# Cwuwhu/FCD-GAN-pytorch

Measured on AMD Instinct MI355X. Metric: tile-pairs/sec (train step) on 256x256x13 OSCD, higher is better.
Workload: dtype f32

## Files before the change

fcd_gan_pytorch_amd/Loss.py:

```python
import os
import warnings

import torch
import torch.nn as nn
import torch.nn.functional as F

from . import _lib
from . import _ops as ops
from .ssim import MS_SSIM

_VGG_CFG = (64, 64, 'M', 128, 128, 'M', 256, 256, 256, 'M', 512, 512, 512, 'M', 512, 512, 512, 'M')
_TAPS = (29, 22, 15, 8, 3)


def _vgg16_features():
    layers, cin = [], 3
    for v in _VGG_CFG:
        if v == 'M':
            layers.append(nn.MaxPool2d(kernel_size=2, stride=2))
        else:
            layers += [nn.Conv2d(cin, v, kernel_size=3, padding=1), nn.ReLU(inplace=True)]
            cin = v
    return nn.Sequential(*layers)


_HUB_FILE = 'vgg16-397923af.pth'


def _vgg_checkpoint_path():
    path = os.environ.get('FCDGAN_VGG16_WEIGHTS', '')
    if path:
        if not os.path.exists(path):
            raise FileNotFoundError('FCDGAN_VGG16_WEIGHTS=%s does not exist' % path)
        return path
    roots = [os.path.join(os.environ['TORCH_HOME'], 'hub')] if os.environ.get('TORCH_HOME') else []
    roots.append(os.path.join(os.path.expanduser('~'), '.cache', 'torch', 'hub'))
    for r in roots:
        cand = os.path.join(r, 'checkpoints', _HUB_FILE)
        if os.path.exists(cand):
            return cand
    return None


def _load_vgg_weights(net, allow_seeded):
    path = _vgg_checkpoint_path()
    if path:
        sd = torch.load(path, map_location='cpu')
        sd = {k.replace('features.', ''): v for k, v in sd.items() if 'classifier' not in k}
        net.load_state_dict(sd)
        return True
    if not allow_seeded:
        raise RuntimeError(
            'PerceptionLoss: the ImageNet VGG16 weights the reference uses (Loss.py:25, vgg16(pretrained=True)) are '
            'not available offline.  Set FCDGAN_VGG16_WEIGHTS to a torch-saved state_dict of torchvision\'s vgg16 '
            '(or place %s in the torch hub cache), or pass allow_seeded=True to run on fixed-seed random filters '
            '(parity tests / benchmarks only: the loss value then differs from the reference\'s).' % _HUB_FILE)
    warnings.warn('PerceptionLoss: allow_seeded=True -- VGG16 runs on a fixed-seed He initialisation, NOT on the '
                  'ImageNet weights of the reference.')
    g = torch.Generator().manual_seed(16)
    with torch.no_grad():
        for m in net:
            if isinstance(m, nn.Conv2d):
                fan_in = m.weight.shape[1] * 9
                m.weight.copy_(torch.randn(m.weight.shape, generator=g) * (2.0 / fan_in) ** 0.5)
                m.bias.zero_()
    return False


class PerceptionLoss(nn.Module):

    def __init__(self, feature_layer=1, perception_perBand=False, allow_seeded=False):
        super(PerceptionLoss, self).__init__()
        vgg = _vgg16_features().eval()
        self.pretrained = _load_vgg_weights(vgg, allow_seeded)
        for param in vgg.parameters():
            param.requires_grad = False
        self.net = vgg
        feature_layer = feature_layer if feature_layer > 0 else 1
        feature_layer = feature_layer if feature_layer < 6 else 5
        self.feature_layer_list = list(_TAPS[:feature_layer])
        self.perception_perBand = perception_perBand
        self.loss = nn.MSELoss()

    def _first_filter_1ch(self):
        w = self.net[0].weight
        hit = self.__dict__.get('_fcd_w1')
        if hit is None or hit[0] != w._version or hit[1].device != w.device:
            hit = (w._version, w.detach().sum(dim=1, keepdim=True).contiguous())
            self.__dict__['_fcd_w1'] = hit
        return hit[1]

    def _features(self, z, single_band=False):
        taps = {}
        layers = list(self.net)
        i = 0
        while i < len(layers):
            layer = layers[i]
            run = self._frozen_run(layers, i) if isinstance(layer, nn.Conv2d) and i > 0 else None
            if run is not None and ops.frozen_chain_ok(z, [c.weight for c in run[0]]):
                convs, pool, nxt = run
                z = ops.frozen_conv_chain(z, [c.weight for c in convs], [c.bias for c in convs], pool=pool)
                last = nxt - 1
                if last in self.feature_layer_list:
                    taps[last] = z
                i = nxt
                continue
            if isinstance(layer, nn.Conv2d):
                fuse = i + 1 < len(layers) and isinstance(layers[i + 1], nn.ReLU)
                wgt = self._first_filter_1ch() if (i == 0 and single_band) else layer.weight
                pool_next = fuse and i + 2 < len(layers) and isinstance(layers[i + 2], nn.MaxPool2d)
                if pool_next and (i + 1) not in self.feature_layer_list:
                    z = ops.conv2d_relu_maxpool2(z, wgt, layer.bias)
                    i += 3
                    continue
                z = ops.conv2d(z, wgt, layer.bias, 1, 1, relu=fuse)
                if fuse:
                    i += 1
            elif isinstance(layer, nn.ReLU):
                z = ops.bn_act(z, None, ops.ACT_RELU)
            else:
                z = ops.maxpool2(z)
            if i in self.feature_layer_list:
                taps[i] = z
            i += 1
        return taps

    def _frozen_run(self, layers, i):
        convs, k = [], i
        while (k + 1 < len(layers) and isinstance(layers[k], nn.Conv2d) and isinstance(layers[k + 1], nn.ReLU)
               and not layers[k].weight.requires_grad and layers[k].bias is not None and not layers[k].bias.requires_grad):
            convs.append(layers[k])
            k += 2
            if (k - 1) in self.feature_layer_list:
                break
        if len(convs) < 2:
            return None
        pool = (k < len(layers) and isinstance(layers[k], nn.MaxPool2d) and (k - 1) not in self.feature_layer_list
                and k not in self.feature_layer_list)
        return convs, pool, (k + 1 if pool else k)

    def forward(self, target_image, generate_image, cmask, stacked=None):
        n = target_image.shape[0]
        nl = len(self.feature_layer_list)
        if not self.perception_perBand:
            assert target_image.shape[1] >= 3
            if target_image.shape[1] == 3:
                z = stacked if stacked is not None else masked_pair(target_image, generate_image, cmask)
            else:
                keep = 1 - cmask
                z = torch.cat([target_image[:, 0:3] * keep, generate_image[:, 0:3] * keep], dim=0)
            nb = n
        else:
            C, H, W = target_image.shape[1:]
            z = stacked if stacked is not None else masked_pair(target_image, generate_image, cmask)
            z = z.reshape(2 * n * C, 1, H, W)
            nb = n * C
        feats = self._features(z, single_band=self.perception_perBand)
        total = 0
        for i in sorted(self.feature_layer_list):
            f = feats[i]
            total = total + mse_halves(f, nb) / nl
        return total


def masked_pair(target_image, generate_image, cmask):
    if not _lib.switch('FUSED_GLUE') or not target_image.is_cuda:
        keep = 1 - cmask
        return torch.cat([target_image * keep, generate_image * keep], dim=0)
    return ops.masked_stack([target_image, generate_image], cmask)


class _MseHalves(torch.autograd.Function):

    @staticmethod
    def forward(ctx, f, nb):
        d = f[:nb] - f[nb:]
        ctx.save_for_backward(d)
        ctx.n_total = f.shape[0]
        flat = d.reshape(-1)
        return torch.dot(flat, flat) / flat.numel()

    @staticmethod
    def backward(ctx, gout):
        d, = ctx.saved_tensors
        nb = d.shape[0]
        c = gout * (2.0 / d.numel())
        g = torch.empty((ctx.n_total,) + tuple(d.shape[1:]), dtype=d.dtype, device=d.device)
        torch.mul(d, c, out=g[:nb])
        torch.mul(d, -c, out=g[nb:])
        return g, None


def mse_halves(f, nb):
    if f.shape[0] != 2 * nb:
        raise ValueError('mse_halves: %d rows for two halves of %d' % (f.shape[0], nb))
    if not _lib.switch('FUSED_GLUE') or not f.is_cuda:
        return F.mse_loss(f[:nb], f[nb:])
    return _MseHalves.apply(f, nb)


def _masked_ratio(a, b, m, kind, complement, scale, skip_zero):
    if not _lib.switch('FUSED_GLUE'):
        num, wsum = ops.masked_sums(a, b, m, kind, complement)
        return _per_sample_ratio(num, wsum, scale, skip_zero)
    return ops.masked_ratio_mean(a, b, m, kind, complement, scale, skip_zero)


def _per_sample_ratio(num, wsum, scale, skip_zero):
    if skip_zero:
        ok = wsum != 0
        terms = torch.where(ok, num * scale / torch.where(ok, wsum, torch.ones_like(wsum)), torch.zeros_like(num))
    else:
        terms = num * scale / wsum
    return terms.sum() / num.shape[0]


class CNetLoss(nn.Module):

    def __init__(self, channel=4, perception_layer=1, perception_perBand=True, allow_seeded=False):
        super(CNetLoss, self).__init__()
        self.mse = nn.MSELoss()
        self.loss_generator = nn.L1Loss()
        self.loss_perception = PerceptionLoss(feature_layer=perception_layer, perception_perBand=perception_perBand,
                                              allow_seeded=allow_seeded)
        self.ssim = MS_SSIM(data_range=1.0, channel=channel)

    def forward(self, target_image, generate_image, cmap, generator_mask_switch=False):
        C = target_image.shape[1]
        cmask = (torch.sign(cmap - 0.5) + 1) / 2
        generator_loss = _masked_ratio(target_image, generate_image, cmap, 0, True, 1.0 / C, skip_zero=False)
        l1_loss = torch.mean(abs(cmap))
        n = target_image.shape[0]
        z = masked_pair(target_image, generate_image, cmap)
        perception_loss = self.loss_perception(target_image, generate_image, cmask if generator_mask_switch else cmap,
                                               stacked=None if generator_mask_switch else z)
        ssim_loss = 1 - self.ssim(*z.split(n, dim=0))
        return generator_loss, l1_loss, perception_loss, ssim_loss


class CGeneratorLoss(nn.Module):

    def __init__(self, channel=3, perception_layer=1, perception_perBand=False, allow_seeded=False):
        super(CGeneratorLoss, self).__init__()
        self.loss_generator = nn.MSELoss()
        self.ssim = MS_SSIM(data_range=1.0, channel=channel)
        self.loss_perception = PerceptionLoss(feature_layer=perception_layer, perception_perBand=perception_perBand,
                                              allow_seeded=allow_seeded)

    def forward(self, target_image, generate_image, cmap):
        C = target_image.shape[1]
        generator_loss = _masked_ratio(target_image, generate_image, cmap, 1, True, 1.0 / C, skip_zero=True)
        n = target_image.shape[0]
        z = masked_pair(target_image, generate_image, cmap)
        ssim_loss = 1 - self.ssim(*z.split(n, dim=0))
        perception_loss = self.loss_perception(target_image, generate_image, cmap, stacked=z)
        return generator_loss, ssim_loss, perception_loss


def region_loss(cmap, region, criterion):
    if isinstance(criterion, str):
        kind = {'l1': 0, 'mse': 1}[criterion]
    elif isinstance(criterion, nn.L1Loss):
        kind = 0
    elif isinstance(criterion, nn.MSELoss):
        kind = 1
    else:
        raise TypeError('region_loss: criterion must be nn.L1Loss / nn.MSELoss')
    return _masked_ratio(cmap, None, region, kind, False, 1.0 / cmap.shape[1], skip_zero=True)
```

fcd_gan_pytorch_amd/_lib.py:

```python
import ctypes
import os
import subprocess

import torch

from ctypes import POINTER, Structure, c_char_p, c_double, c_float, c_int, c_int32, c_int64, c_size_t, c_void_p

_HERE = os.path.dirname(os.path.abspath(__file__))
LIB_PATH = os.environ.get('FCD_LIB') or os.path.join(_HERE, 'libfcdgan_hip.so')
CSRC = os.path.join(_HERE, 'csrc')


class FcdError(RuntimeError):
    pass


def build(force=False, verbose=False):
    if force and os.path.exists(LIB_PATH):
        os.remove(LIB_PATH)
    cmd = ['make', '-C', CSRC, '-j', str(max(2, os.cpu_count() or 2))]
    r = subprocess.run(cmd, stdout=subprocess.PIPE, stderr=subprocess.STDOUT, text=True)
    if verbose or r.returncode != 0:
        print(r.stdout)
    if r.returncode != 0 or not os.path.exists(LIB_PATH):
        raise FcdError('building libfcdgan_hip.so failed (make -C %s)' % CSRC)
    return LIB_PATH


def kernel_source_hash():
    import runpy
    return runpy.run_path(os.path.join(CSRC, 'source_hash.py'))['source_hash']()


class WinoFwdExtras(Structure):
    _fields_ = [('v_keep', c_void_p), ('bn_part', c_void_p), ('bn_groups', c_int32), ('in_groups', c_int32),
                ('in_scale', c_void_p), ('in_shift', c_void_p)]


class ConvDesc(Structure):
    _fields_ = [(n, c_int32) for n in ('N', 'C', 'H', 'W', 'K', 'R', 'S', 'stride', 'pad', 'P', 'Q')]


P = c_void_p

_SIGS = {
    'fcd_version': (c_int, []),
    'fcd_build_hash': (c_char_p, []),
    'fcd_last_error_string': (c_char_p, []),
    'fcd_switch_count': (c_int, []),
    'fcd_switch_name': (c_char_p, [c_int]),
    'fcd_switch_help': (c_char_p, [c_int]),
    'fcd_switch_default': (c_int, [c_int]),
    'fcd_switch_get': (c_int, [c_char_p]),
    'fcd_switch_set': (c_int, [c_char_p, c_int]),
    'fcd_conv_packed_elems': (c_int64, [c_int, c_int, c_int, c_int, c_int]),
    'fcd_conv_pack_weights': (c_int, [P, P, c_int, c_int, c_int, c_int, c_int, P]),
    'fcd_conv2d_fwd': (c_int, [POINTER(ConvDesc), P, P, P, P, c_int, P]),
    'fcd_conv2d_fwd_ex': (c_int, [POINTER(ConvDesc), P, P, P, P, c_int, P, c_float, P, P]),
    'fcd_conv2d_relu_bits_bytes': (c_size_t, [POINTER(ConvDesc)]),
    'fcd_conv2d_fwd_relu_bits': (c_int, [POINTER(ConvDesc), P, P, P, P, P, P]),
    'fcd_conv2d_bwd_data_bits': (c_int, [POINTER(ConvDesc), P, P, P, P, P]),
    'fcd_conv1x1_head_plan': (c_int, [c_int, c_int, c_int, c_int]),
    'fcd_conv1x1_head_fwd': (c_int, [P, P, P, P, c_int, c_int, c_int, c_int, P]),
    'fcd_conv1x1_head_bwd_ws_bytes': (c_size_t, [c_int, c_int]),
    'fcd_conv1x1_head_bwd': (c_int, [P, P, P, P, P, P, P, c_int, c_int, c_int, P, c_size_t, P]),
    'fcd_conv1x1_head_bn_fwd': (c_int, [P, P, P, c_int, P, P, P, c_int, c_int, c_int, c_int, P]),
    'fcd_conv1x1_head_bn_bwd_ws_bytes': (c_size_t, [c_int, c_int, c_int]),
    'fcd_conv1x1_head_bn_bwd': (c_int, [P, P, P, P, P, P, P, P, c_int, P, P, P, P, P, c_int, c_int, c_int, P, c_size_t, P]),
    'fcd_conv_wino_plan': (c_int, [POINTER(ConvDesc), c_int]),
    'fcd_conv_wino_set': (c_int, [c_int]),
    'fcd_conv_wino_split_set': (c_int, [c_int]),
    'fcd_conv_wgrad_split_set': (c_int, [c_int]),
    'fcd_conv_wino_cat_ok': (c_int, [P]),
    'fcd_conv2d_fwd_wino_cat': (c_int, [P, P, P, c_int, P, P, P, c_int, P, c_size_t, P]),
    'fcd_conv2d_bwd_data_wino_cat': (c_int, [P, P, P, P, P, P, c_int, P, c_size_t, P]),
    'fcd_conv2d_bwd_weight_bias_cat': (c_int, [P, P, P, c_int, P, P, P, P, P, c_size_t, P]),
    'fcd_conv_wino_ws_bytes': (c_size_t, [POINTER(ConvDesc), c_int]),
    'fcd_conv_wino_keepv_bytes': (c_size_t, [POINTER(ConvDesc)]),
    'fcd_conv_wino_in_affine_ok': (c_int, [POINTER(ConvDesc)]),
    'fcd_conv_wino_bn_split': (c_int, [POINTER(ConvDesc), c_int]),
    'fcd_conv_wino_bn_part_bytes': (c_size_t, [POINTER(ConvDesc), c_int]),
    'fcd_conv2d_fwd_wino_x': (c_int, [POINTER(ConvDesc), P, P, P, P, c_int, P, P, P, c_size_t, P, P]),
    'fcd_conv2d_fwd_wino_cat_x': (c_int, [P, P, P, c_int, P, P, P, c_int, P, c_size_t, P, P]),
    'fcd_conv_wino_relu_bits_bytes': (c_size_t, [POINTER(ConvDesc)]),
    'fcd_conv2d_fwd_wino_relu_bits': (c_int, [POINTER(ConvDesc), P, P, P, P, P, P, c_size_t, P]),
    'fcd_conv2d_bwd_data_wino_bits': (c_int, [POINTER(ConvDesc), P, P, P, P, P, c_size_t, P]),
    'fcd_conv_wino_chain_ok': (c_int, [P, c_int, c_int]),
    'fcd_conv_wino_chain_ws_bytes': (c_size_t, [P, c_int, c_int]),
    'fcd_conv_wino_chain_bits_bytes': (c_size_t, [POINTER(ConvDesc)]),
    'fcd_conv2d_fwd_wino_chain': (c_int, [P, c_int, P, P, P, P, P, P, P, P, c_size_t, P]),
    'fcd_conv2d_bwd_data_wino_chain': (c_int, [P, c_int, P, P, P, P, P, P, P, c_size_t, P]),
    'fcd_conv2d_fwd_wino_keepv': (c_int, [POINTER(ConvDesc), P, P, P, P, c_int, P, P, P, c_size_t, P, P]),
    'fcd_conv2d_fwd_wino_cat_keepv': (c_int, [P, P, P, c_int, P, P, P, c_int, P, c_size_t, P, P]),
    'fcd_conv2d_bwd_weight_bias_v': (c_int, [POINTER(ConvDesc), P, P, P, P, P, P, c_size_t, P]),
    'fcd_conv_wino_filter_elems': (c_int64, [c_int, c_int, c_int, c_int]),
    'fcd_conv_wino_pack': (c_int, [P, P, c_int, c_int, c_int, c_int, P]),
    'fcd_conv_wino_pack_blocks': (c_int, [c_int, c_int, c_int]),
    'fcd_conv_wino_pack_multi': (c_int, [P, c_int, c_int, c_double, P]),
    'fcd_conv2d_fwd_wino': (c_int, [POINTER(ConvDesc), P, P, P, P, c_int, P, P, P, c_size_t, P]),
    'fcd_conv2d_bwd_data_wino': (c_int, [POINTER(ConvDesc), P, P, P, P, P, P, c_size_t, P]),
    'fcd_conv_s2_dgrad_plan': (c_int, [POINTER(ConvDesc)]),
    'fcd_conv_s2_dgrad_packed_elems': (c_int64, [c_int, c_int]),
    'fcd_conv_s2_dgrad_pack': (c_int, [P, P, c_int, c_int, P]),
    'fcd_conv2d_bwd_data_s2': (c_int, [POINTER(ConvDesc), P, P, P, P, P]),
    'fcd_conv_wino2_plan': (c_int, [POINTER(ConvDesc), c_int]),
    'fcd_conv_wino2_filter_elems': (c_int64, [c_int, c_int, c_int]),
    'fcd_conv_wino2_pack': (c_int, [P, P, c_int, c_int, c_int, P]),
    'fcd_conv2d_fwd_wino2': (c_int, [POINTER(ConvDesc), P, P, P, P, c_int, P, c_float, P, P, P, P]),
    'fcd_conv2d_bwd_data_wino2': (c_int, [POINTER(ConvDesc), P, P, P, P, P, P]),
    'fcd_conv2d_bwd_data': (c_int, [POINTER(ConvDesc), P, P, P, P, P]),
    'fcd_conv2d_fwd_relu_pool': (c_int, [POINTER(ConvDesc), P, P, P, P, P, P]),
    'fcd_conv2d_bwd_data_pooled': (c_int, [POINTER(ConvDesc), P, P, P, P, P]),
    'fcd_conv2d_bwd_weight_ws_bytes': (c_size_t, [POINTER(ConvDesc)]),
    'fcd_conv2d_bwd_weight': (c_int, [POINTER(ConvDesc), P, P, P, P, P, c_size_t, P]),
    'fcd_conv2d_bwd_weight_bias': (c_int, [POINTER(ConvDesc), P, P, P, P, P, P, c_size_t, P]),
    'fcd_channel_sum_ws_bytes': (c_size_t, [c_int]),
    'fcd_channel_sum': (c_int, [P, P, P, c_int, c_int, c_int, P, c_size_t, P]),
    'fcd_bn_act_ws_bytes': (c_size_t, [c_int, c_int]),
    'fcd_bn_act_fwd': (c_int, [P, P, c_int, c_int, c_int, c_int, c_int, P, P, P, P, c_float, c_float, c_int,
                               P, P, c_int, P, c_float, P, c_size_t, P]),
    'fcd_bn_act_fwd_replay': (c_int, [P, P, c_int, c_int, c_int, c_int, P, c_int, P, P, P, P, c_float, c_float, P, P, c_int, P,
                                      c_float, P, c_size_t, P]),
    'fcd_bn_act_bwd': (c_int, [P, P, P, c_int, c_int, c_int, c_int, c_int, P, P, P, P, c_float, c_int, P, P,
                               c_int, P, c_float, P, P, P, P, c_size_t, P]),
    'fcd_bn_relu_pool_plan': (c_int, [c_int, c_int, c_int, c_int, c_int]),
    'fcd_bn_relu_pool_fwd': (c_int, [P, P, P, c_int, c_int, c_int, c_int, c_int, P, P, P]),
    'fcd_bn_relu_pool_bwd': (c_int, [P, P, P, P, c_int, c_int, c_int, c_int, c_int, P, P, P, P, P, P, P, c_size_t, P]),
    'fcd_bn_train_stats': (c_int, [P, c_int, c_int, c_int, c_int, P, c_int, P, P, P, P, c_float, c_float, P, P, P, P, P, c_size_t, P]),
    'fcd_bn_act_fwd_parts': (c_int, [P, P, c_int, c_int, c_int, c_int, P, c_int, P, P, P, P, c_float, c_float, P, P, c_int, P, c_float,
                                     P, c_size_t, P]),
    'fcd_bn_partial_stats': (c_int, [P, P, c_int, c_int, c_int, c_int, P, c_size_t, P]),
    'fcd_bn_act_fwd_from_stats': (c_int, [P, P, c_int, c_int, c_int, c_int, P, c_double, P, P, P, P, c_float, c_float,
                                          P, P, c_int, P, c_float, P, c_size_t, P]),
    'fcd_bn_bwd_partial': (c_int, [P, P, P, c_int, c_int, c_int, c_int, P, P, P, P, c_int, P, c_float, P, c_size_t, P]),
    'fcd_bn_bwd_from_sums': (c_int, [P, P, P, c_int, c_int, c_int, c_int, P, c_double, P, P, P, P, c_int, P, c_float,
                                     P, c_size_t, P]),
    'fcd_maxpool2_fwd': (c_int, [P, P, c_int, c_int, c_int, P]),
    'fcd_maxpool2_bwd': (c_int, [P, P, P, c_int, c_int, c_int, P]),
    'fcd_maxpool2_bwd_add': (c_int, [P, P, P, P, c_int, c_int, c_int, P]),
    'fcd_upsample2x_fwd': (c_int, [P, P, c_int, c_int, c_int, P]),
    'fcd_upsample2x_bwd': (c_int, [P, P, c_int, c_int, c_int, P]),
    'fcd_avgpool2_pad_fwd': (c_int, [P, P, c_int, c_int, c_int, P]),
    'fcd_avgpool2_pad_bwd': (c_int, [P, P, c_int, c_int, c_int, P]),
    'fcd_pair_gap_diff_fwd': (c_int, [P, P, c_int, c_int, c_int, c_int, P]),
    'fcd_pair_gap_diff_bwd': (c_int, [P, P, c_int, c_int, c_int, c_int, P]),
    'fcd_masked_stack_fwd': (c_int, [P, P, P, P, c_int, P, P, c_int, c_int, c_int, P]),
    'fcd_masked_stack_bwd': (c_int, [P, P, P, P, P, c_int, P, P, P, P, P, P, c_int, c_int, c_int, P]),
    'fcd_normalize_tiles': (c_int, [P, P, P, P, P, c_int, c_int, c_int, P]),
    'fcd_masked_recon_ws_bytes': (c_size_t, [c_int]),
    'fcd_masked_recon_fwd': (c_int, [P, P, P, P, c_int, c_int, c_int, c_int, c_int, P, c_size_t, P]),
    'fcd_masked_recon_bwd': (c_int, [P, P, P, P, P, P, P, P, c_int, c_int, c_int, c_int, c_int, P]),
    'fcd_ratio_mean_fwd': (c_int, [P, c_int, c_float, c_int, P, P]),
    'fcd_ratio_mean_bwd': (c_int, [P, P, c_int, c_float, c_int, P, P, P]),
    'fcd_ssim_ws_bytes': (c_size_t, [c_int, c_int, c_int]),
    'fcd_ssim_level_fwd': (c_int, [P, P, P, c_int, P, c_int, c_int, c_int, c_float, c_float, P, c_size_t, P]),
    'fcd_ssim_level_bwd': (c_int, [P, P, P, c_int, P, P, P, P, c_int, c_int, c_int, c_float, c_float, P, c_size_t, P]),
    'fcd_adam_step': (c_int, [P, P, P, P, c_int64, c_float, c_float, c_float, c_float, c_float, c_int, c_float, P]),
    'fcd_rmsprop_step': (c_int, [P, P, P, c_int64, c_float, c_float, c_float, c_float, c_float, P]),
    'fcd_adam_step_h': (c_int, [P, P, P, P, c_int64, P, c_float, c_float, c_float, c_float, c_float, P]),
    'fcd_rmsprop_step_h': (c_int, [P, P, P, c_int64, P, c_float, c_float, c_float, c_float, P]),
    'fcd_prof_enable': (None, [c_int]),
    'fcd_prof_families': (c_int, []),
    'fcd_prof_detail_read': (c_int64, [c_char_p, c_int64, c_int]),
    'fcd_prof_read': (c_int, [POINTER(c_double), c_int]),
    'fcd_prof_family_name': (c_char_p, [c_int]),
}

EXPORTS = sorted(_SIGS)


def _load():
    if not os.path.exists(LIB_PATH):
        raise FcdError('libfcdgan_hip.so not found at %s -- run `python -c "import __graft_entry__ as g; '
                       'g.build()"` (needs hipcc); there is no CPU fallback.' % LIB_PATH)
    lib = ctypes.CDLL(LIB_PATH)
    for name, (res, args) in _SIGS.items():
        try:
            fn = getattr(lib, name)
        except AttributeError:
            raise FcdError('libfcdgan_hip.so does not export %s (stale build?)' % name)
        fn.restype = res
        fn.argtypes = args
    return lib


lib = _load()


def switch(name):
    v = lib.fcd_switch_get(name.encode())
    if v < 0:
        raise FcdError('unknown switch %r' % name)
    return v


def set_switch(name, value):
    old = lib.fcd_switch_set(name.encode(), -1 if value is None else int(value))
    if old < 0:
        raise FcdError('unknown switch %r' % name)
    return old


class switched:

    def __init__(self, **kv):
        self.kv, self.old = kv, {}

    def __enter__(self):
        for k, v in self.kv.items():
            self.old[k] = set_switch(k, v)
        return self

    def __exit__(self, *exc):
        for k, v in self.old.items():
            set_switch(k, v)
        return False


def switch_table():
    return [(lib.fcd_switch_name(i).decode(), lib.fcd_switch_get(lib.fcd_switch_name(i)), lib.fcd_switch_default(i),
             lib.fcd_switch_help(i).decode()) for i in range(lib.fcd_switch_count())]


def build_hash():
    return lib.fcd_build_hash().decode()


def check(rc, what=''):
    if rc != 0:
        msg = lib.fcd_last_error_string()
        raise FcdError('%s failed (%d): %s' % (what or 'fcd call', rc, msg.decode() if msg else ''))


def prof_read(reset=True):
    nf = lib.fcd_prof_families()
    buf = (c_double * (nf * 4))()
    check(lib.fcd_prof_read(buf, 1 if reset else 0), 'fcd_prof_read')
    out = {}
    for f in range(nf):
        out[lib.fcd_prof_family_name(f).decode()] = dict(ms=buf[f * 4], launches=int(buf[f * 4 + 1]),
                                                         flops=buf[f * 4 + 2], bytes=buf[f * 4 + 3])
    return out


def prof_detail(reset=True):
    need = lib.fcd_prof_detail_read(None, 0, 0)
    buf = ctypes.create_string_buffer(int(need))
    lib.fcd_prof_detail_read(buf, need, 1 if reset else 0)
    out = []
    for line in buf.value.decode().splitlines():
        fam, tag, ms, fl, by = line.split('\t')
        out.append(dict(family=fam, tag=tag, ms=float(ms), flops=float(fl), bytes=float(by)))
    return out
```

fcd_gan_pytorch_amd/_ops.py:

```python
import collections
import ctypes
import threading
import time

import torch

from . import _lib
from ._lib import ConvDesc, check, lib, switch

ACT_NONE, ACT_RELU, ACT_LEAKY, ACT_PRELU = 0, 1, 2, 3


class _LaunchWindow:
    EVERY = 128

    def __init__(self):
        self.count, self.events = 0, collections.deque()

    def note(self, stream):
        self.count += 1
        if self.count % self.EVERY:
            return
        limit = switch('LAUNCH_WINDOW')
        if limit <= 0 or torch.cuda.is_current_stream_capturing():
# ... 278 lines not shown
                nw = lib.fcd_conv_wino_relu_bits_bytes(ctypes.byref(d))
                if nw and switch('WINO_RELU_BITS'):
                    wbits = torch.empty(nw // 2, dtype=torch.int16, device=x.device)
                    ws = _ws(lib.fcd_conv_wino_ws_bytes(ctypes.byref(d), 0), x.device)
                    check(lib.fcd_conv2d_fwd_wino_relu_bits(ctypes.byref(d), _p(x), _p(wino_weight(weight, 0, 4)), _p(b), _p(y),
                                                            _p(wbits), _p(ws), ws.numel(), _stream()),
                          'fcd_conv2d_fwd_wino_relu_bits')
        vk = None
        if bits is None and wbits is None:
            vk = _keepv(d, ctx.needs_input_grad[1], x.device)
            _fwd_conv(d, x, weight, b, y, relu, v_keep=vk, bn_part=bn_part, bn_groups=bn_groups)
        ctx.save_for_backward(x if (weight.requires_grad and vk is None) else None, weight,
                              (y if relu and bits is None and wbits is None else None), bits, vk, wbits)
        ctx.geom = (stride, pad, bias is not None, tuple(x.shape))
        ctx.bias_param = bias
        return y

    @staticmethod
    def backward(ctx, dy):
        x, weight, yrelu, bits, vk, wbits = ctx.saved_tensors
        stride, pad, has_bias, xshape = ctx.geom
        dy = _dev(dy, 'conv grad')
        d = _desc(xshape, weight.shape, stride, pad)
        dx = dw = db = None
        if ctx.needs_input_grad[0]:
            dx = torch.empty(xshape, dtype=torch.float32, device=dy.device)
            if bits is not None:
                check(lib.fcd_conv2d_bwd_data_bits(ctypes.byref(d), _p(dy), _p(bits), _p(packed_weight(weight, 1)), _p(dx),
                                                   _stream()), 'fcd_conv2d_bwd_data_bits')
            elif wbits is not None:
                ws = _ws(lib.fcd_conv_wino_ws_bytes(ctypes.byref(d), 1), dy.device)
                check(lib.fcd_conv2d_bwd_data_wino_bits(ctypes.byref(d), _p(dy), _p(wbits), _p(wino_weight(weight, 1, 4)), _p(dx),
                                                        _p(ws), ws.numel(), _stream()), 'fcd_conv2d_bwd_data_wino_bits')
            else:
                _bwd_data_conv(d, dy, weight, dx, yrelu=yrelu)
        want_db = has_bias and ctx.needs_input_grad[2]
        if ctx.needs_input_grad[1]:
            dw = _grad_out(weight, weight.shape, dy.device)
            if want_db:
                db = _grad_out(ctx.bias_param, (d.K,), dy.device)
            ws = _ws(lib.fcd_conv2d_bwd_weight_ws_bytes(ctypes.byref(d)), dy.device)
            if vk is not None:
                check(lib.fcd_conv2d_bwd_weight_bias_v(ctypes.byref(d), _p(vk), _p(dy), _p(yrelu), _p(dw), _p(db), _p(ws),
                                                       ws.numel(), _stream()), 'fcd_conv2d_bwd_weight_bias_v')
            else:
                check(lib.fcd_conv2d_bwd_weight_bias(ctypes.byref(d), _p(x), _p(dy), _p(yrelu), _p(dw), _p(db), _p(ws),
                                                     ws.numel(), _stream()), 'fcd_conv2d_bwd_weight_bias')
        elif want_db:
            db = _channel_sum(dy, yrelu, d.N, d.K, d.P * d.Q)
        return dx, dw, db, None, None, None, None, None


def _ptr_list(ptrs):
    return (ctypes.c_void_p * len(ptrs))(*ptrs)


class _ConvPairCat(torch.autograd.Function):

    @staticmethod
    def forward(ctx, f2n, up, weight, bias, relu, bn_part=None, bn_groups=0):
        f2n, up = _dev(f2n, 'skip pair'), _dev(up, 'upsampled input')
        n, cu, H, W = up.shape
        c = f2n.shape[1]
        d = _desc((n, 2 * c + cu, H, W), weight.shape, 1, 1)
        y = torch.empty((d.N, d.K, d.P, d.Q), dtype=torch.float32, device=up.device)
        half = n * c * H * W * 4
        srcs = _ptr_list([f2n.data_ptr(), f2n.data_ptr() + half, up.data_ptr()])
        chans = (ctypes.c_int * 3)(c, c, cu)
        ws = _ws(lib.fcd_conv_wino_ws_bytes(ctypes.byref(d), 0), up.device)
        b = _dev(bias, 'conv bias') if bias is not None else None
        vk = _keepv(d, ctx.needs_input_grad[2], up.device)
        check(lib.fcd_conv2d_fwd_wino_cat_x(ctypes.byref(d), srcs, chans, 3, _p(wino_weight(weight, 0, 4)), _p(b), _p(y),
                                            1 if relu else 0, _p(ws), ws.numel(), _extras(vk, bn_part, bn_groups), _stream()),
              'fcd_conv2d_fwd_wino_cat')
        keep_x = weight.requires_grad and vk is None
        ctx.save_for_backward(f2n if keep_x else None, up if keep_x else None, weight, y if relu else None, vk)
        ctx.geom = (tuple(f2n.shape), tuple(up.shape), bias is not None)
        ctx.bias_param = bias
        return y

    @staticmethod
    def backward(ctx, dy):
        f2n, up, weight, yrelu, vk = ctx.saved_tensors
        fshape, ushape, has_bias = ctx.geom
        dy = _dev(dy, 'conv grad')
        n, cu, H, W = ushape
        c = fshape[1]
        d = _desc((n, 2 * c + cu, H, W), weight.shape, 1, 1)
        chans = (ctypes.c_int * 3)(c, c, cu)
        half = n * c * H * W * 4
        df = du = dw = db = None
        if ctx.needs_input_grad[0] or ctx.needs_input_grad[1]:
            df = torch.empty(fshape, dtype=torch.float32, device=dy.device)
            du = torch.empty(ushape, dtype=torch.float32, device=dy.device)
            ws = _ws(lib.fcd_conv_wino_ws_bytes(ctypes.byref(d), 1), dy.device)
            check(lib.fcd_conv2d_bwd_data_wino_cat(ctypes.byref(d), _p(dy), _p(yrelu), _p(wino_weight(weight, 1, 4)),
                                                   _ptr_list([df.data_ptr(), df.data_ptr() + half, du.data_ptr()]), chans, 3,
                                                   _p(ws), ws.numel(), _stream()), 'fcd_conv2d_bwd_data_wino_cat')
        want_db = has_bias and ctx.needs_input_grad[3]
        if ctx.needs_input_grad[2]:
            dw = _grad_out(weight, weight.shape, dy.device)
            if want_db:
                db = _grad_out(ctx.bias_param, (d.K,), dy.device)
            ws = _ws(lib.fcd_conv2d_bwd_weight_ws_bytes(ctypes.byref(d)), dy.device)
            if vk is not None:
                check(lib.fcd_conv2d_bwd_weight_bias_v(ctypes.byref(d), _p(vk), _p(dy), _p(yrelu), _p(dw), _p(db), _p(ws),
                                                       ws.numel(), _stream()), 'fcd_conv2d_bwd_weight_bias_v')
            else:
                check(lib.fcd_conv2d_bwd_weight_bias_cat(ctypes.byref(d), _ptr_list([f2n.data_ptr(), f2n.data_ptr() + half,
                                                                                      up.data_ptr()]), chans, 3, _p(dy), _p(yrelu),
                                                         _p(dw), _p(db), _p(ws), ws.numel(), _stream()),
                      'fcd_conv2d_bwd_weight_bias_cat')
        elif want_db:
            db = _channel_sum(dy, yrelu, d.N, d.K, d.P * d.Q)
        return df, du, dw, db, None, None, None


def conv3x3_pair_cat_ok(f2n, up, weight):
    if f2n.dim() != 4 or up.dim() != 4 or tuple(weight.shape[2:]) != (3, 3) or not switch('PAIR_CAT'):
        return False
    n, cu, H, W = up.shape
    c = f2n.shape[1]
    if f2n.shape[0] != 2 * n or tuple(f2n.shape[2:]) != (H, W) or (c % 32) or (cu % 32) or weight.shape[1] != 2 * c + cu:
        return False
    if not (f2n.is_cuda and up.is_cuda and f2n.is_contiguous() and up.is_contiguous()):
        return False
    d = _desc((n, 2 * c + cu, H, W), weight.shape, 1, 1)
    return bool(lib.fcd_conv_wino_cat_ok(ctypes.byref(d)))


def conv3x3_pair_cat(f2n, up, weight, bias=None, relu=False, bn_groups=0):
    n, cu, H, W = up.shape
    d = _desc((n, 2 * f2n.shape[1] + cu, H, W), weight.shape, 1, 1)
    part = _bn_part(d, bn_groups, relu, up.device)
    return _tag_bn(_ConvPairCat.apply(f2n, up, weight, bias, bool(relu), part, int(bn_groups)), d, part, bn_groups)


def conv2d(x, weight, bias=None, stride=1, padding=0, relu=False, bn_groups=0):
    part = None
    if bn_groups and not relu and x.is_cuda:
        d = _desc(x.shape, weight.shape, int(stride), int(padding))
        part = _bn_part(d, bn_groups, relu, x.device)
        if part is not None:
            return _tag_bn(_Conv2d.apply(x, weight, bias, int(stride), int(padding), False, part, int(bn_groups)), d, part, bn_groups)
    return _Conv2d.apply(x, weight, bias, int(stride), int(padding), bool(relu))


@torch.no_grad()
def conv2d_infer(x, weight, bias, stride=1, padding=0, act=ACT_NONE, slope=None, slope_imm=0.0, residual=None):
    x = _dev(x, 'conv input')
    d = _desc(x.shape, weight.shape, int(stride), int(padding))
    y = torch.empty((d.N, d.K, d.P, d.Q), dtype=torch.float32, device=x.device)
    res = _dev(residual, 'residual') if residual is not None else None
    if res is not None and res.shape != y.shape:
        raise _lib.FcdError('conv2d_infer: residual shape %s != output shape %s' % (tuple(res.shape), tuple(y.shape)))
    if lib.fcd_conv_wino2_plan(ctypes.byref(d), 0):
        check(lib.fcd_conv2d_fwd_wino2(ctypes.byref(d), _p(x), _p(wino2_weight(weight, 0)), _p(bias), _p(y), act, _p(slope),
                                       float(slope_imm), _p(res), None, None, _stream()), 'fcd_conv2d_fwd_wino2')
        return y
    wp = packed_weight(weight, 0)
    check(lib.fcd_conv2d_fwd_ex(ctypes.byref(d), _p(x), _p(wp), _p(bias), _p(y), act, _p(slope), float(slope_imm),
                                _p(res), _stream()), 'fcd_conv2d_fwd_ex')
    return y


class _ConvReluPool(torch.autograd.Function):

    @staticmethod
    def forward(ctx, x, weight, bias):
        x = _dev(x, 'conv input')
        d = _desc(x.shape, weight.shape, 1, 1)
        yp = torch.empty((d.N, d.K, d.P // 2, d.Q // 2), dtype=torch.float32, device=x.device)
        code = torch.empty(yp.shape, dtype=torch.uint8, device=x.device)
        _fwd_conv(d, x, weight, bias, None, True, pool_y=yp, code=code)
        ctx.save_for_backward(weight, code)
        ctx.xshape = tuple(x.shape)
        return yp

    @staticmethod
    def backward(ctx, dyp):
        weight, code = ctx.saved_tensors
        dyp = _dev(dyp, 'pooled grad')
        d = _desc(ctx.xshape, weight.shape, 1, 1)
        dx = None
        if ctx.needs_input_grad[0]:
            dx = torch.empty(ctx.xshape, dtype=torch.float32, device=dyp.device)
            _bwd_data_conv(d, dyp, weight, dx, code=code)
        return dx, None, None


def conv_relu_pool_supported(x, weight):
    K, C, R, S = weight.shape
    if switch('NO_POOLFUSE'):
        return False
    return (R == 3 and S == 3 and K > 32 and C > 32 and not weight.requires_grad
            and x.shape[2] >= 2 and x.shape[3] >= 2)


def conv2d_relu_maxpool2(x, weight, bias):
    if conv_relu_pool_supported(x, weight) and (bias is None or not bias.requires_grad):
        return _ConvReluPool.apply(x, weight, bias)
    return maxpool2(conv2d(x, weight, bias, 1, 1, relu=True))


def _desc_array(descs):
    arr = (ConvDesc * len(descs))()
    for i, d in enumerate(descs):
        for f, _ in ConvDesc._fields_:
            setattr(arr[i], f, getattr(d, f))
    return arr


def _chain_descs(xshape, weights):
    N, C, H, W = xshape
    out = []
    for w in weights:
        out.append(_desc((N, C, H, W), w.shape, 1, 1))
        C = w.shape[0]
    return out


def _chain_bwd_start(descs):
    n = len(descs)
    for j in range(n):
        if lib.fcd_conv_wino_chain_ok(_desc_array(descs[j:]), n - j, 1):
            return j
    return n


def frozen_chain_ok(x, weights):
    if not switch('WINO_CHAIN') or len(weights) < 2 or len(weights) > 8 or not x.is_cuda or x.dim() != 4:
        return False
    if any(w.requires_grad or tuple(w.shape[2:]) != (3, 3) for w in weights):
        return False
    descs = _chain_descs(x.shape, weights)
    if not lib.fcd_conv_wino_chain_ok(_desc_array(descs), len(descs), 0):
        return False
    return _chain_bwd_start(descs) <= 1


class _FrozenChain(torch.autograd.Function):

    @staticmethod
    def forward(ctx, x, pool, *wb):
        x = _dev(x, 'conv input')
        n = len(wb) // 2
        weights, biases = list(wb[:n]), [_dev(b, 'conv bias') for b in wb[n:]]
        descs = _chain_descs(x.shape, weights)
        darr = _desc_array(descs)
        N, H, W = descs[0].N, descs[0].H, descs[0].W
        K = descs[-1].K
        dev = x.device
        want = ctx.needs_input_grad[0]
        bits = []
        if want:
            for i in range(n - (1 if pool else 0)):
                bits.append(torch.empty(lib.fcd_conv_wino_chain_bits_bytes(ctypes.byref(descs[i])) // 2, dtype=torch.int16, device=dev))
        y = yp = code = None
        if pool:
            yp = torch.empty((N, K, H // 2, W // 2), dtype=torch.float32, device=dev)
            code = torch.empty(yp.shape, dtype=torch.uint8, device=dev)
        else:
            y = torch.empty((N, K, H, W), dtype=torch.float32, device=dev)
        Us = [wino_weight(w, 0, 4) for w in weights]
        ws = _ws(lib.fcd_conv_wino_chain_ws_bytes(darr, n, 0), dev)
        bptr = _ptr_list([b.data_ptr() for b in bits] + [None] * (n - len(bits))) if want else None
        check(lib.fcd_conv2d_fwd_wino_chain(darr, n, _p(x), _ptr_list([u.data_ptr() for u in Us]),
                                            _ptr_list([b.data_ptr() for b in biases]), _p(y), _p(yp), _p(code), bptr, _p(ws),
                                            ws.numel(), _stream()), 'fcd_conv2d_fwd_wino_chain')
        ctx.save_for_backward(code, *weights, *bits)
        ctx.geom = (tuple(x.shape), n, bool(pool))
        return yp if pool else y

    @staticmethod
    def backward(ctx, dy):
        xshape, n, pool = ctx.geom
        saved = ctx.saved_tensors
        code, weights, bits = saved[0], list(saved[1:1 + n]), list(saved[1 + n:])
        dy = _dev(dy, 'conv grad')
        if not ctx.needs_input_grad[0]:
            return (None,) * (2 + 2 * n)
        descs = _chain_descs(xshape, weights)
        j = _chain_bwd_start(descs)
        if j > 1:
            raise _lib.FcdError('frozen_conv_chain: no backward run for these layers (frozen_chain_ok was not consulted)')
        dev = dy.device
        dx = torch.empty((xshape[0], descs[j].C) + tuple(xshape[2:]), dtype=torch.float32, device=dev)
        darr = _desc_array(descs[j:])
        m = n - j
        ws = _ws(lib.fcd_conv_wino_chain_ws_bytes(darr, m, 1), dev)
        blist = [(bits[i].data_ptr() if i < len(bits) else None) for i in range(j, n)]
        U1 = [wino_weight(w, 1, 4) for w in weights[j:]]
        check(lib.fcd_conv2d_bwd_data_wino_chain(darr, m, _p(dy), _p(code) if pool else None, _ptr_list(blist),
                                                 _p(bits[0]) if j == 1 else None, _ptr_list([u.data_ptr() for u in U1]),
                                                 _p(dx), _p(ws), ws.numel(), _stream()), 'fcd_conv2d_bwd_data_wino_chain')
        if j == 1:
            dx0 = torch.empty(xshape, dtype=torch.float32, device=dev)
            _bwd_data_conv(descs[0], dx, weights[0], dx0)
            dx = dx0
        return (dx, None) + (None,) * (2 * n)


def frozen_conv_chain(x, weights, biases, pool=False):
    return _FrozenChain.apply(x, bool(pool), *weights, *biases)


class _ConvT2x2(torch.autograd.Function):

    @staticmethod
    def forward(ctx, x, weight, bias):
        x = _dev(x, 'convT input')
        Cin, Cout = weight.shape[0], weight.shape[1]
        N, _, h, w = x.shape
        d = ConvDesc(N, Cout, 2 * h, 2 * w, Cin, 2, 2, 2, 0, h, w)
        y = torch.empty((N, Cout, 2 * h, 2 * w), dtype=torch.float32, device=x.device)
        wpb = packed_weight(weight, 1)
        check(lib.fcd_conv2d_bwd_data(ctypes.byref(d), _p(x), None, _p(wpb), _p(y), _stream()), 'convT fwd')
        if bias is not None:
            y += bias.view(1, -1, 1, 1)
        ctx.save_for_backward(x, weight)
        ctx.has_bias = bias is not None
        return y

    @staticmethod
    def backward(ctx, dy):
        x, weight = ctx.saved_tensors
        dy = _dev(dy, 'convT grad')
        Cin, Cout = weight.shape[0], weight.shape[1]
        N, _, h, w = x.shape
        d = ConvDesc(N, Cout, 2 * h, 2 * w, Cin, 2, 2, 2, 0, h, w)
        dx = dw = db = None
        if ctx.needs_input_grad[0]:
            dx = torch.empty_like(x)
            wp = packed_weight(weight, 0)
            check(lib.fcd_conv2d_fwd(ctypes.byref(d), _p(dy), _p(wp), None, _p(dx), 0, _stream()), 'convT bwd data')
        if ctx.needs_input_grad[1]:
            dw = _grad_out(weight, weight.shape, x.device)
            ws = _ws(lib.fcd_conv2d_bwd_weight_ws_bytes(ctypes.byref(d)), x.device)
            check(lib.fcd_conv2d_bwd_weight(ctypes.byref(d), _p(dy), _p(x), None, _p(dw), _p(ws), ws.numel(), _stream()),
                  'convT bwd weight')
        if ctx.has_bias and ctx.needs_input_grad[2]:
            db = _channel_sum(dy, None, N, Cout, 4 * h * w)
        return dx, dw, db


def conv_transpose2x2(x, weight, bias=None):
    return _ConvT2x2.apply(x, weight, bias)


SYNC_BN = {'enabled': False, 'group': None}


def _sync_world():
    if SYNC_BN['enabled']:
        from . import dp
        return dp.exchanging(SYNC_BN['group'])
    return 0


def sync_bn_active():
    return bool(_sync_world())


class _BnAct(torch.autograd.Function):
    @staticmethod
    def forward(ctx, x, gamma, beta, slope, running_mean, running_var, training, momentum, eps, groups, act,
                slope_imm, order=None):
        x = _dev(x, 'bn input')
        N, C, H, W = x.shape
        has_bn = gamma is not None
        y = torch.empty_like(x)
        save_mean = save_invstd = None
        if has_bn and training:
            save_mean = torch.empty(groups * C, dtype=torch.float32, device=x.device)
            save_invstd = torch.empty(groups * C, dtype=torch.float32, device=x.device)
        ws = _ws(lib.fcd_bn_act_ws_bytes(C, groups), x.device)
        world = _sync_world() if (has_bn and training) else 0
        parts = getattr(x, '_fcd_bn', None) if (has_bn and training and not world) else None
        if parts is not None and (parts[3] != x.data_ptr() or parts[4] != x._version):
            parts = None
        if order is not None:
            if not (has_bn and training) or world:
                raise ValueError('bn_act(order=...): train-mode BatchNorm without SyncBN only')
            arr = (ctypes.c_int * len(order))(*[int(g) for g in order])
            check(lib.fcd_bn_act_fwd_replay(_p(x), _p(y), N, C, H * W, groups, arr, len(order), _p(gamma), _p(beta),
                                            _p(running_mean), _p(running_var), float(momentum), float(eps), _p(save_mean),
                                            _p(save_invstd), act, _p(slope), float(slope_imm), _p(ws), ws.numel(), _stream()),
                  'fcd_bn_act_fwd_replay')
        elif parts is not None and parts[2] == groups and parts[1] > 0:
            check(lib.fcd_bn_act_fwd_parts(_p(x), _p(y), N, C, H * W, groups, _p(parts[0]), parts[1], _p(gamma), _p(beta),
                                           _p(running_mean), _p(running_var), float(momentum), float(eps), _p(save_mean),
                                           _p(save_invstd), act, _p(slope), float(slope_imm), _p(ws), ws.numel(), _stream()),
                  'fcd_bn_act_fwd_parts')
        elif world:
            import torch.distributed as dist
            sums = torch.empty(groups * C * 2, dtype=torch.float64, device=x.device)
            check(lib.fcd_bn_partial_stats(_p(x), _p(sums), N, C, H * W, groups, _p(ws), ws.numel(), _stream()),
                  'fcd_bn_partial_stats')
            dist.all_reduce(sums, group=SYNC_BN['group'])
            SYNC_BN['calls'] = SYNC_BN.get('calls', 0) + 1
            count = float(N // groups) * H * W * world
            check(lib.fcd_bn_act_fwd_from_stats(_p(x), _p(y), N, C, H * W, groups, _p(sums), count, _p(gamma), _p(beta),
                                                _p(running_mean), _p(running_var), float(momentum), float(eps),
                                                _p(save_mean), _p(save_invstd), act, _p(slope), float(slope_imm),
                                                _p(ws), ws.numel(), _stream()), 'fcd_bn_act_fwd_from_stats')
        else:
            check(lib.fcd_bn_act_fwd(_p(x), _p(y), N, C, H * W, groups, int(has_bn), _p(gamma), _p(beta),
                                     _p(running_mean), _p(running_var), float(momentum), float(eps), int(training),
                                     _p(save_mean), _p(save_invstd), act, _p(slope), float(slope_imm), _p(ws),
                                     ws.numel(), _stream()), 'fcd_bn_act_fwd')
        if has_bn and training and running_mean is not None:
            torch._C._increment_version([running_mean, running_var])
        keep_running = has_bn and not training
        ctx.save_for_backward(x, gamma, beta, slope, save_mean, save_invstd,
                              running_mean if keep_running else None, running_var if keep_running else None)
        ctx.cfg = (bool(training), float(eps), groups, act, float(slope_imm), has_bn, world)
        return y

    @staticmethod
    def backward(ctx, dz):
        x, gamma, beta, slope, save_mean, save_invstd, running_mean, running_var = ctx.saved_tensors
        training, eps, groups, act, slope_imm, has_bn, world = ctx.cfg
        dz = _dev(dz, 'bn grad')
        N, C, H, W = x.shape
        dx = torch.empty_like(x)
        dgamma = dbeta = dslope = None
        ws = _ws(lib.fcd_bn_act_ws_bytes(C, groups), x.device)
        if world:
            import torch.distributed as dist
            part = torch.empty(groups * C * 3, dtype=torch.float64, device=x.device)
            check(lib.fcd_bn_bwd_partial(_p(dz), _p(x), _p(part), N, C, H * W, groups, _p(gamma), _p(beta),
                                         _p(save_mean), _p(save_invstd), act, _p(slope), slope_imm, _p(ws), ws.numel(),
                                         _stream()), 'fcd_bn_bwd_partial')
            local = part.view(groups, C, 3)
            dbeta = local[:, :, 0].sum(0).float()
            dgamma = local[:, :, 1].sum(0).float()
            if slope is not None and ctx.needs_input_grad[3]:
                dslope = local[:, :, 2].sum().float().view(slope.shape)
            tot = part.clone()
            dist.all_reduce(tot, group=SYNC_BN['group'])
            SYNC_BN['calls'] = SYNC_BN.get('calls', 0) + 1
            count = float(N // groups) * H * W * world
            check(lib.fcd_bn_bwd_from_sums(_p(dz), _p(x), _p(dx), N, C, H * W, groups, _p(tot), count, _p(gamma),
                                           _p(beta), _p(save_mean), _p(save_invstd), act, _p(slope), slope_imm, _p(ws),
                                           ws.numel(), _stream()), 'fcd_bn_bwd_from_sums')
            return dx, dgamma, dbeta, dslope, None, None, None, None, None, None, None, None, None
        if has_bn and (ctx.needs_input_grad[1] or ctx.needs_input_grad[2]):
            dgamma = _grad_out(gamma, (C,), x.device)
            dbeta = _grad_out(beta, (C,), x.device)
        if slope is not None and ctx.needs_input_grad[3]:
            dslope = _grad_out(slope, tuple(slope.shape), x.device)
        check(lib.fcd_bn_act_bwd(_p(dz), _p(x), _p(dx), N, C, H * W, groups, int(has_bn), _p(gamma), _p(beta),
                                 _p(running_mean), _p(running_var), eps, int(training), _p(save_mean),
                                 _p(save_invstd), act, _p(slope), slope_imm, _p(dgamma), _p(dbeta), _p(dslope),
                                 _p(ws), ws.numel(), _stream()), 'fcd_bn_act_bwd')
        return dx, dgamma, dbeta, dslope, None, None, None, None, None, None, None, None, None


class _BnReluConv2d(torch.autograd.Function):

    @staticmethod
    def forward(ctx, z, gamma, beta, running_mean, running_var, momentum, eps, groups, weight, bias, parts, bn_part, bn_groups):
        z = _dev(z, 'bn input')
        _dev(weight, 'conv weight')
        N, C, H, W = z.shape
        d = _desc(z.shape, weight.shape, 1, 1)
        dev = z.device
        save_mean = torch.empty(groups * C, dtype=torch.float32, device=dev)
        save_invstd = torch.empty(groups * C, dtype=torch.float32, device=dev)
        sc = torch.empty(2, groups * C, dtype=torch.float32, device=dev)
        ws = _ws(lib.fcd_bn_act_ws_bytes(C, groups), dev)
        check(lib.fcd_bn_train_stats(_p(z), N, C, H * W, groups, _p(parts[0]) if parts is not None else None,
                                     parts[1] if parts is not None else 0, _p(gamma), _p(beta), _p(running_mean), _p(running_var),
                                     float(momentum), float(eps), _p(save_mean), _p(save_invstd), _p(sc[0]), _p(sc[1]), _p(ws),
                                     ws.numel(), _stream()), 'fcd_bn_train_stats')
        if running_mean is not None:
            torch._C._increment_version([running_mean, running_var])
        y = torch.empty((d.N, d.K, d.P, d.Q), dtype=torch.float32, device=dev)
        b = _dev(bias, 'conv bias') if bias is not None else None
        vk = _keepv(d, ctx.needs_input_grad[8], dev)
        ex = _lib.WinoFwdExtras(vk.data_ptr() if vk is not None else None, bn_part.data_ptr() if bn_part is not None else None,
                                int(bn_groups), int(groups), sc[0].data_ptr(), sc[1].data_ptr())
        wsc = _ws(lib.fcd_conv_wino_ws_bytes(ctypes.byref(d), 0), dev)
        check(lib.fcd_conv2d_fwd_wino_x(ctypes.byref(d), _p(z), _p(wino_weight(weight, 0, 4)), _p(b), _p(y), 0, None, None, _p(wsc),
                                        wsc.numel(), ctypes.byref(ex), _stream()), 'fcd_conv2d_fwd_wino_x')
        if ctx.needs_input_grad[8] and vk is None:
            raise _lib.FcdError('bn_relu_conv3x3: the layer keeps no transformed input for its weight gradient (check bn_relu_conv3x3_ok)')
        ctx.save_for_backward(z, gamma, beta, save_mean, save_invstd, weight, vk)
        ctx.cfg = (float(eps), int(groups), bias is not None)
        ctx.bias_param = bias
        return y

    @staticmethod
    def backward(ctx, dy):
        z, gamma, beta, save_mean, save_invstd, weight, vk = ctx.saved_tensors
        eps, groups, has_bias = ctx.cfg
        dy = _dev(dy, 'conv grad')
        N, C, H, W = z.shape
        d = _desc(z.shape, weight.shape, 1, 1)
        dev = dy.device
        dz = dgamma = dbeta = dw = db = None
        want_bn = ctx.needs_input_grad[0] or ctx.needs_input_grad[1] or ctx.needs_input_grad[2]
        if want_bn:
            da = torch.empty(z.shape, dtype=torch.float32, device=dev)
            _bwd_data_conv(d, dy, weight, da)
            dz = torch.empty_like(z)
            if ctx.needs_input_grad[1] or ctx.needs_input_grad[2]:
                dgamma = _grad_out(gamma, (C,), dev)
                dbeta = _grad_out(beta, (C,), dev)
            ws = _ws(lib.fcd_bn_act_ws_bytes(C, groups), dev)
            check(lib.fcd_bn_act_bwd(_p(da), _p(z), _p(dz), N, C, H * W, groups, 1, _p(gamma), _p(beta), None, None, eps, 1,
                                     _p(save_mean), _p(save_invstd), ACT_RELU, None, 0.0, _p(dgamma), _p(dbeta), None, _p(ws),
                                     ws.numel(), _stream()), 'fcd_bn_act_bwd')
            del da
        want_db = has_bias and ctx.needs_input_grad[9]
        if ctx.needs_input_grad[8]:
            dw = _grad_out(weight, weight.shape, dev)
            if want_db:
                db = _grad_out(ctx.bias_param, (d.K,), dev)
            ws = _ws(lib.fcd_conv2d_bwd_weight_ws_bytes(ctypes.byref(d)), dev)
            check(lib.fcd_conv2d_bwd_weight_bias_v(ctypes.byref(d), _p(vk), _p(dy), None, _p(dw), _p(db), _p(ws), ws.numel(),
                                                   _stream()), 'fcd_conv2d_bwd_weight_bias_v')
        elif want_db:
            db = _channel_sum(dy, None, d.N, d.K, d.P * d.Q)
        return dz, dgamma, dbeta, None, None, None, None, None, dw, db, None, None, None


def bn_relu_conv3x3_ok(z, bn, weight, groups=1):
    if not (torch.is_tensor(z) and z.is_cuda and z.dim() == 4 and z.dtype == torch.float32):
        return False
    if not (bn.training or bn.running_mean is None) or bn.weight is None or bn.bias is None or _sync_world():
        return False
    if tuple(weight.shape[2:]) != (3, 3) or weight.shape[1] != z.shape[1] or z.shape[0] % groups:
        return False
    d = _desc(z.shape, weight.shape, 1, 1)
    if lib.fcd_conv_wino2_plan(ctypes.byref(d), 0) or not lib.fcd_conv_wino_in_affine_ok(ctypes.byref(d)):
        return False
    return not (weight.requires_grad and torch.is_grad_enabled()) or lib.fcd_conv_wino_keepv_bytes(ctypes.byref(d)) > 0


def bn_relu_conv3x3(z, bn, weight, bias=None, groups=1, bn_groups=0):
    parts = getattr(z, '_fcd_bn', None)
    if parts is not None and (parts[3] != z.data_ptr() or parts[4] != z._version or parts[2] != groups or parts[1] <= 0):
        parts = None
    d = _desc(z.shape, weight.shape, 1, 1)
    part = _bn_part(d, bn_groups, False, z.device)
    y = _BnReluConv2d.apply(z, bn.weight, bn.bias, bn.running_mean, bn.running_var,
                            bn.momentum if bn.momentum is not None else 0.1, bn.eps, int(groups), weight, bias,
                            (parts[0], parts[1]) if parts is not None else None, part, int(bn_groups) if part is not None else 0)
    _count_batches(bn, groups)
    return _tag_bn(y, d, part, bn_groups)


_TLS = threading.local()


def _count_batches(bn, calls):
    if bn.track_running_stats and bn.num_batches_tracked is not None:
        pending = getattr(_TLS, 'counters', None)
        if pending is not None:
            pending.append((bn.num_batches_tracked, calls))
        else:
            bn.num_batches_tracked += calls


class batched_bn_counters:

    def __enter__(self):
        self.outer = getattr(_TLS, 'counters', None) is not None
        if not self.outer:
            _TLS.counters = []
        return self

    def __exit__(self, *exc):
        if self.outer:
            return False
        todo, _TLS.counters = _TLS.counters, None
        by_step = {}
        for t, g in todo:
            by_step.setdefault(int(g), []).append(t)
        for g, ts in by_step.items():
            uniq, seen = [], {}
            for t in ts:
                k = id(t)
                if k in seen:
                    seen[k][1] += g
                else:
                    seen[k] = [t, g]
            same = [v[0] for v in seen.values() if v[1] == g]
            if same:
                torch._foreach_add_(same, g)
            for t, tot in seen.values():
                if tot != g:
                    t += tot
        return False


def bn_act(x, bn=None, act=ACT_NONE, slope=None, slope_imm=0.0, groups=1, order=None):
    if bn is None:
        return _BnAct.apply(x, None, None, slope, None, None, False, 0.0, 0.0, groups, act, slope_imm)
    training = bn.training or bn.running_mean is None
    if order is not None and not (training and bn.running_mean is not None):
        order = None
    calls = len(order) if order is not None else groups
    y = _BnAct.apply(x, bn.weight, bn.bias, slope, bn.running_mean, bn.running_var, training,
                     bn.momentum if bn.momentum is not None else 0.1, bn.eps, groups, act, slope_imm,
                     tuple(order) if order is not None else None)
# ... 511 lines not shown
```

fcd_gan_pytorch_amd/csrc/conv_wino.h:

```cpp
#pragma once
#include <stdlib.h>

#include "common.h"

typedef float f32x16 __attribute__((ext_vector_type(16)));
typedef float f32x4 __attribute__((ext_vector_type(4)));
typedef float f32x2 __attribute__((ext_vector_type(2)));
typedef __attribute__((address_space(3))) void lds_void_t;
typedef __attribute__((address_space(1))) const void gbl_void_t;

template <int M> struct WinoMat;
template <> struct WinoMat<2> {
  static constexpr int A = 4;
  __host__ __device__ static constexpr float BT(int i, int j) {
    constexpr float t[4][4] = {{1, 0, -1, 0}, {0, 1, 1, 0}, {0, -1, 1, 0}, {0, 1, 0, -1}};
    return t[i][j];
  }
  __host__ __device__ static constexpr float G(int i, int j) {
    constexpr float t[4][3] = {{1, 0, 0}, {.5f, .5f, .5f}, {.5f, -.5f, .5f}, {0, 0, 1}};
    return t[i][j];
  }
  __host__ __device__ static constexpr float AT(int i, int j) {
    constexpr float t[2][4] = {{1, 1, 1, 0}, {0, 1, -1, -1}};
    return t[i][j];
  }
};
template <> struct WinoMat<4> {
  static constexpr int A = 6;
  __host__ __device__ static constexpr float BT(int i, int j) {
    constexpr float t[6][6] = {{225.f / 512, 0, -169.f / 128, 0, 1.f / 2, 0},   {0, -45.f / 64, -9.f / 8, 5.f / 16, 1.f / 2, 0},
                               {0, 45.f / 64, -9.f / 8, -5.f / 16, 1.f / 2, 0}, {0, -75.f / 128, -25.f / 64, 3.f / 2, 1, 0},
                               {0, 75.f / 128, -25.f / 64, -3.f / 2, 1, 0},     {0, 225.f / 512, 0, -169.f / 128, 0, 1.f / 2}};
    return t[i][j];
  }
  __host__ __device__ static constexpr float G(int i, int j) {
    constexpr float t[6][3] = {{512.f / 225, 0, 0},
                               {-4096.f / 2975, -512.f / 595, -64.f / 119},
                               {-4096.f / 2975, 512.f / 595, -64.f / 119},
                               {128.f / 1071, 64.f / 357, 32.f / 119},
                               {128.f / 1071, -64.f / 357, 32.f / 119},
                               {0, 0, 2}};
    return t[i][j];
  }
  __host__ __device__ static constexpr float AT(int i, int j) {
    constexpr float t[4][6] = {{1, 1, 1, 1, 1, 0},
                               {0, 5.f / 8, -5.f / 8, 3.f / 2, -3.f / 2, 0},
                               {0, 25.f / 64, 25.f / 64, 9.f / 4, 9.f / 4, 0},
                               {0, 125.f / 512, -125.f / 512, 27.f / 8, -27.f / 8, 1}};
    return t[i][j];
  }
};

struct WinoCat {
  const float* p[3];
  int c[3];
  int n;
};
__device__ __forceinline__ const float* wino_cat_pick(const WinoCat& k, int& ch, int& chans) {
  int s = 0;
  if (k.n > 1 && ch >= k.c[0]) { ch -= k.c[0]; s = 1; if (k.n > 2 && ch >= k.c[1]) { ch -= k.c[1]; s = 2; } }
  chans = k.c[s];
  return k.p[s];
}

struct WinoInArgs {
  const float* x;
  const float* mask;
  const unsigned short* mbits;
  const unsigned char* code;
  float* V;
  int N, C, H, W, Hp, Wp, TH, TW, Q;
  long long T;
  int exp;
  int xcd;
  WinoCat cat;
  const float* aff_scale;
  const float* aff_shift;
  int aff_ng;
};

__device__ __forceinline__ unsigned xcd_contiguous_id(unsigned lin, unsigned total) {
  const unsigned j = lin & 7u, i = lin >> 3, q8 = total >> 3, r8 = total & 7u;
  return j * q8 + (j < r8 ? j : r8) + i;
}

struct WinoGemmArgs {
  const float* A;
  const float* B;
  float* C;
  int M, N, Kc, m_tiles, n_tiles, xcd_remap;
  long long a_ld, a_batch, b_ld, b_adv, b_batch;
  long long a_adv;
  int stages_per_split;
  const unsigned short* As;
  long long as_plane;
  int batches, xb;
  int c_blk;
  int c_mblk, c_tblk;
  long long c_batch;
  int bt;
  long long bt_T;
  unsigned long long* tbuf;
};

__device__ __forceinline__ void wino_gemm_block(int mode, unsigned& v, unsigned& by, unsigned& bz) {
  const unsigned gx = gridDim.x, gy = gridDim.y;
  if (mode == 2) {
    const unsigned L = blockIdx.x + gx * (blockIdx.y + gy * blockIdx.z);
    const unsigned P = gy * gridDim.z, P8 = P & ~7u;
    unsigned p, t;
    if (L < P8 * gx) {
      const unsigned r = L >> 3;
      t = r % gx;
      p = (r / gx) * 8 + (L & 7u);
    } else {
      const unsigned Lt = L - P8 * gx, rem = P - P8;
      p = P8 + Lt % rem;
      t = Lt / rem;
    }
    v = t; by = p % gy; bz = p / gy;
    return;
  }
  by = blockIdx.y; bz = blockIdx.z;
  const unsigned b = blockIdx.x;
  if (mode == 1) {
    const unsigned q8 = gx >> 3, r8 = gx & 7u, xcd = b & 7u;
    v = (xcd < r8 ? xcd * (q8 + 1) : r8 * (q8 + 1) + (xcd - r8) * q8) + (b >> 3);
  } else {
    v = b;
  }
}

struct WinoOutArgs {
  const float* Mb;
  const float* bias;
  float* y;
  float* pool_y;
  unsigned char* code;
  int K, P, Q, TH, TW, relu;
  long long T;
  WinoCat cat;
  int tblk;
  long long xs_blk;
  unsigned short* bits;
  const unsigned short* gate;
  double* bn_part;
  int bn_bpg;
};

struct WinoOiArgs {
  const float* Mb;
  long long xs_blk;
  int tblk;
  const float* bias;
  int relu;
  unsigned short* bits_out;
  const unsigned short* gate;
  float* V;
  int N, K, H, W, TH, TW, Q;
  long long T;
};
int wino_oi_ok(int K, int H, int W);
void wino_oi_launch(const WinoOiArgs& a, hipStream_t st);

struct WinoPlan {
  int m, A2, rows, red, Kc, Q, TH, TW;
  long long T;
  size_t v_bytes, m_bytes;
};


#define WINO_TERM(S, FIRST, C, X)                                        \
  {                                                                      \
    const float c_ = (C);                                                \
    if (c_ != 0.f) {                                                     \
      if (FIRST) { S = (c_ == 1.f) ? (X) : ((c_ == -1.f) ? -(X) : c_ * (X)); FIRST = false; } \
      else if (c_ == 1.f) S = S + (X);                                   \
      else if (c_ == -1.f) S = S - (X);                                  \
      else S = __builtin_fmaf(c_, (X), S);                               \
    }                                                                    \
  }
template <int MM>
__device__ __forceinline__ void wino_out_tile(const float (&mv)[WinoMat<MM>::A][WinoMat<MM>::A], float b, int relu,
                                              float (&o)[MM][MM]) {
#pragma clang fp contract(off)
  constexpr int A = WinoMat<MM>::A;
  float t1[MM][A];
#pragma unroll
  for (int i = 0; i < MM; ++i)
#pragma unroll
    for (int j = 0; j < A; ++j) {
      float s = 0.f;
      bool first = true;
#pragma unroll
      for (int q = 0; q < A; ++q) WINO_TERM(s, first, WinoMat<MM>::AT(i, q), mv[q][j])
      t1[i][j] = s;
    }
#pragma unroll
  for (int i = 0; i < MM; ++i)
#pragma unroll
    for (int j = 0; j < MM; ++j) {
      float s = 0.f;
      bool first = true;
#pragma unroll
      for (int q = 0; q < A; ++q) WINO_TERM(s, first, WinoMat<MM>::AT(j, q), t1[i][q])
      s = s + b;
      if (relu) s = s > 0.f ? s : 0.f;
      o[i][j] = s;
    }
}
template <int MM>
__device__ __forceinline__ void wino_in_rows(const float (&d)[WinoMat<MM>::A][WinoMat<MM>::A],
                                             float (&t1)[WinoMat<MM>::A][WinoMat<MM>::A]) {
#pragma clang fp contract(off)
  constexpr int A = WinoMat<MM>::A;
#pragma unroll
  for (int i = 0; i < A; ++i)
#pragma unroll
    for (int j = 0; j < A; ++j) {
      float s = 0.f;
      bool first = true;
#pragma unroll
      for (int k = 0; k < A; ++k) WINO_TERM(s, first, WinoMat<MM>::BT(i, k), d[k][j])
      t1[i][j] = s;
    }
}
template <int MM>
__device__ __forceinline__ float wino_in_col(const float (&t1)[WinoMat<MM>::A][WinoMat<MM>::A], int i, int j) {
#pragma clang fp contract(off)
  constexpr int A = WinoMat<MM>::A;
  float s = 0.f;
  bool first = true;
#pragma unroll
  for (int k = 0; k < A; ++k) WINO_TERM(s, first, WinoMat<MM>::BT(j, k), t1[i][k])
  return s;
}
```

fcd_gan_pytorch_amd/csrc/conv_wino.hip:

```cpp
#include "conv_wino.h"


__device__ __forceinline__ unsigned short bf16_rn_bits(float x) {
  const __bf16 b = (__bf16)x;
  return __builtin_bit_cast(unsigned short, b);
}

template <int MM>
__device__ __forceinline__ void wino_filter_items(const float* __restrict__ w, float* __restrict__ U, int K, int C, int rows, int Kc,
                                                  int mode, unsigned short* __restrict__ planes, long long i0, long long istep) {
  constexpr int A = WinoMat<MM>::A;
  const long long total = (long long)rows * Kc;
  const long long pairs = total >> 1;
  for (long long i = i0; i < pairs; i += istep) {
    const int kc0 = (int)((2 * i) % Kc), row = (int)((2 * i) / Kc);
    float g[2][3][3];
#pragma unroll
    for (int e = 0; e < 2; ++e) {
      const int kc = kc0 + e;
#pragma unroll
      for (int r = 0; r < 3; ++r)
#pragma unroll
        for (int s = 0; s < 3; ++s) {
          float v = 0.f;
// ... 971 lines not shown
#pragma unroll
    for (int j = 0; j < 2; ++j)
#pragma unroll
      for (int r = 0; r < 16; ++r) acc[i][j][r] = 0.f;

#if YG_TIME
  unsigned long long ytacc[8] = {0, 0, 0, 0, 0, 0, 0, 0};
#endif
  YG_T(y_begin)
  int fq = 0, fb = 0;
#define Y_DMA(SA, SB)                                                                            \
  {                                                                                              \
    const unsigned short* as_ = Ab + (size_t)fb * a.a_batch + (size_t)fq * KC;                   \
    const float* bs_ = Bb + (size_t)fb * a.b_batch + (size_t)fq * a.b_adv;                       \
    _Pragma("unroll") for (int j = 0; j < PPW_A; ++j)                                            \
      __builtin_amdgcn_global_load_lds((gbl_void_t*)(as_ + (size_t)(j >> 1) * a.as_plane + a_goff[j & 1]), \
                                       (lds_void_t*)((SA) + (wave + NW * j) * 512), 16, 0, 0);   \
    _Pragma("unroll") for (int j = 0; j < PPW_B; ++j)                                            \
      __builtin_amdgcn_global_load_lds((gbl_void_t*)(bs_ + b_goff[j]),                           \
                                       (lds_void_t*)((SB) + (wave + NW * j) * 256), 16, 0, 0);   \
    if (++fq == Q) { fq = 0; ++fb; }                                                             \
  }
#define Y_LOADA(SA, S, IH, AH, AM, AL)                                                           \
  _Pragma("unroll") for (int i = 0; i < 2; ++i) {                                                \
    const unsigned short* ap = (SA) + aoff[2 * (IH) + i] + (((S) ^ swa) * 8);                    \
    AH[i] = *(const u32x4*)(ap);                        \
    AM[i] = *(const u32x4*)(ap + 2 * BM * 2 * 8);         \
    AL[i] = *(const u32x4*)(ap + 2 * (2 * BM * 2 * 8)); \
  }
#define Y_MFMA(IH, AV, BV)                                                                       \
  _Pragma("unroll") for (int i = 0; i < 2; ++i)                                                  \
    _Pragma("unroll") for (int j = 0; j < 2; ++j)                                                \
      acc[2 * (IH) + i][j] = __builtin_amdgcn_mfma_f32_32x32x16_bf16(                            \
          __builtin_bit_cast(bf16x8, AV[i]), __builtin_bit_cast(bf16x8, BV[j]), acc[2 * (IH) + i][j], 0, 0, 0);
#define Y_SIX(IH, AH, AM, AL, BH, BM_, BL)                                                       \
  Y_MFMA(IH, AL, BH) Y_MFMA(IH, AH, BL) Y_MFMA(IH, AM, BM_) Y_MFMA(IH, AM, BH) Y_MFMA(IH, AH, BM_) Y_MFMA(IH, AH, BH)
#define Y_STEP(SA, SB, SAN, SBN)                                                                 \
  {                                                                                              \
    YG_T(ys0)                                                                                    \
    f32x4 xa[2][2];                                                                              \
    u32x4 pah[2], pam[2], pal[2], qah[2], qam[2], qal[2];                                        \
    u32x4 bh0[2], bm0[2], bl0[2], bh1[2], bm1[2], bl1[2];                                        \
    _Pragma("unroll") for (int j = 0; j < 2; ++j) {                                              \
      xa[j][0] = *(const f32x4*)((SB) + boff[j] + ((0 ^ swb) * 4)); \
      xa[j][1] = *(const f32x4*)((SB) + boff[j] + ((1 ^ swb) * 4)); \
    }                                                                                            \
    Y_LOADA(SA, 0, 0, pah, pam, pal)                                                             \
    _Pragma("unroll") for (int j = 0; j < 2; ++j) WS_SPLIT(xa[j][0], xa[j][1], bh0[j], bm0[j], bl0[j]) \
    _Pragma("unroll") for (int j = 0; j < 2; ++j) {                                              \
      xa[j][0] = *(const f32x4*)((SB) + boff[j] + ((2 ^ swb) * 4)); \
      xa[j][1] = *(const f32x4*)((SB) + boff[j] + ((3 ^ swb) * 4)); \
    }                                                                                            \
    YG_T(ys1)                                                                                    \
    Y_SIX(0, pah, pam, pal, bh0, bm0, bl0)                                                       \
    _Pragma("unroll") for (int j = 0; j < 2; ++j) WS_SPLIT(xa[j][0], xa[j][1], bh1[j], bm1[j], bl1[j]) \
    Y_LOADA(SA, 0, 1, qah, qam, qal)                                                             \
    Y_SIX(1, qah, qam, qal, bh0, bm0, bl0)                                                       \
    if (fb < nb) Y_DMA(SAN, SBN)       \
    Y_LOADA(SA, 1, 0, pah, pam, pal)                                                             \
    Y_SIX(0, pah, pam, pal, bh1, bm1, bl1)                                                       \
    Y_LOADA(SA, 1, 1, qah, qam, qal)                                                             \
    Y_SIX(1, qah, qam, qal, bh1, bm1, bl1)                                                       \
    __builtin_amdgcn_sched_group_barrier(0x100, 10, 0);              \
    __builtin_amdgcn_sched_group_barrier(0x002, 88, 0);                        \
    __builtin_amdgcn_sched_group_barrier(0x008, 1, 0);                                           \
    __builtin_amdgcn_sched_group_barrier(0x100, 4, 0);                         \
    __builtin_amdgcn_sched_group_barrier(0x008, 3, 0);                                           \
    _Pragma("unroll") for (int k = 0; k < 14; ++k) {         \
      __builtin_amdgcn_sched_group_barrier(0x008, 1, 0);                                         \
      __builtin_amdgcn_sched_group_barrier(0x002, 6, 0);                                         \
    }                                                                                            \
    __builtin_amdgcn_sched_group_barrier(0x002, 4, 0);                                           \
    _Pragma("unroll") for (int k = 0; k < 6; ++k) {           \
      __builtin_amdgcn_sched_group_barrier(0x008, 1, 0);                                         \
      __builtin_amdgcn_sched_group_barrier(0x100, 1, 0);                                         \
    }                                                                                            \
    _Pragma("unroll") for (int k = 0; k < 6; ++k) {          \
      __builtin_amdgcn_sched_group_barrier(0x008, 2, 0);                                         \
      __builtin_amdgcn_sched_group_barrier(0x100, 1, 0);                                         \
    }                                                                                            \
    __builtin_amdgcn_sched_group_barrier(0x008, 12, 0);                                          \
    _Pragma("unroll") for (int k = 0; k < 6; ++k) {          \
      __builtin_amdgcn_sched_group_barrier(0x008, 2, 0);                                         \
      __builtin_amdgcn_sched_group_barrier(0x100, 1, 0);                                         \
    }                                                                                            \
    __builtin_amdgcn_sched_group_barrier(0x008, 36, 0);                                          \
    __builtin_amdgcn_sched_barrier(0);                                                           \
    YG_T(ys2)                                                                                    \
    if (YG_TIME) __builtin_amdgcn_s_waitcnt(0x0F70);         \
    YG_T(ys2b)                                                                                   \
    __syncthreads();                                                                             \
    YG_T(ys3)                                                                                    \
    YG_TACC(0, ys1, ys0) YG_TACC(1, ys2, ys1) YG_TACC(2, ys3, ys2b) YG_TACC(4, ys2b, ys2)         \
  }

  Y_DMA(sa0, sb0)
  __syncthreads();
#pragma unroll 1
  for (int cb = 0; cb < nb; ++cb) {
    for (int qc = 0; qc < Q; qc += 2) {
      Y_STEP(sa0, sb0, sa1, sb1)
      if (qc + 1 < Q) Y_STEP(sa1, sb1, sa0, sb0)
    }
    YG_T(yc0)
    if (a.c_blk) {
      float* Cb = a.C + (size_t)(b_first + cb) * a.c_batch;
#pragma unroll
      for (int i = 0; i < 4; ++i)
#pragma unroll
        for (int j = 0; j < 2; ++j) {
          const int mb = (m0 + wm * 128 + i * 32) >> 5, tb = (n0 + wn * 64 + j * 32) >> 5;
          if (mb < a.c_mblk && tb < a.c_tblk) {
            float* blk = Cb + ((size_t)mb * a.c_tblk + tb) * 1024 + (half * 4 * 32 + l31) * 4;
#pragma unroll
            for (int g = 0; g < 4; ++g)
              { const f32x4 cv_ = f32x4{acc[i][j][4 * g], acc[i][j][4 * g + 1], acc[i][j][4 * g + 2], acc[i][j][4 * g + 3]};
                __builtin_nontemporal_store(cv_, (f32x4*)(blk + g * 128)); }
          }
#pragma unroll
          for (int r = 0; r < 16; ++r) acc[i][j][r] = 0.f;
        }
      YG_T(yc1)
      YG_TACC(3, yc1, yc0)
      continue;
    }
    int ldc = a.N;
    asm volatile("" : "+s"(ldc));
    float* Cb = a.C + (size_t)(b_first + cb) * a.M * ldc;
#pragma unroll
    for (int i = 0; i < 4; ++i)
#pragma unroll
      for (int r = 0; r < 16; ++r) {
        const int m = m0 + wm * 128 + i * 32 + (r & 3) + 8 * (r >> 2) + 4 * half;
#pragma unroll
        for (int j = 0; j < 2; ++j) {
          const int n = n0 + wn * 64 + j * 32 + l31;
          if (m < a.M && n < ldc) Cb[(size_t)m * ldc + n] = acc[i][j][r];
          acc[i][j][r] = 0.f;
        }
      }
  }
#if YG_TIME
  {
    const unsigned long long y_end = __builtin_readcyclecounter();
    ytacc[6] = y_end - y_begin;
    if (a.tbuf && lane == 0) {
      const size_t wg = (size_t)blockIdx.y * gridDim.x + blockIdx.x;
#pragma unroll
      for (int i = 0; i < 8; ++i) a.tbuf[(wg * NW + wave) * 8 + i] = ytacc[i];
    }
  }
#endif
#undef Y_STEP
#undef Y_SIX
#undef Y_MFMA
#undef Y_LOADA
#undef Y_DMA
}

static int wino_gemm_cfg() { return fcd_sw(FCD_SW_WINO_TILE); }

static int wino_gemm_xb(long long tiles, int batches, int splits, int q_stages) {
  const int forced = fcd_sw(FCD_SW_WINO_XB);
  if (forced > 0) return std::min(forced, batches);
  if (q_stages & 1) return 1;
  static const int cand[] = {36, 18, 12, 9, 6, 4, 3, 2};
  for (int xb : cand) {
    if (batches % xb) continue;
    if (tiles * (batches / xb) * splits >= 2048) return xb;
  }
  return 1;
}

static int wino_split() { return fcd_sw(FCD_SW_WINO_SPLIT); }
static int wino_split_state() { return wino_split(); }
extern "C" int fcd_conv_wino_split_set(int on) {
  const int old = wino_split();
  if (on >= 0) g_fcd_switch[FCD_SW_WINO_SPLIT] = on > 2 ? 1 : on;
  return old;
}

static int wino_xcd();
static int wino_xcd_mode(int tiles, int groups) {
  const int max_tiles = fcd_sw(FCD_SW_WINO_XCD2);
  if (!wino_xcd()) return 0;
  return (tiles <= max_tiles && groups >= 8) ? 2 : 1;
}

static void wino_gemm_launch(WinoGemmArgs ga, int batches, int splits, hipStream_t st) {
  int cfg = wino_gemm_cfg();
  if (ga.As && ga.M > 64 && wino_split()) {
    ga.batches = batches;
    if (splits > 1 || ga.bt || ga.a_adv) {
      ga.m_tiles = cdiv(ga.M, 128); ga.n_tiles = cdiv(ga.N, 128);
      ga.xb = 1;
      ga.xcd_remap = wino_xcd_mode(ga.m_tiles * ga.n_tiles, batches * splits) == 2 ? 2 : 0;
      const dim3 grid((unsigned)(ga.m_tiles * ga.n_tiles), (unsigned)batches, (unsigned)splits);
      if (ga.bt) hipLaunchKernelGGL((wino_gemm_split_kernel<2, 2, true>), grid, dim3(256), 0, st, ga);
      else hipLaunchKernelGGL((wino_gemm_split_kernel<2, 2>), grid, dim3(256), 0, st, ga);
      return;
    }
    if (fcd_sw(FCD_SW_WINO_RES) && ga.c_blk && ga.M <= 128 && ga.Kc <= 128 && (long long)cdiv(ga.N, 256) * batches >= 512) {
      ga.m_tiles = 1; ga.n_tiles = cdiv(ga.N, 256);
      ga.xb = 1;
      const int wgs = fcd_sw(FCD_SW_WINO_RES_WGS);
      const int chunks = std::max(1, std::min(ga.n_tiles, wgs / batches));
      hipLaunchKernelGGL(wino_gemm_split_res_kernel, dim3((unsigned)chunks, (unsigned)batches), dim3(512), 0, st, ga);
      return;
    }
    const int big = fcd_sw(FCD_SW_WINO_SPLIT_BIG);
    const bool force = big == 2 || wino_split() == 2;
    if (big && ga.M >= 256 && (force || (long long)cdiv(ga.M, 256) * cdiv(ga.N, 256) * batches >= 1024)) {
      ga.m_tiles = cdiv(ga.M, 256); ga.n_tiles = cdiv(ga.N, 256);
      ga.xb = wino_gemm_xb((long long)ga.m_tiles * ga.n_tiles * 2, batches, 1, ga.Kc / 32);
      ga.xcd_remap = wino_xcd_mode(ga.m_tiles * ga.n_tiles, cdiv(batches, ga.xb));
      const dim3 grid((unsigned)(ga.m_tiles * ga.n_tiles), (unsigned)cdiv(batches, ga.xb));
#if YG_TIME
      ga.tbuf = g_yg_tbuf;
#endif
      hipLaunchKernelGGL((wino_gemm_split256_kernel<0>), grid, dim3(512), 0, st, ga);
      return;
    }
    ga.m_tiles = cdiv(ga.M, 128); ga.n_tiles = cdiv(ga.N, 128);
    ga.xb = wino_gemm_xb((long long)ga.m_tiles * ga.n_tiles, batches, 1, ga.Kc / 32);
    ga.xcd_remap = wino_xcd_mode(ga.m_tiles * ga.n_tiles, cdiv(batches, ga.xb));
    hipLaunchKernelGGL((wino_gemm_split_kernel<2, 2>), dim3((unsigned)(ga.m_tiles * ga.n_tiles), (unsigned)cdiv(batches, ga.xb)),
                       dim3(256), 0, st, ga);
    return;
  }
  if (cfg == 2 && (ga.M < 256 || ga.N < 256)) cfg = 1;
  if (cfg == 1 && ga.M < 256) cfg = 0;
  ga.batches = batches;
#define WG_LAUNCH(WM_, WN_, BM_, BN_, THREADS_)                                                              \
  {                                                                                                          \
    ga.m_tiles = cdiv(ga.M, BM_); ga.n_tiles = cdiv(ga.N, BN_);                                              \
    ga.xb = splits > 1 ? 1 : wino_gemm_xb((long long)ga.m_tiles * ga.n_tiles, batches, splits, ga.Kc / 32);                               \
    hipLaunchKernelGGL((wino_gemm_kernel<WM_, WN_>),                                                         \
                       dim3((unsigned)(ga.m_tiles * ga.n_tiles), (unsigned)cdiv(batches, ga.xb), (unsigned)splits), \
                       dim3(THREADS_), 0, st, ga);                                                           \
  }
  if (ga.M <= 64) {
    WG_LAUNCH(1, 4, 64, 256, 256)
  } else if (cfg == 2) {
    WG_LAUNCH(4, 4, 256, 256, 1024)
  } else if (cfg == 1) {
    WG_LAUNCH(4, 2, 256, 128, 512)
  } else {
    WG_LAUNCH(2, 2, 128, 128, 256)
  }
#undef WG_LAUNCH
}

template <int MM>
__device__ __forceinline__ void wino_out_one(const WinoOutArgs& a, const float (&mv)[WinoMat<MM>::A][WinoMat<MM>::A], int k,
                                             long long t, double* s1 = nullptr, double* s2 = nullptr) {
  constexpr int A = WinoMat<MM>::A;
  const float b = a.bias ? a.bias[k] : 0.f;
  float o[MM][MM];
  wino_out_tile<MM>(mv, b, a.relu, o);
  const int tx = (int)(t % a.TW);
  const long long r2 = t / a.TW;
  const int ty = (int)(r2 % a.TH), n = (int)(r2 / a.TH);
  if (MM == 4 && a.gate != nullptr) {
    const unsigned gw = a.gate[(((size_t)n * a.K + k) * a.TH + ty) * a.TW + tx];
#pragma unroll
    for (int i = 0; i < MM; ++i)
#pragma unroll
      for (int j = 0; j < MM; ++j) o[i][j] = ((gw >> (4 * i + j)) & 1u) ? o[i][j] : 0.f;
  }
  if (s1 != nullptr) {
    double a1 = 0.0, a2 = 0.0;
#pragma unroll
    for (int i = 0; i < MM; ++i)
#pragma unroll
      for (int j = 0; j < MM; ++j)
        if (ty * MM + i < a.P && tx * MM + j < a.Q) { a1 += (double)o[i][j]; a2 += (double)o[i][j] * (double)o[i][j]; }
    *s1 = a1; *s2 = a2;
  }
  if (MM == 4 && a.bits != nullptr) {
    unsigned w = 0;
#pragma unroll
    for (int i = 0; i < MM; ++i)
#pragma unroll
      for (int j = 0; j < MM; ++j) w |= (o[i][j] > 0.f ? 1u : 0u) << (4 * i + j);
    a.bits[(((size_t)n * a.K + k) * a.TH + ty) * a.TW + tx] = (unsigned short)w;
  }
  const int p0 = ty * MM, q0 = tx * MM;
  if (a.pool_y != nullptr) {
    const int Pp = a.P >> 1, Qp = a.Q >> 1;
    float mabs = 0.f;
#pragma unroll
    for (int i = 0; i < A; ++i)
#pragma unroll
      for (int j = 0; j < A; ++j) mabs = fmaxf(mabs, fabsf(mv[i][j]));
    const float tie_floor = (MM == 4 ? 4e-6f : 5e-7f) * mabs;
#pragma unroll
    for (int wi = 0; wi < MM / 2; ++wi)
#pragma unroll
      for (int wj = 0; wj < MM / 2; ++wj) {
        const int pp = (p0 >> 1) + wi, qq = (q0 >> 1) + wj;
        if (pp >= Pp || qq >= Qp) continue;
        const float c0 = o[2 * wi][2 * wj], c1 = o[2 * wi][2 * wj + 1], c2 = o[2 * wi + 1][2 * wj],
                    c3 = o[2 * wi + 1][2 * wj + 1];
        const float m = fmaxf(fmaxf(c0, c1), fmaxf(c2, c3));
        const float tie = (MM == 4 ? 3e-5f : 2e-6f) * fmaxf(fmaxf(fabsf(c0), fabsf(c1)), fmaxf(fabsf(c2), fabsf(c3))) + tie_floor;
        const float mx = m - tie;
        int arg = 3;
        if (c2 >= mx) arg = 2;
        if (c1 >= mx) arg = 1;
        if (c0 >= mx) arg = 0;
        const size_t oo = (((size_t)n * a.K + k) * Pp + pp) * Qp + qq;
        a.pool_y[oo] = m;
        a.code[oo] = (unsigned char)(arg | (m > 0.f ? 4 : 0));
      }
    return;
  }
  float* yo = a.y + (((size_t)n * a.K + k) * a.P + p0) * a.Q + q0;
  if (a.cat.n > 0) {
    int ch = k, chans;
    float* base = const_cast<float*>(wino_cat_pick(a.cat, ch, chans));
    yo = base + (((size_t)n * chans + ch) * a.P + p0) * a.Q + q0;
  }
  const bool vec = (MM == 4) ? ((a.Q & 3) == 0) : ((a.Q & 1) == 0);
#pragma unroll
  for (int i = 0; i < MM; ++i) {
    if (p0 + i >= a.P) continue;
    if (vec && q0 + MM <= a.Q) {
      if (MM == 4) {
        f32x4 v4 = {o[i][0], o[i][1], o[i][2], o[i][3]};
        *(f32x4*)(yo + (size_t)i * a.Q) = v4;
      } else {
        f32x2 v2 = {o[i][0], o[i][1]};
        *(f32x2*)(yo + (size_t)i * a.Q) = v2;
      }
    } else {
#pragma unroll
      for (int j = 0; j < MM; ++j)
        if (q0 + j < a.Q) yo[(size_t)i * a.Q + j] = o[i][j];
    }
  }
}

template <int MM>
__global__ __launch_bounds__(256) void wino_output_kernel(WinoOutArgs a) {
  constexpr int A = WinoMat<MM>::A;
  const long long t = (long long)blockIdx.x * 256 + threadIdx.x;
  const int k = blockIdx.y;
  if (t >= a.T) return;
  const size_t xs = (size_t)a.K * a.T;
  const float* mp = a.Mb + (size_t)k * a.T + t;
  float mv[A][A];
#pragma unroll
  for (int i = 0; i < A; ++i)
#pragma unroll
    for (int j = 0; j < A; ++j) mv[i][j] = mp[(size_t)(i * A + j) * xs];
  wino_out_one<MM>(a, mv, k, t);
}

__global__ __launch_bounds__(256) void wino_output_blk_kernel(WinoOutArgs a) {
  constexpr int A = 6;
  const long long t = (long long)blockIdx.x * 256 + threadIdx.x;
  const int k0 = blockIdx.y * 4;
  if (t >= a.T) return;
  const float* mp = a.Mb + ((size_t)(k0 >> 5) * a.tblk + (size_t)(t >> 5)) * 1024 +
                    ((((k0 >> 2) & 1) * 4 + ((k0 >> 3) & 3)) * 32 + (int)(t & 31)) * 4;
  f32x4 m4[A * A];
#pragma unroll
  for (int q = 0; q < A * A; ++q) m4[q] = __builtin_nontemporal_load((const f32x4*)(mp + (size_t)q * a.xs_blk));
#pragma unroll
  for (int c = 0; c < 4; ++c) {
    if (k0 + c >= a.K) break;
    float mv[A][A];
#pragma unroll
    for (int q = 0; q < A * A; ++q) mv[q / A][q % A] = m4[q][c];
    wino_out_one<4>(a, mv, k0 + c, t);
  }
}

__global__ __launch_bounds__(256) void wino_output_blk_bn_kernel(WinoOutArgs a) {
  constexpr int A = 6;
  __shared__ double red[4][8];
  const long long t = (long long)blockIdx.x * 256 + threadIdx.x;
  const int k0 = blockIdx.y * 4;
  const bool live = t < a.T;
  double bs[4][2];
#pragma unroll
  for (int c = 0; c < 4; ++c) bs[c][0] = bs[c][1] = 0.0;
  if (live) {
    const float* mp = a.Mb + ((size_t)(k0 >> 5) * a.tblk + (size_t)(t >> 5)) * 1024 +
                      ((((k0 >> 2) & 1) * 4 + ((k0 >> 3) & 3)) * 32 + (int)(t & 31)) * 4;
    f32x4 m4[A * A];
#pragma unroll
    for (int q = 0; q < A * A; ++q) m4[q] = __builtin_nontemporal_load((const f32x4*)(mp + (size_t)q * a.xs_blk));
#pragma unroll
    for (int c = 0; c < 4; ++c) {
      if (k0 + c >= a.K) break;
      float mv[A][A];
#pragma unroll
      for (int q = 0; q < A * A; ++q) mv[q / A][q % A] = m4[q][c];
      wino_out_one<4>(a, mv, k0 + c, t, &bs[c][0], &bs[c][1]);
    }
  }
  const int lane = threadIdx.x & 63, wave = threadIdx.x >> 6;
#pragma unroll
  for (int c = 0; c < 4; ++c)
#pragma unroll
    for (int e = 0; e < 2; ++e) {
      const double v = wave_sum_d(bs[c][e]);
      if (lane == 0) red[wave][c * 2 + e] = v;
    }
  __syncthreads();
  if (threadIdx.x < 8) {
    const int c = threadIdx.x >> 1, e = threadIdx.x & 1;
    if (k0 + c < a.K) {
      const double v = (red[0][threadIdx.x] + red[1][threadIdx.x]) + (red[2][threadIdx.x] + red[3][threadIdx.x]);
      const int g = (int)(blockIdx.x / a.bn_bpg), bi = (int)(blockIdx.x % a.bn_bpg);
      a.bn_part[(((size_t)g * a.K + (k0 + c)) * a.bn_bpg + bi) * 3 + e] = v;
    }
  }
}

static int wino_env() { return fcd_sw(FCD_SW_WINO); }

int fcd_wino_mode_now() { return wino_env(); }

extern "C" int fcd_conv_wino_set(int m) {
  const int prev = wino_env();
  if (m == 0 || m == 2 || m == 4) g_fcd_switch[FCD_SW_WINO] = m;
  return prev;
}

extern "C" int fcd_conv_wino_plan(const fcd_conv_desc* d, int mode) {
  if (!d || wino_env() == 0) return 0;
  if (!(d->R == 3 && d->S == 3 && d->stride == 1 && d->pad == 1)) return 0;
  const int red = mode == 0 ? d->C : d->K;
  const int rows = mode == 0 ? d->K : d->C;
  const int min_red = fcd_sw(FCD_SW_WINO_MINC), min_rows = fcd_sw(FCD_SW_WINO_MINROWS);
  if (red % 32 != 0 || red < min_red || rows < min_rows) return 0;
  if (d->P < 4 || d->Q < 4) return 0;
  return wino_env();
}

static bool wino_plan(const fcd_conv_desc* d, int mode, WinoPlan* pl) {
  pl->m = fcd_conv_wino_plan(d, mode);
  if (!pl->m) return false;
  const int a = pl->m + 2;
  pl->A2 = a * a;
  pl->rows = mode == 0 ? d->K : d->C;
  pl->red = mode == 0 ? d->C : d->K;
  pl->Kc = round_up(pl->red, 32);
  pl->Q = pl->Kc / 32;
  pl->TH = cdiv(d->H, pl->m);
  pl->TW = cdiv(d->W, pl->m);
  pl->T = (long long)d->N * pl->TH * pl->TW;
  pl->v_bytes = (size_t)pl->A2 * pl->Q * pl->T * 32 * sizeof(float);
  pl->m_bytes = (size_t)pl->A2 * round_up(pl->rows, 32) * ((pl->T + 31) / 32 * 32) * sizeof(float);
  return true;
}

extern "C" size_t fcd_conv_wino_ws_bytes(const fcd_conv_desc* d, int mode) {
  WinoPlan pl;
  if (!d || !wino_plan(d, mode, &pl)) return 0;
  return pl.v_bytes + pl.m_bytes + 256;
}

extern "C" int64_t fcd_conv_wino_filter_elems(int K, int C, int mode, int m) {
  if (m != 2 && m != 4) return 0;
  const int rows = mode == 0 ? K : C, red = mode == 0 ? C : K;
  const int64_t elems = (int64_t)(m + 2) * (m + 2) * rows * round_up(red, 32);
  return elems + elems / 2 * 3;
}

static int wino_split_state();
extern "C" int fcd_conv_wino_pack(const float* w, float* U, int K, int C, int mode, int m, void* stream) {
  FCD_CHECK_ARG(w && U && K > 0 && C > 0 && (mode == 0 || mode == 1) && (m == 2 || m == 4),
                "fcd_conv_wino_pack: bad arguments");
  const int rows = mode == 0 ? K : C, Kc = round_up(mode == 0 ? C : K, 32);
  const long long total = (long long)rows * Kc;
  const int grid = (int)std::min<long long>(cdiv64(total / 2, 256), 4096);
  FcdProfScope prof(FCD_K_PACK, (hipStream_t)stream, 0.0, 4.0 * total * (9 + 1.5 * (m + 2) * (m + 2)));
  unsigned short* planes = (unsigned short*)(U + (long long)(m + 2) * (m + 2) * total);
  const bool split = wino_split_state() != 0 && rows > 64;
  float* Uw = split ? nullptr : U;
  if (!split) planes = nullptr;
  if (m == 2)
    hipLaunchKernelGGL(wino_filter_kernel<2>, dim3(grid), dim3(256), 0, (hipStream_t)stream, w, Uw, K, C, rows, Kc, mode, planes);
  else
    hipLaunchKernelGGL(wino_filter_kernel<4>, dim3(grid), dim3(256), 0, (hipStream_t)stream, w, Uw, K, C, rows, Kc, mode, planes);
  FCD_LAUNCH_CHECK("wino_pack");
  return FCD_OK;
}

extern "C" int fcd_conv_wino_pack_blocks(int K, int C, int mode) {
  const int rows = mode == 0 ? K : C, Kc = round_up(mode == 0 ? C : K, 32);
  return (int)std::min<long long>(cdiv64((long long)rows * Kc / 2, 256), 4096);
}
extern "C" int fcd_conv_wino_pack_multi(const long long* items_dev, int n, int total_blocks, double total_elems, void* stream) {
  FCD_CHECK_ARG(items_dev && n > 0 && total_blocks > 0, "fcd_conv_wino_pack_multi: bad arguments");
  FcdProfScope prof(FCD_K_PACK, (hipStream_t)stream, 0.0, 4.0 * total_elems * (9 + 1.5 * 36));
  hipLaunchKernelGGL(wino_filter_multi_kernel, dim3((unsigned)total_blocks), dim3(256), 0, (hipStream_t)stream, items_dev, n);
  FCD_LAUNCH_CHECK("wino_pack_multi");
  return FCD_OK;
}

static int wino_xcd() { return fcd_sw(FCD_SW_CONV_XCD); }

template <int MM, int TRB, int TWB>
static void wino_launch_input_cfg(const WinoInArgs& ia, int src, hipStream_t st) {
  dim3 grid((unsigned)cdiv(ia.TW, TWB), (unsigned)cdiv(ia.TH, TRB), (unsigned)(ia.N * ia.Q));
  const bool vec = (ia.W & 3) == 0 && (src != 2 || (ia.Wp & 1) == 0);
#define WINO_IN(SRC_, VEC_) \
  hipLaunchKernelGGL((wino_input_kernel<MM, SRC_, TRB, TWB, VEC_>), grid, dim3(256), 0, st, ia)
  if (src == 0) { if (vec) WINO_IN(0, true); else WINO_IN(0, false); }
  else if (src == 1) { if (vec) WINO_IN(1, true); else WINO_IN(1, false); }
  else { if (vec) WINO_IN(2, true); else WINO_IN(2, false); }
#undef WINO_IN
}

template <int MM>
static void wino_launch_input(const WinoInArgs& ia, int src, hipStream_t st) {
  constexpr int NT = 64 / MM;
  const int roll = fcd_sw(FCD_SW_WINO_IN_ROLL);
  if ((ia.W & 3) == 0 && (src != 2 || (ia.Wp & 1) == 0) && roll > 1 && ia.TW > NT / 4) {
    const int trb = ia.TW > NT / 2 ? 1 : 2, strips = cdiv(ia.TH, trb);
    if (strips >= 2) {
      const int r = std::min(roll, strips);
      dim3 grid((unsigned)cdiv(ia.TW, NT / trb), (unsigned)cdiv(strips, r), (unsigned)(ia.N * ia.Q));
#define WINO_ROLL(SRC_, TRB_) hipLaunchKernelGGL((wino_input_roll_kernel<MM, SRC_, TRB_, NT / TRB_>), grid, dim3(256), 0, st, ia, r)
      if (src == 0) { if (trb == 1) WINO_ROLL(0, 1); else WINO_ROLL(0, 2); }
      else if (src == 1) { if (trb == 1) WINO_ROLL(1, 1); else WINO_ROLL(1, 2); }
      else if (src == 3) {
        if constexpr (MM == 4) { if (trb == 1) WINO_ROLL(3, 1); else WINO_ROLL(3, 2); }
      }
      else { if (trb == 1) WINO_ROLL(2, 1); else WINO_ROLL(2, 2); }
#undef WINO_ROLL
      return;
    }
  }
  if (src == 3) return;
  if (ia.TW > NT / 2 && (ia.exp & 1)) wino_launch_input_cfg<MM, 1, NT / 2>(ia, src, st);
  else if (ia.TW > NT / 2) wino_launch_input_cfg<MM, 1, NT>(ia, src, st);
  else if (ia.TW > NT / 4) wino_launch_input_cfg<MM, 2, NT / 2>(ia, src, st);
  else wino_launch_input_cfg<MM, 4, NT / 4>(ia, src, st);
}

static bool wino_cat_input_ok(const WinoPlan& pl, int W) {
  if (pl.m != 4 || (W & 3) != 0 || pl.TW <= 4) return false;
  const int trb = pl.TW > 8 ? 1 : 2;
  return cdiv(pl.TH, trb) >= 2;
}

static bool wino_blk_path(const WinoPlan& pl) {
  return fcd_sw(FCD_SW_WINO_CBLK) && pl.m == 4 && pl.rows > 64 && wino_split() && (pl.rows & 3) == 0;
}

struct WinoInSrc {
  const float* src; const float* mask; const unsigned short* mask_bits; const unsigned char* code; int Hp, Wp;
  const WinoCat* cat;
  const float* aff_scale; const float* aff_shift; int aff_ng;
};
static void wino_stage_input(const WinoPlan& pl, int N, int in_ch, int H, int W, const WinoInSrc& in, float* V, hipStream_t st) {
  WinoInArgs ia;
  memset(&ia, 0, sizeof(ia));
  if (in.cat) ia.cat = *in.cat;
  ia.x = in.src; ia.mask = in.mask; ia.mbits = in.mask_bits; ia.code = in.code; ia.V = V;
  ia.N = N; ia.C = in_ch; ia.H = H; ia.W = W; ia.Hp = in.Hp; ia.Wp = in.Wp;
  ia.TH = pl.TH; ia.TW = pl.TW; ia.Q = pl.Q; ia.T = pl.T;
  const int srcmode = in.aff_scale ? 3 : (in.code ? 2 : ((in.mask || in.mask_bits) ? 1 : 0));
  ia.aff_scale = in.aff_scale; ia.aff_shift = in.aff_shift; ia.aff_ng = in.aff_ng > 0 ? in.aff_ng : 1;
  {
    const int exp = fcd_sw(FCD_SW_WINO_IN_EXP);
    ia.exp = exp;
    ia.xcd = (wino_xcd() && !(exp & 8)) ? 1 : 0;
  }
  const double in_elems = (double)N * in_ch * H * W;
  FcdProfScope p1(FCD_K_WINO_XFORM, st, 0.0, 4.0 * in_elems * (srcmode == 1 ? (in.mask_bits ? 1.03125 : 2.0) : 1.0) + (double)pl.v_bytes,
                  fcd_prof_tagf("in src=%d C=%d img=%dx%dx%d", srcmode, in_ch, N, H, W));
  if (pl.m == 2) wino_launch_input<2>(ia, srcmode, st); else wino_launch_input<4>(ia, srcmode, st);
}

static WinoGemmArgs wino_stage_gemm(const WinoPlan& pl, const float* U, const float* V, float* Mb, int N, int H, int W, hipStream_t st) {
  WinoGemmArgs ga;
  memset(&ga, 0, sizeof(ga));
  ga.A = U; ga.B = V; ga.C = Mb;
  ga.M = pl.rows; ga.N = (int)pl.T; ga.Kc = pl.Kc;
  ga.m_tiles = cdiv(pl.rows, 128); ga.n_tiles = cdiv((int)pl.T, 128);
  ga.xcd_remap = wino_xcd();
  ga.a_ld = pl.Kc; ga.a_batch = (long long)pl.rows * pl.Kc;
  ga.as_plane = (long long)pl.A2 * pl.rows * pl.Kc;
  ga.As = (const unsigned short*)(U + ga.as_plane);
  ga.b_ld = 32; ga.b_adv = (long long)pl.T * 32; ga.b_batch = (long long)pl.Q * pl.T * 32;
  ga.stages_per_split = pl.Q;
  if (wino_blk_path(pl)) {
    ga.c_blk = 1; ga.c_mblk = cdiv(pl.rows, 32); ga.c_tblk = (int)((pl.T + 31) / 32);
    ga.c_batch = (long long)ga.c_mblk * ga.c_tblk * 1024;
  }
  const bool split = pl.rows > 64 && wino_split();
  FcdProfScope p2(split ? FCD_K_WINO_GEMM_SPLIT : FCD_K_WINO_GEMM, st, 2.0 * pl.A2 * pl.rows * (double)pl.Kc * (double)pl.T,
                  (double)pl.v_bytes + (double)pl.m_bytes + (split ? 6.0 : 4.0) * pl.A2 * pl.rows * pl.Kc,
                  fcd_prof_tagf("conv M=%d N=%lld Kc=%d batch=%d img=%dx%dx%d", pl.rows, pl.T, pl.Kc, pl.A2, N, H, W));
  wino_gemm_launch(ga, pl.A2, 1, st);
  return ga;
}

struct WinoOutDst {
  const float* bias; int relu; float* y; float* pool_y; unsigned char* code;
  const WinoCat* cat; unsigned short* bits; const unsigned short* gate; double* bn_part; int bn_bpg;
};
static void wino_stage_output(const WinoPlan& pl, const WinoGemmArgs& ga, const float* Mb, int N, int H, int W, const WinoOutDst& o,
                              hipStream_t st) {
  WinoOutArgs oa;
  memset(&oa, 0, sizeof(oa));
  if (o.cat) oa.cat = *o.cat;
  oa.Mb = Mb; oa.bias = o.bias; oa.y = o.y; oa.pool_y = o.pool_y; oa.code = o.code; oa.bits = o.bits; oa.gate = o.gate;
  oa.K = pl.rows; oa.P = H; oa.Q = W; oa.TH = pl.TH; oa.TW = pl.TW; oa.relu = o.relu; oa.T = pl.T;
  dim3 og((unsigned)cdiv64(pl.T, 256), (unsigned)pl.rows);
  const double mm = pl.m * pl.m;
  FcdProfScope p3(FCD_K_WINO_XFORM, st, 0.0,
                  (double)pl.m_bytes + (double)pl.m_bytes / pl.A2 * mm * (o.pool_y ? 0.3125 : 1.0),
                  fcd_prof_tagf("out pool=%d K=%d img=%dx%dx%d", o.pool_y ? 1 : 0, pl.rows, N, H, W));
  if (ga.c_blk) {
    oa.tblk = ga.c_tblk; oa.xs_blk = ga.c_batch;
    const dim3 ogb((unsigned)cdiv64(pl.T, 256), (unsigned)cdiv(pl.rows, 4));
    if (o.bn_part) {
      oa.bn_part = o.bn_part; oa.bn_bpg = o.bn_bpg;
      hipLaunchKernelGGL(wino_output_blk_bn_kernel, ogb, dim3(256), 0, st, oa);
    } else {
      hipLaunchKernelGGL(wino_output_blk_kernel, ogb, dim3(256), 0, st, oa);
    }
  } else if (pl.m == 2) hipLaunchKernelGGL(wino_output_kernel<2>, og, dim3(256), 0, st, oa);
  else hipLaunchKernelGGL(wino_output_kernel<4>, og, dim3(256), 0, st, oa);
}

static int wino_run(const WinoPlan& pl, int N, int in_ch, int H, int W, const float* src, const float* mask,
                    const unsigned char* code_in, int Hp, int Wp, const float* U, const float* bias, int relu, float* y,
                    float* pool_y, unsigned char* code_out, void* ws, hipStream_t st,
                    const WinoCat* in_cat = nullptr, const WinoCat* out_cat = nullptr, float* v_keep = nullptr,
                    const unsigned short* mask_bits = nullptr, unsigned short* relu_bits_out = nullptr,
                    double* bn_part = nullptr, int bn_bpg = 0, const float* aff_scale = nullptr, const float* aff_shift = nullptr,
                    int aff_ng = 0) {
  float* V = v_keep ? v_keep : (float*)ws;
  float* Mb = (float*)((char*)ws + ((pl.v_bytes + 255) & ~(size_t)255));
  const WinoInSrc in = {src, mask, mask_bits, code_in, Hp, Wp, in_cat, aff_scale, aff_shift, aff_ng};
  wino_stage_input(pl, N, in_ch, H, W, in, V, st);
  const WinoGemmArgs ga = wino_stage_gemm(pl, U, V, Mb, N, H, W, st);
  const WinoOutDst out = {bias, relu, y, pool_y, code_out, out_cat, relu_bits_out, nullptr, bn_part, bn_bpg};
  wino_stage_output(pl, ga, Mb, N, H, W, out, st);
  return 0;
}

static double conv_flops(const fcd_conv_desc* d) { return 2.0 * d->N * d->K * (double)d->P * d->Q * d->C * 9; }
static double wino_bytes(const WinoPlan& pl) {
  const double v = (double)pl.v_bytes, m = (double)pl.m_bytes;
  const int a2 = pl.A2, mm = pl.m * pl.m;
  return v / a2 * mm + 2.0 * v + 2.0 * m + m / a2 * mm + 4.0 * a2 * pl.rows * pl.Kc;
}

extern "C" size_t fcd_conv_wino_keepv_bytes(const fcd_conv_desc* d);

extern "C" int fcd_conv2d_fwd_wino_x(const fcd_conv_desc* d, const float* x, const float* U, const float* bias, float* y,
                                     int fuse_relu, float* pool_y, unsigned char* code, void* ws, size_t ws_bytes,
                                     const fcd_wino_fwd_extras* ex, void* stream);
extern "C" int fcd_conv2d_fwd_wino_keepv(const fcd_conv_desc* d, const float* x, const float* U, const float* bias, float* y,
                                         int fuse_relu, float* pool_y, unsigned char* code, void* ws, size_t ws_bytes,
                                         float* v_keep, void* stream);
extern "C" int fcd_conv2d_fwd_wino(const fcd_conv_desc* d, const float* x, const float* U, const float* bias, float* y,
                                   int fuse_relu, float* pool_y, unsigned char* code, void* ws, size_t ws_bytes,
                                   void* stream) {
  return fcd_conv2d_fwd_wino_keepv(d, x, U, bias, y, fuse_relu, pool_y, code, ws, ws_bytes, nullptr, stream);
}
extern "C" int fcd_conv2d_fwd_wino_keepv(const fcd_conv_desc* d, const float* x, const float* U, const float* bias, float* y,
                                         int fuse_relu, float* pool_y, unsigned char* code, void* ws, size_t ws_bytes,
                                         float* v_keep, void* stream) {
  fcd_wino_fwd_extras ex;
  memset(&ex, 0, sizeof(ex));
  ex.v_keep = v_keep;
  return fcd_conv2d_fwd_wino_x(d, x, U, bias, y, fuse_relu, pool_y, code, ws, ws_bytes, &ex, stream);
}

extern "C" int fcd_conv_wino_bn_split(const fcd_conv_desc* d, int groups) {
  WinoPlan pl;
  if (!d || !fcd_sw(FCD_SW_WINO_BNSTATS) || groups < 1 || !wino_plan(d, 0, &pl) || !wino_blk_path(pl) || d->N % groups) return 0;
  const long long per_group = pl.T / groups;
  if (per_group < 256 || per_group % 256) return 0;
  return (int)(per_group / 256);
}
extern "C" size_t fcd_conv_wino_bn_part_bytes(const fcd_conv_desc* d, int groups) {
  return (size_t)fcd_conv_wino_bn_split(d, groups) * groups * d->K * 3 * sizeof(double);
}

extern "C" int fcd_conv_wino_in_affine_ok(const fcd_conv_desc* d) {
  WinoPlan pl;
  if (!d || !fcd_sw(FCD_SW_BN_FUSE) || !wino_plan(d, 0, &pl)) return 0;
  if (fcd_sw(FCD_SW_WINO_IN_ROLL) <= 1) return 0;
  return wino_cat_input_ok(pl, d->W) ? 1 : 0;
}

extern "C" int fcd_conv2d_fwd_wino_x(const fcd_conv_desc* d, const float* x, const float* U, const float* bias, float* y,
                                     int fuse_relu, float* pool_y, unsigned char* code, void* ws, size_t ws_bytes,
                                     const fcd_wino_fwd_extras* ex, void* stream) {
  float* v_keep = ex ? ex->v_keep : nullptr;
  double* bn_part = ex ? ex->bn_part : nullptr;
  const int bn_bpg = bn_part ? fcd_conv_wino_bn_split(d, ex->bn_groups) : 0;
  const float* in_scale = ex ? ex->in_scale : nullptr;
  const float* in_shift = ex ? ex->in_shift : nullptr;
  FCD_CHECK_ARG(d && x && U && (y || (pool_y && code)), "fcd_conv2d_fwd_wino: null pointer");
  FCD_CHECK_ARG(!in_scale || (in_shift && ex->in_groups > 0 && d->N % ex->in_groups == 0 && fcd_conv_wino_in_affine_ok(d)),
                "fcd_conv2d_fwd_wino_x: in_scale needs in_shift, in_groups | N and fcd_conv_wino_in_affine_ok(d)");
  FCD_CHECK_ARG(!bn_part || (bn_bpg > 0 && !pool_y && !fuse_relu), "fcd_conv2d_fwd_wino_x: BatchNorm partial sums not available for this call "
                "(fcd_conv_wino_bn_split(d, groups) == 0, or a fused ReLU / pool in front of the BatchNorm)");
  FCD_CHECK_ARG(!v_keep || fcd_conv_wino_keepv_bytes(d) > 0, "fcd_conv2d_fwd_wino_keepv: fcd_conv_wino_keepv_bytes(d) == 0 for this layer");
  WinoPlan pl;
  FCD_CHECK_ARG(wino_plan(d, 0, &pl), "fcd_conv2d_fwd_wino: layer is not planned for the Winograd path");
  if (!ws || ws_bytes < fcd_conv_wino_ws_bytes(d, 0)) {
    fcd_set_error("fcd_conv2d_fwd_wino: workspace %zu < %zu bytes", ws_bytes, fcd_conv_wino_ws_bytes(d, 0));
    return FCD_ERR_WORKSPACE;
  }
  FcdProfScope prof(FCD_K_WINO_FWD, (hipStream_t)stream, conv_flops(d), wino_bytes(pl), fcd_prof_tag_desc("wino_fwd", d));
  wino_run(pl, d->N, d->C, d->H, d->W, x, nullptr, nullptr, 0, 0, U, bias, (fuse_relu || pool_y) ? 1 : 0,
           pool_y ? nullptr : y, pool_y, code, ws, (hipStream_t)stream, nullptr, nullptr, v_keep, nullptr, nullptr, bn_part, bn_bpg,
           in_scale, in_shift, in_scale ? d->N / ex->in_groups : 0);
  FCD_LAUNCH_CHECK("conv2d_fwd_wino");
  return FCD_OK;
}

extern "C" size_t fcd_conv_wino_relu_bits_bytes(const fcd_conv_desc* d) {
  WinoPlan pf, pd;
  if (!d || !wino_plan(d, 0, &pf) || !wino_plan(d, 1, &pd) || pf.m != 4 || pd.m != 4) return 0;
  return (size_t)d->N * d->K * pf.TH * pf.TW * sizeof(unsigned short);
}

extern "C" int fcd_conv2d_fwd_wino_relu_bits(const fcd_conv_desc* d, const float* x, const float* U, const float* bias, float* y,
                                             unsigned short* relu_bits, void* ws, size_t ws_bytes, void* stream) {
  FCD_CHECK_ARG(d && x && U && y && relu_bits, "fcd_conv2d_fwd_wino_relu_bits: null pointer");
  FCD_CHECK_ARG(fcd_conv_wino_relu_bits_bytes(d) > 0, "fcd_conv2d_fwd_wino_relu_bits: fcd_conv_wino_relu_bits_bytes(d) == 0");
  WinoPlan pl;
  wino_plan(d, 0, &pl);
  if (!ws || ws_bytes < fcd_conv_wino_ws_bytes(d, 0)) {
    fcd_set_error("fcd_conv2d_fwd_wino_relu_bits: workspace %zu < %zu bytes", ws_bytes, fcd_conv_wino_ws_bytes(d, 0));
    return FCD_ERR_WORKSPACE;
  }
  FcdProfScope prof(FCD_K_WINO_FWD, (hipStream_t)stream, conv_flops(d), wino_bytes(pl), fcd_prof_tag_desc("wino_fwd", d));
  wino_run(pl, d->N, d->C, d->H, d->W, x, nullptr, nullptr, 0, 0, U, bias, 1, y, nullptr, nullptr, ws, (hipStream_t)stream,
           nullptr, nullptr, nullptr, nullptr, relu_bits);
  FCD_LAUNCH_CHECK("conv2d_fwd_wino_relu_bits");
  return FCD_OK;
}

extern "C" int fcd_conv2d_bwd_data_wino_bits(const fcd_conv_desc* d, const float* dy, const unsigned short* relu_bits,
                                             const float* U, float* dx, void* ws, size_t ws_bytes, void* stream) {
  FCD_CHECK_ARG(d && dy && relu_bits && U && dx, "fcd_conv2d_bwd_data_wino_bits: null pointer");
  FCD_CHECK_ARG(fcd_conv_wino_relu_bits_bytes(d) > 0, "fcd_conv2d_bwd_data_wino_bits: fcd_conv_wino_relu_bits_bytes(d) == 0");
  WinoPlan pl;
  wino_plan(d, 1, &pl);
  if (!ws || ws_bytes < fcd_conv_wino_ws_bytes(d, 1)) {
    fcd_set_error("fcd_conv2d_bwd_data_wino_bits: workspace %zu < %zu bytes", ws_bytes, fcd_conv_wino_ws_bytes(d, 1));
    return FCD_ERR_WORKSPACE;
  }
  FcdProfScope prof(FCD_K_WINO_DGRAD, (hipStream_t)stream, conv_flops(d), wino_bytes(pl), fcd_prof_tag_desc("wino_dgrad", d));
  wino_run(pl, d->N, d->K, d->P, d->Q, dy, nullptr, nullptr, 0, 0, U, nullptr, 0, dx, nullptr, nullptr, ws, (hipStream_t)stream,
           nullptr, nullptr, nullptr, relu_bits, nullptr);
  FCD_LAUNCH_CHECK("conv2d_bwd_data_wino_bits");
  return FCD_OK;
}

extern "C" int fcd_conv2d_bwd_data_wino(const fcd_conv_desc* d, const float* dy, const float* relu_out,
                                        const unsigned char* pool_code, const float* U, float* dx, void* ws,
                                        size_t ws_bytes, void* stream) {
  FCD_CHECK_ARG(d && dy && U && dx, "fcd_conv2d_bwd_data_wino: null pointer");
  WinoPlan pl;
  FCD_CHECK_ARG(wino_plan(d, 1, &pl), "fcd_conv2d_bwd_data_wino: layer is not planned for the Winograd path");
  if (!ws || ws_bytes < fcd_conv_wino_ws_bytes(d, 1)) {
    fcd_set_error("fcd_conv2d_bwd_data_wino: workspace %zu < %zu bytes", ws_bytes, fcd_conv_wino_ws_bytes(d, 1));
    return FCD_ERR_WORKSPACE;
  }
  FcdProfScope prof(FCD_K_WINO_DGRAD, (hipStream_t)stream, conv_flops(d), wino_bytes(pl), fcd_prof_tag_desc("wino_dgrad", d));
  wino_run(pl, d->N, d->K, d->P, d->Q, dy, pool_code ? nullptr : relu_out, pool_code, d->P / 2, d->Q / 2, U, nullptr, 0,
           dx, nullptr, nullptr, ws, (hipStream_t)stream);
  FCD_LAUNCH_CHECK("conv2d_bwd_data_wino");
  return FCD_OK;
}

static bool wino_chain_plans(const fcd_conv_desc* d, int n, int mode, WinoPlan* pls) {
  if (!d || n < 1 || n > 8) return false;
  for (int i = 0; i < n; ++i) {
    if (!wino_plan(&d[i], mode, &pls[i]) || pls[i].m != 4 || !wino_blk_path(pls[i])) return false;
    if (d[i].N != d[0].N || d[i].H != d[0].H || d[i].W != d[0].W || d[i].P != d[0].H || d[i].Q != d[0].W) return false;
    if (i > 0 && (d[i].C != d[i - 1].K || !wino_oi_ok(d[i].C, d[i].H, d[i].W))) return false;
  }
  return true;
}
extern "C" int fcd_conv_wino_chain_ok(const fcd_conv_desc* d, int n, int mode) {
  WinoPlan pls[8];
  return (mode == 0 || mode == 1) && wino_chain_plans(d, n, mode, pls) ? 1 : 0;
}
extern "C" size_t fcd_conv_wino_chain_bits_bytes(const fcd_conv_desc* d) {
  WinoPlan pf;
  if (!d || !wino_plan(d, 0, &pf) || pf.m != 4) return 0;
  return (size_t)d->N * d->K * pf.TH * pf.TW * sizeof(unsigned short);
}
extern "C" size_t fcd_conv_wino_chain_ws_bytes(const fcd_conv_desc* d, int n, int mode) {
  WinoPlan pls[8];
  if (!(mode == 0 || mode == 1) || !wino_chain_plans(d, n, mode, pls)) return 0;
  size_t v = 0, m = 0;
  for (int i = 0; i < n; ++i) { v = std::max(v, pls[i].v_bytes); m = std::max(m, pls[i].m_bytes); }
  return ((v + 255) & ~(size_t)255) + m + 256;
}

static void wino_stage_oi(const WinoPlan& prod, const WinoGemmArgs& ga, const float* Mb, const WinoPlan& cons, int N, int H, int W,
                          const float* bias, int relu, unsigned short* bits_out, const unsigned short* gate, float* V, hipStream_t st) {
  WinoOiArgs oa;
  memset(&oa, 0, sizeof(oa));
  oa.Mb = Mb; oa.xs_blk = ga.c_batch; oa.tblk = ga.c_tblk;
  oa.bias = bias; oa.relu = relu; oa.bits_out = bits_out; oa.gate = gate; oa.V = V;
  oa.N = N; oa.K = prod.rows; oa.H = H; oa.W = W; oa.TH = cons.TH; oa.TW = cons.TW; oa.Q = cons.Q; oa.T = cons.T;
  FcdProfScope p(FCD_K_WINO_XFORM, st, 0.0, (double)prod.m_bytes + (double)cons.v_bytes + 2.0 * prod.rows * (double)cons.T,
                 fcd_prof_tagf("oi gate=%d K=%d img=%dx%dx%d", gate ? 1 : 0, prod.rows, N, H, W));
  wino_oi_launch(oa, st);
}

extern "C" int fcd_conv2d_fwd_wino_chain(const fcd_conv_desc* d, int n, const float* x, const float* const* U,
                                         const float* const* bias, float* y, float* pool_y, unsigned char* code,
                                         unsigned short* const* relu_bits, void* ws, size_t ws_bytes, void* stream) {
  WinoPlan pls[8];
  FCD_CHECK_ARG(d && x && U && bias && (y || (pool_y && code)), "fcd_conv2d_fwd_wino_chain: null pointer");
  FCD_CHECK_ARG(wino_chain_plans(d, n, 0, pls), "fcd_conv2d_fwd_wino_chain: fcd_conv_wino_chain_ok(d, n, 0) == 0 for this run");
  const size_t need = fcd_conv_wino_chain_ws_bytes(d, n, 0);
  if (!ws || ws_bytes < need) {
    fcd_set_error("fcd_conv2d_fwd_wino_chain: workspace %zu < %zu bytes", ws_bytes, need);
    return FCD_ERR_WORKSPACE;
  }
  size_t vmax = 0;
  for (int i = 0; i < n; ++i) vmax = std::max(vmax, pls[i].v_bytes);
  float* V = (float*)ws;
  float* Mb = (float*)((char*)ws + ((vmax + 255) & ~(size_t)255));
  hipStream_t st = (hipStream_t)stream;
  const int N = d[0].N, H = d[0].H, W = d[0].W;
  WinoGemmArgs ga;
  for (int i = 0; i < n; ++i) {
    FCD_CHECK_ARG(U[i], "fcd_conv2d_fwd_wino_chain: null filter pack");
    const WinoPlan& pl = pls[i];
    const double v = (double)pl.v_bytes, m = (double)pl.m_bytes;
    const double in_b = i == 0 ? 4.0 * N * d[0].C * H * W + v : (double)pls[i - 1].m_bytes + v;
    const double out_b = i == n - 1 ? m + m / pl.A2 * 16.0 * (pool_y ? 0.3125 : 1.0) : 0.0;
    FcdProfScope prof(FCD_K_WINO_FWD, st, conv_flops(&d[i]), in_b + v + m + out_b + 4.0 * pl.A2 * pl.rows * pl.Kc,
                      fcd_prof_tag_desc("wino_fwd_chain", &d[i]));
    if (i == 0) {
      const WinoInSrc in = {x, nullptr, nullptr, nullptr, 0, 0, nullptr};
      wino_stage_input(pl, N, d[0].C, H, W, in, V, st);
    } else {
      wino_stage_oi(pls[i - 1], ga, Mb, pl, N, H, W, bias[i - 1], 1, relu_bits ? relu_bits[i - 1] : nullptr, nullptr, V, st);
    }
    ga = wino_stage_gemm(pl, U[i], V, Mb, N, H, W, st);
    if (i == n - 1) {
      const WinoOutDst out = {bias[i], 1, pool_y ? nullptr : y, pool_y, code, nullptr,
                              (!pool_y && relu_bits) ? relu_bits[i] : nullptr, nullptr, nullptr, 0};
      wino_stage_output(pl, ga, Mb, N, H, W, out, st);
    }
  }
  FCD_LAUNCH_CHECK("conv2d_fwd_wino_chain");
  return FCD_OK;
}

extern "C" int fcd_conv2d_bwd_data_wino_chain(const fcd_conv_desc* d, int n, const float* dy, const unsigned char* pool_code,
                                              const unsigned short* const* relu_bits, const unsigned short* gate_in,
                                              const float* const* U1, float* dx, void* ws, size_t ws_bytes, void* stream) {
  WinoPlan pls[8];
  FCD_CHECK_ARG(d && dy && U1 && dx && (n == 1 || relu_bits), "fcd_conv2d_bwd_data_wino_chain: null pointer");
  FCD_CHECK_ARG(wino_chain_plans(d, n, 1, pls), "fcd_conv2d_bwd_data_wino_chain: fcd_conv_wino_chain_ok(d, n, 1) == 0 for this run");
  const size_t need = fcd_conv_wino_chain_ws_bytes(d, n, 1);
  if (!ws || ws_bytes < need) {
    fcd_set_error("fcd_conv2d_bwd_data_wino_chain: workspace %zu < %zu bytes", ws_bytes, need);
    return FCD_ERR_WORKSPACE;
  }
  size_t vmax = 0;
  for (int i = 0; i < n; ++i) vmax = std::max(vmax, pls[i].v_bytes);
  float* V = (float*)ws;
  float* Mb = (float*)((char*)ws + ((vmax + 255) & ~(size_t)255));
  hipStream_t st = (hipStream_t)stream;
  const int N = d[0].N, H = d[0].H, W = d[0].W;
  WinoGemmArgs ga;
  for (int i = n - 1; i >= 0; --i) {
    FCD_CHECK_ARG(U1[i] && (i == 0 || relu_bits[i - 1]), "fcd_conv2d_bwd_data_wino_chain: null filter pack / sign bits");
    const WinoPlan& pl = pls[i];
    const double v = (double)pl.v_bytes, m = (double)pl.m_bytes;
    const double in_b = i == n - 1 ? 4.0 * N * d[i].K * H * W * (pool_code ? 0.3125 : 1.03125) + v : (double)pls[i + 1].m_bytes + v;
    const double out_b = i == 0 ? m + m / pl.A2 * 16.0 : 0.0;
    FcdProfScope prof(FCD_K_WINO_DGRAD, st, conv_flops(&d[i]), in_b + v + m + out_b + 4.0 * pl.A2 * pl.rows * pl.Kc,
                      fcd_prof_tag_desc("wino_dgrad_chain", &d[i]));
    if (i == n - 1) {
      const WinoInSrc in = {dy, nullptr, pool_code ? nullptr : (relu_bits ? relu_bits[i] : nullptr), pool_code, H / 2, W / 2, nullptr};
      wino_stage_input(pl, N, d[i].K, H, W, in, V, st);
    } else {
      wino_stage_oi(pls[i + 1], ga, Mb, pl, N, H, W, nullptr, 0, nullptr, relu_bits[i], V, st);
    }
    ga = wino_stage_gemm(pl, U1[i], V, Mb, N, H, W, st);
    if (i == 0) {
      const WinoOutDst out = {nullptr, 0, dx, nullptr, nullptr, nullptr, nullptr, gate_in, nullptr, 0};
      wino_stage_output(pl, ga, Mb, N, H, W, out, st);
    }
  }
  FCD_LAUNCH_CHECK("conv2d_bwd_data_wino_chain");
  return FCD_OK;
}

struct WinoWgArgs {
  const float* src;
  const float* mask;
  float* dst;
  float* psum;
  unsigned short* planes;
  WinoCat cat;
  int N, CH, H, W, TH, TW;
  long long T, Tpad;
};

__global__ __launch_bounds__(256) void wino_wg_input_kernel(WinoWgArgs a) {
  constexpr int A = 6;
  const long long t = (long long)blockIdx.x * 256 + threadIdx.x;
  const int c = blockIdx.y;
  if (t >= a.Tpad) return;
  float* vout = a.dst + (size_t)c * a.Tpad + t;
  const size_t xs = (size_t)a.CH * a.Tpad;
  if (t >= a.T) {
#pragma unroll
    for (int i = 0; i < A * A; ++i) vout[(size_t)i * xs] = 0.f;
    return;
  }
  const int tx = (int)(t % a.TW);
  const long long r2 = t / a.TW;
  const int ty = (int)(r2 % a.TH), n = (int)(r2 / a.TH);
  const float* xp = a.src + ((size_t)n * a.CH + c) * a.H * a.W;
  if (a.cat.n > 0) {
    int ch = c, chans;
    const float* base = wino_cat_pick(a.cat, ch, chans);
    xp = base + ((size_t)n * chans + ch) * a.H * a.W;
  }
  const int ih0 = ty * 4 - 1, iw0 = tx * 4 - 1;
  float d[A][A];
#pragma unroll
  for (int i = 0; i < A; ++i) {
    const int ih = ih0 + i;
    const bool rok = ih >= 0 && ih < a.H;
#pragma unroll
    for (int j = 0; j < A; ++j) {
      const int iw = iw0 + j;
      d[i][j] = (rok && iw >= 0 && iw < a.W) ? xp[(size_t)ih * a.W + iw] : 0.f;
    }
  }
  float t1[A][A];
#pragma unroll
  for (int i = 0; i < A; ++i)
#pragma unroll
    for (int j = 0; j < A; ++j) {
      float s = 0.f;
#pragma unroll
      for (int k = 0; k < A; ++k)
        if (WinoMat<4>::BT(i, k) != 0.f) s += WinoMat<4>::BT(i, k) * d[k][j];
      t1[i][j] = s;
    }
#pragma unroll
  for (int i = 0; i < A; ++i)
#pragma unroll
    for (int j = 0; j < A; ++j) {
      float s = 0.f;
#pragma unroll
      for (int k = 0; k < A; ++k)
        if (WinoMat<4>::BT(j, k) != 0.f) s += t1[i][k] * WinoMat<4>::BT(j, k);
      vout[(size_t)(i * A + j) * xs] = s;
    }
}

__global__ __launch_bounds__(256) void wino_wg_dy_kernel(WinoWgArgs a) {
  constexpr int A = 6;
  __shared__ double red[16];
  const int lane = threadIdx.x & 63, wv = threadIdx.x >> 6;
  const int ks = (lane >> 4) & 1, stg = (lane >> 5) + 2 * wv;
  const long long t0 = (long long)blockIdx.x * 256 + stg * 32 + (lane & 15) * 2;
  const int k = min((int)blockIdx.y * 2 + ks, a.CH - 1);
  const bool kok = (int)blockIdx.y * 2 + ks < a.CH;
  float dy[2][4][4];
  float lsum = 0.f;
  const bool vec = (a.W & 3) == 0;
#pragma unroll
  for (int e = 0; e < 2; ++e) {
    const long long t = t0 + e;
#pragma unroll
    for (int i = 0; i < 4; ++i)
#pragma unroll
      for (int j = 0; j < 4; ++j) dy[e][i][j] = 0.f;
    if (t < a.T && kok) {
      const int tx = (int)(t % a.TW);
      const long long r2 = t / a.TW;
      const int ty = (int)(r2 % a.TH), n = (int)(r2 / a.TH);
      const size_t base = ((size_t)n * a.CH + k) * a.H * a.W;
#pragma unroll
      for (int i = 0; i < 4; ++i) {
        const int ih = ty * 4 + i;
        if (ih >= a.H) continue;
        const size_t off = base + (size_t)ih * a.W + tx * 4;
        if (vec) {
          f32x4 v = *(const f32x4*)(a.src + off);
          if (a.mask) {
            const f32x4 m = *(const f32x4*)(a.mask + off);
#pragma unroll
            for (int j = 0; j < 4; ++j) if (!(m[j] > 0.f)) v[j] = 0.f;
          }
#pragma unroll
          for (int j = 0; j < 4; ++j) dy[e][i][j] = v[j];
        } else {
#pragma unroll
          for (int j = 0; j < 4; ++j) {
            if (tx * 4 + j < a.W) {
              float v = a.src[off + j];
              if (a.mask && !(a.mask[off + j] > 0.f)) v = 0.f;
              dy[e][i][j] = v;
            }
          }
        }
      }
#pragma unroll
      for (int i = 0; i < 4; ++i)
#pragma unroll
        for (int j = 0; j < 4; ++j) lsum += dy[e][i][j];
    }
  }
  if (a.psum != nullptr) {
    const double b0 = block_sum_d(ks == 0 ? (double)lsum : 0.0, red);
    const double b1 = block_sum_d(ks == 1 ? (double)lsum : 0.0, red);
    if (threadIdx.x == 0) {
      a.psum[(size_t)blockIdx.x * a.CH + blockIdx.y * 2] = (float)b0;
      if ((int)blockIdx.y * 2 + 1 < a.CH) a.psum[(size_t)blockIdx.x * a.CH + blockIdx.y * 2 + 1] = (float)b1;
    }
  }
  if (t0 >= a.Tpad || !kok) return;
  float* wout = a.dst + (size_t)k * a.Tpad + t0;
  const size_t xs = (size_t)a.CH * a.Tpad;
  unsigned short* pout = a.planes ? a.planes + ((size_t)(t0 >> 5) * a.CH + k) * 32 + (t0 & 31) : nullptr;
  const size_t ps = 36 * xs;
  float t1[2][A][4];
#pragma unroll
  for (int e = 0; e < 2; ++e)
#pragma unroll
    for (int q = 0; q < A; ++q)
#pragma unroll
      for (int j = 0; j < 4; ++j) {
        float s = 0.f;
#pragma unroll
        for (int i = 0; i < 4; ++i)
          if (WinoMat<4>::AT(i, q) != 0.f) s += WinoMat<4>::AT(i, q) * dy[e][i][j];
        t1[e][q][j] = s;
      }
#pragma unroll
  for (int q = 0; q < A; ++q)
#pragma unroll
    for (int p2 = 0; p2 < A; ++p2) {
      float sv[2];
#pragma unroll
      for (int e = 0; e < 2; ++e) {
        float s = 0.f;
#pragma unroll
        for (int j = 0; j < 4; ++j)
          if (WinoMat<4>::AT(j, p2) != 0.f) s += t1[e][q][j] * WinoMat<4>::AT(j, p2);
        sv[e] = s;
      }
      const size_t o = (size_t)(q * A + p2) * xs;
      if (pout) {
        unsigned h[2], m[2], l[2];
#pragma unroll
        for (int e = 0; e < 2; ++e) {
          h[e] = bf16_rn_bits(sv[e]);
          const float r = sv[e] - __uint_as_float(h[e] << 16);
          m[e] = bf16_rn_bits(r);
          l[e] = bf16_rn_bits(r - __uint_as_float(m[e] << 16));
        }
        *(unsigned*)(pout + o) = h[0] | (h[1] << 16);
        *(unsigned*)(pout + ps + o) = m[0] | (m[1] << 16);
        *(unsigned*)(pout + 2 * ps + o) = l[0] | (l[1] << 16);
      } else {
        *(float2*)(wout + o) = make_float2(sv[0], sv[1]);
      }
    }
}

__global__ __launch_bounds__(256) void wino_wg_final_kernel(const float* __restrict__ dU, float* __restrict__ dw, int K,
                                                            int C, int splits) {
  constexpr int A = 6;
  __shared__ float st9[256 * 9];
  const long long total = (long long)K * C;
  const long long i0 = (long long)blockIdx.x * 256;
  const long long i = i0 + threadIdx.x;
  if (i < total) {
    const size_t xs = (size_t)K * C, ss = 36 * xs;
    float u[A][A];
#pragma unroll
    for (int q = 0; q < A * A; ++q) {
      float s = 0.f;
      for (int sp = 0; sp < splits; ++sp) s += dU[(size_t)sp * ss + (size_t)q * xs + i];
      u[q / A][q % A] = s;
    }
    float t1[3][A];
#pragma unroll
    for (int r = 0; r < 3; ++r)
#pragma unroll
      for (int p2 = 0; p2 < A; ++p2) {
        float s = 0.f;
#pragma unroll
        for (int q = 0; q < A; ++q)
          if (WinoMat<4>::G(q, r) != 0.f) s += WinoMat<4>::G(q, r) * u[q][p2];
        t1[r][p2] = s;
      }
#pragma unroll
    for (int r = 0; r < 3; ++r)
#pragma unroll
      for (int s3 = 0; s3 < 3; ++s3) {
        float s = 0.f;
#pragma unroll
        for (int p2 = 0; p2 < A; ++p2)
          if (WinoMat<4>::G(p2, s3) != 0.f) s += t1[r][p2] * WinoMat<4>::G(p2, s3);
        st9[threadIdx.x * 9 + r * 3 + s3] = s;
      }
  }
  __syncthreads();
  const long long nout = (total - i0 < 256 ? total - i0 : 256) * 9;
  for (int j = threadIdx.x; j < nout; j += 256) dw[i0 * 9 + j] = st9[j];
}

__global__ __launch_bounds__(256) void wino_wg_splitsum_kernel(float* __restrict__ dU, long long n4, long long ss4, int splits) {
  const long long i = (long long)blockIdx.x * 256 + threadIdx.x;
  if (i >= n4) return;
  float4* p = (float4*)dU;
  float4 s = p[i];
  for (int sp = 1; sp < splits; ++sp) {
    const float4 v = p[(size_t)sp * ss4 + i];
    s.x += v.x; s.y += v.y; s.z += v.z; s.w += v.w;
  }
  p[i] = s;
}

__global__ __launch_bounds__(256) void wino_psum_fin_kernel(const float* __restrict__ psum, float* __restrict__ out, int C,
                                                            int nblk) {
  __shared__ double red[16];
  const int c = blockIdx.x;
  double s = 0.0;
  for (int b = threadIdx.x; b < nblk; b += 256) s += (double)psum[(size_t)b * C + c];
  s = block_sum_d(s, red);
  if (threadIdx.x == 0) out[c] = (float)s;
}

struct WinoWgPlan {
  int TH, TW, splits, sps, stages;
  long long T, Tpad;
  size_t w_bytes, v_bytes, du_bytes, psum_bytes;
};

int fcd_wino_wgrad_plan(const fcd_conv_desc* d, WinoWgPlan* pl) {
  if (wino_env() != 4) return 0;
  if (!(d->R == 3 && d->S == 3 && d->stride == 1 && d->pad == 1)) return 0;
  const int min_k = fcd_sw(FCD_SW_WINO_WG_MINK), min_c = fcd_sw(FCD_SW_WINO_WG_MINC);
  if (d->K < min_k || d->C < min_c || d->P < 4 || d->Q < 4) return 0;
  pl->TH = cdiv(d->H, 4);
  pl->TW = cdiv(d->W, 4);
  pl->T = (long long)d->N * pl->TH * pl->TW;
  pl->Tpad = (pl->T + 31) / 32 * 32;
  pl->stages = (int)(pl->Tpad / 32);
  const int blocks = cdiv(d->K, 128) * cdiv(d->C, 128) * 36;
  const int wg_wgs = fcd_sw(FCD_SW_WINO_WG_WGS);
  int splits;
  if (wg_wgs > 0) {
    splits = cdiv(wg_wgs, blocks);
  } else {
    const int tiles = blocks / 36;
    long best = -1;
    splits = 1;
    for (int s = 1; s <= 64 && s <= pl->stages; ++s) {
      const int sps = cdiv(pl->stages, s), s2 = cdiv(pl->stages, sps);
      if (s2 != s) continue;
      const long rounds = cdiv(blocks * s, 512);
      const long cost = rounds * (sps + 5) * 10 + 3L * tiles * (s - 1);
      if (best < 0 || cost < best) { best = cost; splits = s; }
    }
  }
  if (splits > pl->stages) splits = pl->stages;
  if (splits > 64) splits = 64;
  if (splits < 1) splits = 1;
  pl->sps = cdiv(pl->stages, splits);
  pl->splits = cdiv(pl->stages, pl->sps);
  pl->w_bytes = (size_t)36 * d->K * pl->Tpad * 6;
  pl->v_bytes = (size_t)36 * d->C * pl->Tpad * sizeof(float);
  pl->du_bytes = (size_t)pl->splits * 36 * d->K * d->C * sizeof(float);
  pl->psum_bytes = (size_t)cdiv64(pl->Tpad, 256) * d->K * sizeof(float);
  return 4;
}

size_t fcd_wino_wgrad_ws_bytes(const fcd_conv_desc* d) {
  WinoWgPlan pl;
  if (!fcd_wino_wgrad_plan(d, &pl)) return 0;
  return pl.w_bytes + pl.v_bytes + pl.du_bytes + pl.psum_bytes + 1024;
}

static int wino_wgrad_run_impl(const fcd_conv_desc* d, const float* x, const WinoCat* xcat, const float* dy,
                               const float* relu_out, float* dw, float* db, void* ws, hipStream_t st, const float* v_fwd = nullptr);
int fcd_wino_wgrad_run(const fcd_conv_desc* d, const float* x, const float* dy, const float* relu_out, float* dw,
                       float* db, void* ws, hipStream_t st) {
  return wino_wgrad_run_impl(d, x, nullptr, dy, relu_out, dw, db, ws, st);
// ... 205 lines not shown
```

fcd_gan_pytorch_amd/csrc/conv_wino_chain.hip:

```cpp
#include "conv_wino.h"

template <int BW, int TRS, int VW, int NT, int MINB>
__global__ __launch_bounds__(NT, MINB) void wino_oi_kernel(WinoOiArgs a) {
  constexpr int A = 6, CHB = 32;
  constexpr int RR = 4 * TRS + 5;
  constexpr int CW = 4 * BW + 2;
  constexpr int PL = (RR * CW) | 1;
  constexpr int JT = VW == 4 ? BW + 2 : BW;
  constexpr int GP = 4 / VW;
  constexpr int QD = CHB / 4;
  static_assert(TRS * JT * QD * GP <= NT, "output phase: one item per thread");
  typedef float mvec __attribute__((ext_vector_type(VW)));
  __shared__ float ring[CHB * PL];
  const int tid = threadIdx.x;
  const int tx0 = blockIdx.x * BW;
  const int kb = blockIdx.y * CHB;
  const int n = blockIdx.z;

  for (int i = tid; i < CHB * RR; i += NT) {
    const int c = i / RR, r = i % RR;
    ring[c * PL + r * CW] = 0.f;
    ring[c * PL + r * CW + CW - 1] = 0.f;
  }
  for (int i = tid; i < CHB * CW; i += NT) ring[(i / CW) * PL + 3 * CW + i % CW] = 0.f;

  const int og = tid % GP, oj = (tid / GP) % JT - (VW == 4 ? 1 : 0), orest = tid / (GP * JT);
  const int otr = orest % TRS, ocq = orest / TRS;
  const int otx = tx0 + oj;
  const bool o_on = ocq < QD && otx >= 0 && otx < a.TW;
  const int k0 = kb + 4 * ocq + VW * og;
  const int cl0 = 4 * ocq + VW * og;
  mvec m4[A * A];
  unsigned gw[VW];
  auto issue = [&](int s) {
    const int ty = s * TRS + otr;
    if (!o_on || ty >= a.TH) return;
    const long long t = ((long long)n * a.TH + ty) * a.TW + otx;
    const float* mp = a.Mb + ((size_t)(k0 >> 5) * a.tblk + (size_t)(t >> 5)) * 1024 +
                      ((((k0 >> 2) & 1) * 4 + ((k0 >> 3) & 3)) * 32 + (int)(t & 31)) * 4 + (k0 & 3);
#pragma unroll
    for (int q = 0; q < A * A; ++q) m4[q] = __builtin_nontemporal_load((const mvec*)(mp + (size_t)q * a.xs_blk));
    if (a.gate) {
#pragma unroll
      for (int e = 0; e < VW; ++e) gw[e] = a.gate[(((size_t)n * a.K + k0 + e) * a.TH + ty) * a.TW + otx];
    }
  };
  auto out_phase = [&](int s) {
    const int ty = s * TRS + otr;
    if (ty == a.TH && ocq < QD) {
#pragma unroll
      for (int e = 0; e < VW; ++e) {
        float* rp = ring + (cl0 + e) * PL + ((4 * ty + 4) % RR) * CW;
        if (oj < 0) rp[0] = 0.f;
        else if (oj >= BW) rp[CW - 1] = 0.f;
        else {
#pragma unroll
          for (int j = 0; j < 4; ++j) rp[1 + 4 * oj + j] = 0.f;
        }
      }
    }
    if (!o_on || ty >= a.TH) return;
    int rrow[4];
#pragma unroll
    for (int i = 0; i < 4; ++i) rrow[i] = ((4 * ty + 4 + i) % RR) * CW;
#pragma unroll
    for (int e = 0; e < VW; ++e) {
      float mv[A][A];
#pragma unroll
      for (int q = 0; q < A * A; ++q) mv[q / A][q % A] = m4[q][e];
      float o[4][4];
      wino_out_tile<4>(mv, a.bias ? a.bias[k0 + e] : 0.f, a.relu, o);
      if (a.gate) {
#pragma unroll
        for (int i = 0; i < 4; ++i)
#pragma unroll
          for (int j = 0; j < 4; ++j) o[i][j] = ((gw[e] >> (4 * i + j)) & 1u) ? o[i][j] : 0.f;
      }
      float* rp = ring + (cl0 + e) * PL;
      if (oj >= 0 && oj < BW) {
        if (a.bits_out) {
          unsigned w = 0;
#pragma unroll
          for (int i = 0; i < 4; ++i)
#pragma unroll
            for (int j = 0; j < 4; ++j) w |= (o[i][j] > 0.f ? 1u : 0u) << (4 * i + j);
          a.bits_out[(((size_t)n * a.K + k0 + e) * a.TH + ty) * a.TW + otx] = (unsigned short)w;
        }
#pragma unroll
        for (int i = 0; i < 4; ++i)
#pragma unroll
          for (int j = 0; j < 4; ++j) rp[rrow[i] + 1 + 4 * oj + j] = o[i][j];
      } else if (oj < 0) {
#pragma unroll
        for (int i = 0; i < 4; ++i) rp[rrow[i]] = o[i][3];
      } else {
#pragma unroll
        for (int i = 0; i < 4; ++i) rp[rrow[i] + CW - 1] = o[i][0];
      }
    }
  };

  const size_t xi_stride = (size_t)a.Q * a.T * 32;
  const int steps = a.TH / TRS + 1;
  issue(0);
#pragma unroll 1
  for (int s = 0; s < steps; ++s) {
    out_phase(s);
    if (s + 1 < steps) issue(s + 1);
    __syncthreads();
#pragma unroll 1
    for (int it = tid; it < TRS * BW * CHB; it += NT) {
      const int c = it % CHB, tl = it / CHB;
      const int tc = tl % BW, r = s * TRS - 1 + tl / BW;
      if (r < 0 || r >= a.TH || tx0 + tc >= a.TW) continue;
      const float* rc = ring + c * PL + 4 * tc;
      float d[A][A];
#pragma unroll
      for (int i = 0; i < A; ++i) {
        const int ro = ((4 * r + 3 + i) % RR) * CW;
#pragma unroll
        for (int j = 0; j < A; ++j) d[i][j] = rc[ro + j];
      }
      float t1[A][A];
      wino_in_rows<4>(d, t1);
      const size_t t = ((size_t)n * a.TH + r) * a.TW + tx0 + tc;
      const int kg = kb + c;
      float* vout = a.V + ((size_t)(kg >> 5) * a.T + t) * 32 + (kg & 31);
#pragma unroll
      for (int i = 0; i < A; ++i)
#pragma unroll
        for (int j = 0; j < A; ++j) vout[(size_t)(i * A + j) * xi_stride] = wino_in_col<4>(t1, i, j);
    }
    __syncthreads();
  }
}

int wino_oi_ok(int K, int H, int W) {
  if (!fcd_sw(FCD_SW_WINO_CHAIN) || (K & 31) || (H & 3) || (W & 3)) return 0;
  const int TW = W / 4, TH = H / 4;
  if (TW >= 16) return (TW % 16) == 0;
  if (TW == 8) return (TH % 2) == 0;
  if (TW == 4) return (TH % 4) == 0;
  return 0;
}

void wino_oi_launch(const WinoOiArgs& a, hipStream_t st) {
  const dim3 grid((unsigned)cdiv(a.TW, a.TW >= 16 ? 16 : a.TW), (unsigned)(a.K / 32), (unsigned)a.N);
  if (a.TW == 32) hipLaunchKernelGGL((wino_oi_kernel<32, 1, 2, 512, 1>), dim3(1, (unsigned)(a.K / 32), (unsigned)a.N), dim3(512), 0, st, a);
  else if (a.TW > 16) hipLaunchKernelGGL((wino_oi_kernel<16, 1, 4, 256, 2>), grid, dim3(256), 0, st, a);
  else if (a.TW == 16) hipLaunchKernelGGL((wino_oi_kernel<16, 1, 2, 256, 2>), grid, dim3(256), 0, st, a);
  else if (a.TW == 8) hipLaunchKernelGGL((wino_oi_kernel<8, 2, 2, 256, 2>), grid, dim3(256), 0, st, a);
  else hipLaunchKernelGGL((wino_oi_kernel<4, 4, 2, 256, 2>), grid, dim3(256), 0, st, a);
}
```

fcd_gan_pytorch_amd/csrc/switches.h:

```cpp
#pragma once

#define FCD_SWITCH_TABLE(X)                                                                                                        \
                                                                                                             \
  X(WINO, 4, "Winograd tile size of the planned 3x3 layers: 4 = F(4x4,3x3), 2 = F(2x2,3x3), 0 = direct kernels only (also fcd_conv_wino_set)") \
  X(WINO_MINC, 64, "F(4x4) plan: least reduction channels")                                                                         \
  X(WINO_MINROWS, 128, "F(4x4) plan: least GEMM rows")                                                                              \
  X(WINO_WG_MINK, 128, "F(4x4) weight-gradient plan: least filters")                                                                \
  X(WINO_WG_MINC, 128, "F(4x4) weight-gradient plan: least channels")                                                               \
  X(WINO_WG_WGS, 0, "F(4x4) weight gradient: reduction splits = ceil(n / blocks) (round-4 rule, n = 1024); 0 = the round model")    \
  X(WINO2, 1, "fused F(2x2,3x3) kernel for the 64-row 3x3 layers (0: those layers on the direct kernels)")                          \
  X(WINO2_MINC, 32, "fused F(2x2): least reduction channels")                                                                       \
  X(WINO2_WAVES, 8, "fused F(2x2): 8 = one 8x32 workgroup per CU, 4 = two 4x32 workgroups, 1 = one wave per SIMD")                   \
  X(WINO2_KS, 2, "fused F(2x2): channels per LDS stage / 4 (1, 2 or 3)")                                                            \
                                                                                                              \
  X(WINO_SPLIT, 1, "F(4x4) GEMMs on the bf16 matrix pipe with exact three-way operand splitting (0: v_mfma_f32_32x32x2_f32; also fcd_conv_wino_split_set)") \
  X(WINO_SPLIT_BIG, 1, "split GEMM tile policy: 0 = 128x128 only, 1 = 256x256 where it fills the chip, 2 = 256x256 for every GEMM with >= 256 rows") \
  X(WINO_TILE, 0, "fp32-pipe GEMM tile: 0 = 128x128, 1 = 256x128, 2 = 256x256")                                                    \
  X(WINO_XB, 0, "transform positions chained per GEMM workgroup (0: chosen per launch)")                                            \
  X(WINO_XCD2, 128, "largest tile count per transform-position group whose tiles all go to one XCD (0: never)")                     \
  X(WINO_RES, 1, "filter-resident split GEMM for one-row-tile layers with a short reduction")                                       \
  X(WINO_RES_WGS, 256, "workgroups in flight of the filter-resident GEMM")                                                          \
  X(WINO_CBLK, 1, "GEMM result in 32x32 MFMA-native blocks (0: row-major M)")                                                       \
                                                                                                        \
  X(WINO_IN_ROLL, 4, "strips per block of the rolling input transform (1: one-strip kernel)")                                       \
  X(WINO_IN_EXP, 0, "input-transform launch experiments (bit 3: no XCD-aware order)")                                               \
  X(WINO_BNSTATS, 1, "BatchNorm statistics out of the F(4x4) output transform")                                                     \
  X(WINO_KEEPV, 1, "weight gradient reuses the forward pass's transformed input (0: re-transforms x)")                              \
  X(WINO_CHAIN, 1, "frozen VGG runs through the fused output->input transform (0: layer by layer)")                                 \
  X(WINO_RELU_BITS, 1, "frozen F(4x4) layers keep 16 sign bits per tile as the ReLU mask (0: fp32 y on the tape)")                  \
  X(BN_FUSE, 1, "train-mode BatchNorm + ReLU inside the next convolution's loader / the density head (0: kernels of their own)")    \
  X(PAIR_CAT, 1, "first decoder convolution reads skip pair + upsampled tensor in place (0: materialise the concatenation)")        \
                                                                                                       \
  X(CONV_XCD, 1, "XCD-aware workgroup -> tile order")                                                                               \
  X(CONV_BIG, 1, "128x256 direct tiles")                                                                                            \
  X(CONV_THINFWD, 1, "thin-channel forward kernel for <= 4 input channels")                                                         \
  X(CONV_ROWS16, 1, "16-row MFMA tiles for <= 16-filter 9x9 layers")                                                                \
  X(CONV_HEAD, 1, "one-filter 1x1 head kernels (0: generic 1x1 path + ATen sigmoid)")                                               \
  X(S2_SUBPIXEL, 1, "stride-2 data gradient as four sub-pixel convolutions (0: zero-dilated)")                                      \
  X(S2_GLDS, 1, "its LDS-DMA kernel (0: register-staged kernel for every layer)")                                                   \
  X(THIN_MFMA, 32, "rows per workgroup of the matrix-core data gradient of the one-band first VGG layer (0: VALU kernel)")          \
                                                                                                   \
  X(WGRAD_WGS, 512, "workgroups the reduction split of the direct weight gradient aims at")                                         \
  X(WGRAD_TKC, 1, "split partials in (tap, filter, channel) order (0: dW's own layout)")                                            \
  X(WGRAD_ROLL, 1, "rolling 4-row ring kernel for 3x3 stride-1 layers")                                                             \
  X(WGRAD_NCHW, 1, "3x3 weight gradient reads x and dY as they lie (0: channel-minor copies first)")                                \
  X(WGRAD_SPLIT, 1, "that kernel on the bf16 matrix pipe, operands split exactly in three (0: fp32 pipe, stride 1 only; also fcd_conv_wgrad_split_set)") \
  X(WGRAD_THIN, 1, "first-layer weight-gradient kernel (<= 4 channels)")                                                            \
  X(WGRAD_THIN9, 1, "9x9 weight-gradient kernel with <= 4 channels on one side")                                                    \
                                                                                             \
  X(BN_POOL, 1, "encoder tails: BatchNorm + ReLU + max-pool + skip-gradient sum as one node (0: separate kernels)")                 \
  X(UPSAMPLE_ROWS, 1, "row-walking kernel for the adjoint of the x2 upsampling")                                                    \
  X(NO_POOLFUSE, 0, "1: ReLU + max-pool behind a frozen convolution as kernels of their own")                                       \
                                                  \
  X(PACK_MULTI, 1, "all F(4x4) filter packs of an optimizer re-packed by one launch after its step")                                \
  X(FUSED_GLUE, 1, "masked stacks / perception-tap MSE as fused kernels (0: ATen compositions)")                                    \
  X(D_SHARE, 1, "Demo_RSSS Discriminator step: the shared masked x through D's net once (0: twice, as the reference)")              \
  X(D_POOL, 0, "Discriminator pooled pair difference: 0 = fused kernel, 1 = ATen (f_x - f_y).mean(), 2 = mean first (round 3)")     \
  X(LAUNCH_WINDOW, 384, "host: launches the issuing thread may be ahead of the device before it sleeps (0: run ahead until the hardware queue is full and spin there)") \
  X(STEP_OVERLAP, 0, "experimental: the Discriminator step of the adversarial loops on a second HIP stream")                        \
  X(DP_FORCE_EXCHANGE, 0, "one-rank process groups run every data-parallel collective")

enum {
#define FCD_SW_ENUM(NAME, DEF, HELP) FCD_SW_##NAME,
  FCD_SWITCH_TABLE(FCD_SW_ENUM)
#undef FCD_SW_ENUM
      FCD_SW_COUNT
};

extern int g_fcd_switch[FCD_SW_COUNT];
static inline int fcd_sw(int id) { return g_fcd_switch[id]; }
```

include/fcdgan_hip.h:

```cpp
#ifndef FCDGAN_HIP_H
#define FCDGAN_HIP_H

#include <stddef.h>
#include <stdint.h>

#ifdef __cplusplus
extern "C" {
#endif

typedef enum fcd_status {
  FCD_OK = 0,
  FCD_ERR_INVALID = -1,
  FCD_ERR_LAUNCH = -2,
  FCD_ERR_WORKSPACE = -3
} fcd_status;

enum { FCD_ACT_NONE = 0, FCD_ACT_RELU = 1, FCD_ACT_LEAKY = 2, FCD_ACT_PRELU = 3 };

int fcd_version(void);
const char* fcd_build_hash(void);
const char* fcd_last_error_string(void);

int fcd_switch_count(void);
const char* fcd_switch_name(int i);
const char* fcd_switch_help(int i);
int fcd_switch_default(int i);
int fcd_switch_get(const char* name);
int fcd_switch_set(const char* name, int value);

typedef struct fcd_conv_desc {
  int32_t N, C, H, W;
  int32_t K, R, S;
  int32_t stride, pad;
  int32_t P, Q;
} fcd_conv_desc;

int64_t fcd_conv_packed_elems(int K, int C, int R, int S, int mode);
int fcd_conv_pack_weights(const float* w, float* wp, int K, int C, int R, int S, int mode, void* stream);

int fcd_conv2d_fwd(const fcd_conv_desc* d, const float* x, const float* wp, const float* bias,
                   float* y, int fuse_relu, void* stream);
int fcd_conv2d_fwd_ex(const fcd_conv_desc* d, const float* x, const float* wp, const float* bias,
                      float* y, int act, const float* slope_ptr, float slope_imm,
                      const float* residual, void* stream);
size_t fcd_conv2d_relu_bits_bytes(const fcd_conv_desc* d);
int fcd_conv2d_fwd_relu_bits(const fcd_conv_desc* d, const float* x, const float* wp, const float* bias,
                             float* y, unsigned char* bits, void* stream);
int fcd_conv2d_bwd_data_bits(const fcd_conv_desc* d, const float* dy, const unsigned char* bits,
                             const float* wp_bwd, float* dx, void* stream);
int fcd_conv1x1_head_plan(int N, int C, int HW, int K);
int fcd_conv1x1_head_fwd(const float* x, const float* w, const float* bias, float* y, int N, int C, int HW,
                         int sigmoid, void* stream);
size_t fcd_conv1x1_head_bwd_ws_bytes(int N, int C);
int fcd_conv1x1_head_bwd(const float* x, const float* w, const float* dy, const float* y_sig, float* dx, float* dw,
                         float* db, int N, int C, int HW, void* ws, size_t ws_bytes, void* stream);
int fcd_conv1x1_head_bn_fwd(const float* z, const float* scale, const float* shift, int groups, const float* w, const float* bias,
                            float* y, int N, int C, int HW, int sigmoid, void* stream);
size_t fcd_conv1x1_head_bn_bwd_ws_bytes(int N, int C, int groups);
int fcd_conv1x1_head_bn_bwd(const float* z, const float* w, const float* dy, const float* y_sig, const float* scale,
                            const float* shift, const float* mean, const float* invstd, int groups, float* dz, float* dw, float* db,
                            float* dgamma, float* dbeta, int N, int C, int HW, void* ws, size_t ws_bytes, void* stream);
int fcd_conv_wino_plan(const fcd_conv_desc* d, int mode);
int fcd_conv_wino_set(int m);
int fcd_conv_wino_split_set(int on);
int fcd_conv_wgrad_split_set(int on);
size_t fcd_conv_wino_ws_bytes(const fcd_conv_desc* d, int mode);
int64_t fcd_conv_wino_filter_elems(int K, int C, int mode, int m);
int fcd_conv_wino_pack(const float* w, float* U, int K, int C, int mode, int m, void* stream);
int fcd_conv_wino_pack_blocks(int K, int C, int mode);
int fcd_conv_wino_pack_multi(const long long* items_dev, int n, int total_blocks, double total_elems, void* stream);
int fcd_conv2d_fwd_wino(const fcd_conv_desc* d, const float* x, const float* U, const float* bias, float* y,
                        int fuse_relu, float* pool_y, unsigned char* code, void* ws, size_t ws_bytes,
                        void* stream);
int fcd_conv_wino_cat_ok(const fcd_conv_desc* d);
int fcd_conv2d_fwd_wino_cat(const fcd_conv_desc* d, const float* const* src, const int* chans, int nsrc, const float* U,
                            const float* bias, float* y, int fuse_relu, void* ws, size_t ws_bytes, void* stream);
int fcd_conv2d_bwd_data_wino_cat(const fcd_conv_desc* d, const float* dy, const float* relu_out, const float* U,
                                 float* const* dsrc, const int* chans, int nsrc, void* ws, size_t ws_bytes, void* stream);
int fcd_conv2d_bwd_weight_bias_cat(const fcd_conv_desc* d, const float* const* src, const int* chans, int nsrc,
                                   const float* dy, const float* relu_out, float* dw, float* db, void* ws, size_t ws_bytes,
                                   void* stream);
typedef struct fcd_wino_fwd_extras {
  float* v_keep;
  double* bn_part;
  int32_t bn_groups;
  int32_t in_groups;
  const float* in_scale;
  const float* in_shift;
} fcd_wino_fwd_extras;
int fcd_conv_wino_in_affine_ok(const fcd_conv_desc* d);
int fcd_conv_wino_bn_split(const fcd_conv_desc* d, int groups);
size_t fcd_conv_wino_bn_part_bytes(const fcd_conv_desc* d, int groups);
int fcd_conv2d_fwd_wino_x(const fcd_conv_desc* d, const float* x, const float* U, const float* bias, float* y, int fuse_relu,
                          float* pool_y, unsigned char* code, void* ws, size_t ws_bytes, const fcd_wino_fwd_extras* ex,
                          void* stream);
int fcd_conv2d_fwd_wino_cat_x(const fcd_conv_desc* d, const float* const* src, const int* chans, int nsrc, const float* U,
                              const float* bias, float* y, int fuse_relu, void* ws, size_t ws_bytes,
                              const fcd_wino_fwd_extras* ex, void* stream);
size_t fcd_conv_wino_keepv_bytes(const fcd_conv_desc* d);
int fcd_conv2d_fwd_wino_keepv(const fcd_conv_desc* d, const float* x, const float* U, const float* bias, float* y,
                              int fuse_relu, float* pool_y, unsigned char* code, void* ws, size_t ws_bytes, float* v_keep,
                              void* stream);
int fcd_conv2d_fwd_wino_cat_keepv(const fcd_conv_desc* d, const float* const* src, const int* chans, int nsrc, const float* U,
                                  const float* bias, float* y, int fuse_relu, void* ws, size_t ws_bytes, float* v_keep,
                                  void* stream);
int fcd_conv2d_bwd_weight_bias_v(const fcd_conv_desc* d, const float* v_fwd, const float* dy, const float* relu_out, float* dw,
                                 float* db, void* ws, size_t ws_bytes, void* stream);
size_t fcd_conv_wino_relu_bits_bytes(const fcd_conv_desc* d);
int fcd_conv2d_fwd_wino_relu_bits(const fcd_conv_desc* d, const float* x, const float* U, const float* bias, float* y,
                                  unsigned short* relu_bits, void* ws, size_t ws_bytes, void* stream);
int fcd_conv2d_bwd_data_wino_bits(const fcd_conv_desc* d, const float* dy, const unsigned short* relu_bits, const float* U,
                                  float* dx, void* ws, size_t ws_bytes, void* stream);
int fcd_conv_wino_chain_ok(const fcd_conv_desc* d, int n, int mode);
size_t fcd_conv_wino_chain_ws_bytes(const fcd_conv_desc* d, int n, int mode);
size_t fcd_conv_wino_chain_bits_bytes(const fcd_conv_desc* d);
int fcd_conv2d_fwd_wino_chain(const fcd_conv_desc* d, int n, const float* x, const float* const* U, const float* const* bias,
                              float* y, float* pool_y, unsigned char* code, unsigned short* const* relu_bits, void* ws,
                              size_t ws_bytes, void* stream);
int fcd_conv2d_bwd_data_wino_chain(const fcd_conv_desc* d, int n, const float* dy, const unsigned char* pool_code,
                                   const unsigned short* const* relu_bits, const unsigned short* gate_in,
                                   const float* const* U1, float* dx, void* ws, size_t ws_bytes, void* stream);
int fcd_conv2d_bwd_data_wino(const fcd_conv_desc* d, const float* dy, const float* relu_out,
                             const unsigned char* pool_code, const float* U, float* dx, void* ws,
                             size_t ws_bytes, void* stream);
int fcd_conv2d_bwd_data(const fcd_conv_desc* d, const float* dy, const float* relu_out,
                        const float* wp_bwd, float* dx, void* stream);
int fcd_conv2d_fwd_relu_pool(const fcd_conv_desc* d, const float* x, const float* wp,
                             const float* bias, float* y_pool, unsigned char* code, void* stream);
int fcd_conv2d_bwd_data_pooled(const fcd_conv_desc* d, const float* dy_pool,
                               const unsigned char* code, const float* wp_bwd, float* dx,
                               void* stream);
size_t fcd_conv2d_bwd_weight_ws_bytes(const fcd_conv_desc* d);
int fcd_conv2d_bwd_weight(const fcd_conv_desc* d, const float* x, const float* dy,
                          const float* relu_out, float* dw, void* ws, size_t ws_bytes, void* stream);
int fcd_conv2d_bwd_weight_bias(const fcd_conv_desc* d, const float* x, const float* dy,
                               const float* relu_out, float* dw, float* db, void* ws, size_t ws_bytes,
                               void* stream);
size_t fcd_channel_sum_ws_bytes(int C);
int fcd_channel_sum(const float* x, const float* relu_out, float* out, int N, int C, int HW,
                    void* ws, size_t ws_bytes, void* stream);

int fcd_bn_act_fwd(const float* x, float* y, int N, int C, int HW, int groups, int has_bn,
                   const float* gamma, const float* beta, float* running_mean, float* running_var,
                   float momentum, float eps, int training, float* save_mean, float* save_invstd,
                   int act, const float* slope, float slope_imm, void* ws, size_t ws_bytes,
                   void* stream);
int fcd_bn_act_fwd_replay(const float* x, float* y, int N, int C, int HW, int groups, const int* order, int norder,
                          const float* gamma, const float* beta, float* running_mean, float* running_var,
                          float momentum, float eps, float* save_mean, float* save_invstd, int act,
                          const float* slope, float slope_imm, void* ws, size_t ws_bytes, void* stream);

size_t fcd_bn_act_ws_bytes(int C, int groups);
int fcd_bn_act_bwd(const float* dz, const float* x, float* dx, int N, int C, int HW, int groups,
                   int has_bn, const float* gamma, const float* beta, const float* running_mean,
                   const float* running_var, float eps, int training, const float* save_mean,
                   const float* save_invstd, int act, const float* slope, float slope_imm,
                   float* dgamma, float* dbeta, float* dslope, void* ws, size_t ws_bytes,
                   void* stream);

int fcd_bn_partial_stats(const float* x, double* out, int N, int C, int HW, int groups, void* ws,
                         size_t ws_bytes, void* stream);
int fcd_bn_act_fwd_from_stats(const float* x, float* y, int N, int C, int HW, int groups,
                              const double* sums, double count, const float* gamma,
                              const float* beta, float* running_mean, float* running_var,
                              float momentum, float eps, float* save_mean, float* save_invstd,
                              int act, const float* slope, float slope_imm, void* ws,
                              size_t ws_bytes, void* stream);
int fcd_bn_act_fwd_parts(const float* x, float* y, int N, int C, int HW, int groups, const double* part, int split,
                         const float* gamma, const float* beta, float* running_mean, float* running_var, float momentum,
                         float eps, float* save_mean, float* save_invstd, int act, const float* slope, float slope_imm,
                         void* ws, size_t ws_bytes, void* stream);
int fcd_bn_train_stats(const float* x, int N, int C, int HW, int groups, const double* part, int split, const float* gamma,
                       const float* beta, float* running_mean, float* running_var, float momentum, float eps, float* save_mean,
                       float* save_invstd, float* scale, float* shift, void* ws, size_t ws_bytes, void* stream);
int fcd_bn_relu_pool_plan(int N, int C, int H, int W, int groups);
int fcd_bn_relu_pool_fwd(const float* z, float* a, float* p, int N, int C, int H, int W, int groups, const float* scale,
                         const float* shift, void* stream);
int fcd_bn_relu_pool_bwd(const float* z, const float* dskip, const float* dpool, float* dz, int N, int C, int H, int W, int groups,
                         const float* gamma, const float* beta, const float* save_mean, const float* save_invstd, float* dgamma,
                         float* dbeta, void* ws, size_t ws_bytes, void* stream);
int fcd_bn_bwd_partial(const float* dz, const float* x, double* out, int N, int C, int HW,
                       int groups, const float* gamma, const float* beta, const float* save_mean,
                       const float* save_invstd, int act, const float* slope, float slope_imm,
                       void* ws, size_t ws_bytes, void* stream);
int fcd_bn_bwd_from_sums(const float* dz, const float* x, float* dx, int N, int C, int HW,
                         int groups, const double* sums, double count, const float* gamma,
                         const float* beta, const float* save_mean, const float* save_invstd,
                         int act, const float* slope, float slope_imm, void* ws, size_t ws_bytes,
                         void* stream);

int fcd_maxpool2_fwd(const float* x, float* y, int NC, int H, int W, void* stream);
int fcd_maxpool2_bwd(const float* x, const float* dy, float* dx, int NC, int H, int W, void* stream);
int fcd_maxpool2_bwd_add(const float* x, const float* dy, const float* add, float* dx, int NC, int H, int W, void* stream);
int fcd_upsample2x_fwd(const float* x, float* y, int NC, int H, int W, void* stream);
int fcd_upsample2x_bwd(const float* dy, float* dx, int NC, int H, int W, void* stream);
int fcd_avgpool2_pad_fwd(const float* x, float* y, int NC, int H, int W, void* stream);
int fcd_avgpool2_pad_bwd(const float* dy, float* dx, int NC, int H, int W, void* stream);
int fcd_pair_gap_diff_fwd(const float* f, float* d, int pairs, int n, int C, int HW, void* stream);
int fcd_pair_gap_diff_bwd(const float* g, float* df, int pairs, int n, int C, int HW, void* stream);
int fcd_masked_stack_fwd(const float* s0, const float* s1, const float* s2, const float* s3, int k, const float* cmask, float* z,
                         int N, int C, int HW, void* stream);
int fcd_masked_stack_bwd(const float* dz, const float* s0, const float* s1, const float* s2, const float* s3, int k,
                         const float* cmask, float* dcmask, float* d0, float* d1, float* d2, float* d3, int N, int C, int HW,
                         void* stream);

int fcd_normalize_tiles(const float* x, const float* valid, const double* mean, const double* stdv, float* out,
                        int N, int C, int HW, void* stream);

size_t fcd_masked_recon_ws_bytes(int N);
int fcd_masked_recon_fwd(const float* a, const float* b, const float* m, float* out2, int N, int C,
                         int HW, int kind, int complement, void* ws, size_t ws_bytes, void* stream);
int fcd_masked_recon_bwd(const float* a, const float* b, const float* m, const float* coef,
                         const float* cw, float* da, float* db, float* dm, int N, int C, int HW,
                         int kind, int complement, void* stream);
int fcd_ratio_mean_fwd(const float* out2, int N, float scale, int skip_zero, float* loss, void* stream);
int fcd_ratio_mean_bwd(const float* g, const float* out2, int N, float scale, int skip_zero, float* coef, float* cw, void* stream);

int fcd_ssim_level_fwd(const float* X, const float* Y, const float* win, int win_size, float* out,
                       int NC, int H, int W, float C1, float C2, void* ws, size_t ws_bytes,
                       void* stream);
size_t fcd_ssim_ws_bytes(int NC, int H, int W);
int fcd_ssim_level_bwd(const float* X, const float* Y, const float* win, int win_size,
                       const float* g_ssim, const float* g_cs, float* dX, float* dY, int NC, int H,
                       int W, float C1, float C2, void* ws, size_t ws_bytes, void* stream);

int fcd_conv_s2_dgrad_plan(const fcd_conv_desc* d);
int64_t fcd_conv_s2_dgrad_packed_elems(int K, int C);
int fcd_conv_s2_dgrad_pack(const float* w, float* wp, int K, int C, void* stream);
int fcd_conv2d_bwd_data_s2(const fcd_conv_desc* d, const float* dy, const float* relu_out, const float* wp_s2, float* dx,
                           void* stream);

int fcd_conv_wino2_plan(const fcd_conv_desc* d, int mode);
int64_t fcd_conv_wino2_filter_elems(int K, int C, int mode);
int fcd_conv_wino2_pack(const float* w, float* U, int K, int C, int mode, void* stream);
int fcd_conv2d_fwd_wino2(const fcd_conv_desc* d, const float* x, const float* U, const float* bias, float* y, int act,
                         const float* slope_ptr, float slope_imm, const float* residual, float* pool_y,
                         unsigned char* code, void* stream);
int fcd_conv2d_bwd_data_wino2(const fcd_conv_desc* d, const float* dy, const float* relu_out,
                              const unsigned char* pool_code, const float* U, float* dx, void* stream);

int fcd_adam_step(float* p, const float* g, float* m, float* v, int64_t n, float lr, float beta1,
                  float beta2, float eps, float weight_decay, int step, float grad_scale,
                  void* stream);
int fcd_rmsprop_step(float* p, const float* g, float* sq, int64_t n, float lr, float alpha,
                     float eps, float weight_decay, float grad_scale, void* stream);
int fcd_adam_step_h(float* p, const float* g, float* m, float* v, int64_t n, const float* hyper, float beta1,
                    float beta2, float eps, float weight_decay, float grad_scale, void* stream);
int fcd_rmsprop_step_h(float* p, const float* g, float* sq, int64_t n, const float* hyper, float alpha,
                       float eps, float weight_decay, float grad_scale, void* stream);

void fcd_prof_enable(int on);
int64_t fcd_prof_detail_read(char* buf, int64_t cap, int reset);
int fcd_prof_families(void);
int fcd_prof_read(double* out, int reset);
const char* fcd_prof_family_name(int f);

#ifdef __cplusplus
}
#endif
#endif
```

Measured before the change: 99.31.

## Fuse frozen VGG Winograd chains across untapped max-pools in forward and backward

Extends the frozen VGG perceptual-loss path so consecutive conv blocks separated by an untapped max-pool run as one fused Winograd chain. New output-to-input transform kernels do the pooling, or the un-pooling in backward, inside the transform, so pooled activations are never written to and re-read from memory. The feature loop also stops after the last tapped layer, which skips VGG layers whose outputs are never used. This adds complex new kernels with tie-handling logic for pool argmax, plus a switch to disable the path.

New measurement: 100.3, median of 6. About the same (+1.0%).

```diff
diff --git a/fcd_gan_pytorch_amd/Loss.py b/fcd_gan_pytorch_amd/Loss.py
--- a/fcd_gan_pytorch_amd/Loss.py
+++ b/fcd_gan_pytorch_amd/Loss.py
@@ -93,11 +93,23 @@
     def _features(self, z, single_band=False):
         taps = {}
         layers = list(self.net)
+        last_tap = max(self.feature_layer_list)
         i = 0
-        while i < len(layers):
+        while i <= last_tap:
             layer = layers[i]
             run = self._frozen_run(layers, i) if isinstance(layer, nn.Conv2d) and i > 0 else None
-            if run is not None and ops.frozen_chain_ok(z, [c.weight for c in run[0]]):
+            chains = run is not None and ops.frozen_chain_ok(z, [c.weight for c in run[0]])
+            runs = self._extend_run(layers, run, z) if chains else []
+            if len(runs) > 1:
+                pend = ops.FrozenRun(z)
+                for convs, pool, _ in runs:
+                    pend = ops.frozen_conv_chain(pend, [c.weight for c in convs], [c.bias for c in convs], pool=pool)
+                z = pend.run()
+                i = runs[-1][2]
+                if i - 1 in self.feature_layer_list:
+                    taps[i - 1] = z
+                continue
+            if chains:
                 convs, pool, nxt = run
                 z = ops.frozen_conv_chain(z, [c.weight for c in convs], [c.bias for c in convs], pool=pool)
                 last = nxt - 1
@@ -125,6 +137,16 @@
             i += 1
         return taps
 
+    def _extend_run(self, layers, run, z):
+        runs = [run]
+        while runs[-1][1]:
+            k = runs[-1][2]
+            more = self._frozen_run(layers, k) if k < len(layers) and isinstance(layers[k], nn.Conv2d) else None
+            if more is None or not ops.frozen_run_ok(z, [[c.weight for c in r[0]] for r in runs + [more]], pool_last=more[1]):
+                break
+            runs.append(more)
+        return runs
+
     def _frozen_run(self, layers, i):
         convs, k = [], i
         while (k + 1 < len(layers) and isinstance(layers[k], nn.Conv2d) and isinstance(layers[k + 1], nn.ReLU)
diff --git a/fcd_gan_pytorch_amd/_lib.py b/fcd_gan_pytorch_amd/_lib.py
--- a/fcd_gan_pytorch_amd/_lib.py
+++ b/fcd_gan_pytorch_amd/_lib.py
@@ -90,6 +90,11 @@
     'fcd_conv_wino_chain_bits_bytes': (c_size_t, [POINTER(ConvDesc)]),
     'fcd_conv2d_fwd_wino_chain': (c_int, [P, c_int, P, P, P, P, P, P, P, P, c_size_t, P]),
     'fcd_conv2d_bwd_data_wino_chain': (c_int, [P, c_int, P, P, P, P, P, P, P, c_size_t, P]),
+    'fcd_conv_wino_chain_pool_ok': (c_int, [P, c_int, P, c_int]),
+    'fcd_conv_wino_chain_pool_ws_bytes': (c_size_t, [P, c_int, P, c_int]),
+    'fcd_conv_wino_chain_pool_bwd_fused': (c_int, [P, c_int, P, c_int]),
+    'fcd_conv2d_fwd_wino_chain_pool': (c_int, [P, c_int, P, P, P, P, P, P, P, P, P, c_size_t, P]),
+    'fcd_conv2d_bwd_data_wino_chain_pool': (c_int, [P, c_int, P, P, P, P, P, P, P, P, c_size_t, P]),
     'fcd_conv2d_fwd_wino_keepv': (c_int, [POINTER(ConvDesc), P, P, P, P, c_int, P, P, P, c_size_t, P, P]),
     'fcd_conv2d_fwd_wino_cat_keepv': (c_int, [P, P, P, c_int, P, P, P, c_int, P, c_size_t, P, P]),
     'fcd_conv2d_bwd_weight_bias_v': (c_int, [POINTER(ConvDesc), P, P, P, P, P, P, c_size_t, P]),
diff --git a/fcd_gan_pytorch_amd/_ops.py b/fcd_gan_pytorch_amd/_ops.py
--- a/fcd_gan_pytorch_amd/_ops.py
+++ b/fcd_gan_pytorch_amd/_ops.py
@@ -604,7 +604,149 @@
 
 
 def frozen_conv_chain(x, weights, biases, pool=False):
+    if isinstance(x, FrozenRun):
+        return x.append(weights, biases, pool)
     return _FrozenChain.apply(x, bool(pool), *weights, *biases)
+
+
+_RUN_MAX_LAYERS = 16
+
+
+def _run_descs(xshape, blocks, pool_last):
+    N, C, H, W = xshape
+    descs, pools = [], []
+    for bi, ws in enumerate(blocks):
+        for w in ws:
+            descs.append(_desc((N, C, H, W), w.shape, 1, 1))
+            pools.append(0)
+            C = w.shape[0]
+        if bi + 1 < len(blocks):
+            pools[-1] = 1
+            H, W = H // 2, W // 2
+    if pool_last:
+        pools[-1] = 1
+    return descs, pools
+
+
+def _int_array(vals):
+    return (ctypes.c_int * len(vals))(*vals)
+
+
+def _run_bwd_start(descs, pools):
+    n = len(descs)
+    for j in (0, 1):
+        if j == 1 and (n < 2 or pools[0]):
+            break
+        if lib.fcd_conv_wino_chain_pool_ok(_desc_array(descs[j:]), n - j, _int_array(pools[j:]), 1):
+            return j
+    return n
+
+
+def frozen_run_ok(x, blocks, pool_last=False):
+    if not switch('WINO_CHAIN') or not switch('WINO_CHAIN_POOL') or len(blocks) < 2 or not x.is_cuda or x.dim() != 4:
+        return False
+    if any(len(b) < 1 for b in blocks) or sum(len(b) for b in blocks) > _RUN_MAX_LAYERS:
+        return False
+    if any(w.requires_grad or tuple(w.shape[2:]) != (3, 3) for b in blocks for w in b):
+        return False
+    descs, pools = _run_descs(x.shape, blocks, pool_last)
+    if not lib.fcd_conv_wino_chain_pool_ok(_desc_array(descs), len(descs), _int_array(pools), 0):
+        return False
+    return _run_bwd_start(descs, pools) <= 1
+
+
+class _FrozenRun(torch.autograd.Function):
+
+    @staticmethod
+    def forward(ctx, x, sizes, pool_last, *wb):
+        x = _dev(x, 'conv input')
+        n = len(wb) // 2
+        weights, biases = list(wb[:n]), [_dev(b, 'conv bias') for b in wb[n:]]
+        blocks, at = [], 0
+        for s in sizes:
+            blocks.append(weights[at:at + s])
+            at += s
+        descs, pools = _run_descs(x.shape, blocks, pool_last)
+        darr, parr = _desc_array(descs), _int_array(pools)
+        dev = x.device
+        want = ctx.needs_input_grad[0]
+        last = descs[-1]
+        bits, codes = [None] * n, [None] * n
+        for i in range(n):
+            if pools[i]:
+                codes[i] = torch.empty((last.N, descs[i].K, descs[i].H // 2, descs[i].W // 2), dtype=torch.uint8, device=dev)
+            elif want:
+                bits[i] = torch.empty(lib.fcd_conv_wino_chain_bits_bytes(ctypes.byref(descs[i])) // 2, dtype=torch.int16, device=dev)
+        y = yp = None
+        if pool_last:
+            yp = torch.empty((last.N, last.K, last.H // 2, last.W // 2), dtype=torch.float32, device=dev)
+        else:
+            y = torch.empty((last.N, last.K, last.H, last.W), dtype=torch.float32, device=dev)
+        Us = [wino_weight(w, 0, 4) for w in weights]
+        ws = _ws(lib.fcd_conv_wino_chain_pool_ws_bytes(darr, n, parr, 0), dev)
+        ptrs = lambda ts: _ptr_list([t.data_ptr() if t is not None else None for t in ts])
+        check(lib.fcd_conv2d_fwd_wino_chain_pool(darr, n, parr, _p(x), ptrs(Us), ptrs(biases), _p(y), _p(yp), ptrs(codes),
+                                                 ptrs(bits), _p(ws), ws.numel(), _stream()), 'fcd_conv2d_fwd_wino_chain_pool')
+        ctx.save_for_backward(*weights, *[t for t in bits + codes if t is not None])
+        ctx.geom = (tuple(x.shape), tuple(sizes), bool(pool_last), [t is not None for t in bits])
+        return yp if pool_last else y
+
+    @staticmethod
+    def backward(ctx, dy):
+        xshape, sizes, pool_last, has_bits = ctx.geom
+        n = sum(sizes)
+        saved = list(ctx.saved_tensors)
+        weights, rest = saved[:n], saved[n:]
+        dy = _dev(dy, 'conv grad')
+        if not ctx.needs_input_grad[0]:
+            return (None,) * (3 + 2 * n)
+        blocks, at = [], 0
+        for s in sizes:
+            blocks.append(weights[at:at + s])
+            at += s
+        descs, pools = _run_descs(xshape, blocks, pool_last)
+        bits = [rest.pop(0) if has_bits[i] else None for i in range(n)]
+        codes = [rest.pop(0) if pools[i] else None for i in range(n)]
+        j = _run_bwd_start(descs, pools)
+        if j > 1:
+            raise _lib.FcdError('frozen_conv_run: no backward run for these layers (frozen_run_ok was not consulted)')
+        dev = dy.device
+        dx = torch.empty((xshape[0], descs[j].C, descs[j].H, descs[j].W), dtype=torch.float32, device=dev)
+        darr, parr, m = _desc_array(descs[j:]), _int_array(pools[j:]), n - j
+        ws = _ws(lib.fcd_conv_wino_chain_pool_ws_bytes(darr, m, parr, 1), dev)
+        U1 = [wino_weight(w, 1, 4) for w in weights[j:]]
+        ptrs = lambda ts: _ptr_list([t.data_ptr() if t is not None else None for t in ts])
+        check(lib.fcd_conv2d_bwd_data_wino_chain_pool(darr, m, parr, _p(dy), ptrs(codes[j:]), ptrs(bits[j:]),
+                                                      _p(bits[0]) if j == 1 else None, ptrs(U1), _p(dx), _p(ws), ws.numel(),
+                                                      _stream()), 'fcd_conv2d_bwd_data_wino_chain_pool')
+        if j == 1:
+            dx0 = torch.empty(xshape, dtype=torch.float32, device=dev)
+            _bwd_data_conv(descs[0], dx, weights[0], dx0)
+            dx = dx0
+        return (dx, None, None) + (None,) * (2 * n)
+
+
+def frozen_conv_run(x, blocks, bias_blocks, pool_last=False):
+    weights = [w for b in blocks for w in b]
+    biases = [b for bb in bias_blocks for b in bb]
+    return _FrozenRun.apply(x, tuple(len(b) for b in blocks), bool(pool_last), *weights, *biases)
+
+
+class FrozenRun:
+
+    def __init__(self, x):
+        self.x, self.blocks, self.biases, self.pool_last = x, [], [], False
+
+    def append(self, weights, biases, pool):
+        if self.blocks and not self.pool_last:
+            raise _lib.FcdError('FrozenRun: a block can only follow a pooled block')
+        self.blocks.append(list(weights))
+        self.biases.append(list(biases))
+        self.pool_last = bool(pool)
+        return self
+
+    def run(self):
+        return frozen_conv_run(self.x, self.blocks, self.biases, self.pool_last)
 
 
 class _ConvT2x2(torch.autograd.Function):
diff --git a/fcd_gan_pytorch_amd/csrc/conv_wino.h b/fcd_gan_pytorch_amd/csrc/conv_wino.h
--- a/fcd_gan_pytorch_amd/csrc/conv_wino.h
+++ b/fcd_gan_pytorch_amd/csrc/conv_wino.h
@@ -159,9 +159,15 @@
   float* V;
   int N, K, H, W, TH, TW, Q;
   long long T;
+  unsigned char* code;
+  int pTH, pTW;
 };
 int wino_oi_ok(int K, int H, int W);
 void wino_oi_launch(const WinoOiArgs& a, hipStream_t st);
+int wino_oi_pool_ok(int K, int H, int W);
+void wino_oi_pool_launch(const WinoOiArgs& a, hipStream_t st);
+int wino_oi_unpool_ok(int K, int H, int W);
+void wino_oi_unpool_launch(const WinoOiArgs& a, hipStream_t st);
 
 struct WinoPlan {
   int m, A2, rows, red, Kc, Q, TH, TW;
@@ -209,6 +215,18 @@
       o[i][j] = s;
     }
 }
+__device__ __forceinline__ float wino_pool_window4(float c0, float c1, float c2, float c3, float tie_floor, unsigned& code) {
+#pragma clang fp contract(off)
+  const float m = fmaxf(fmaxf(c0, c1), fmaxf(c2, c3));
+  const float tie = __builtin_fmaf(fmaxf(fmaxf(fabsf(c0), fabsf(c1)), fmaxf(fabsf(c2), fabsf(c3))), 3e-5f, tie_floor);
+  const float mx = m - tie;
+  unsigned arg = 3;
+  if (c2 >= mx) arg = 2;
+  if (c1 >= mx) arg = 1;
+  if (c0 >= mx) arg = 0;
+  code = arg | (m > 0.f ? 4u : 0u);
+  return m;
+}
 template <int MM>
 __device__ __forceinline__ void wino_in_rows(const float (&d)[WinoMat<MM>::A][WinoMat<MM>::A],
                                              float (&t1)[WinoMat<MM>::A][WinoMat<MM>::A]) {
diff --git a/fcd_gan_pytorch_amd/csrc/conv_wino.hip b/fcd_gan_pytorch_amd/csrc/conv_wino.hip
--- a/fcd_gan_pytorch_amd/csrc/conv_wino.hip
+++ b/fcd_gan_pytorch_amd/csrc/conv_wino.hip
@@ -1297,6 +1297,13 @@
         if (pp >= Pp || qq >= Qp) continue;
         const float c0 = o[2 * wi][2 * wj], c1 = o[2 * wi][2 * wj + 1], c2 = o[2 * wi + 1][2 * wj],
                     c3 = o[2 * wi + 1][2 * wj + 1];
+        const size_t oo = (((size_t)n * a.K + k) * Pp + pp) * Qp + qq;
+        if (MM == 4) {
+          unsigned cd;
+          a.pool_y[oo] = wino_pool_window4(c0, c1, c2, c3, tie_floor, cd);
+          a.code[oo] = (unsigned char)cd;
+          continue;
+        }
         const float m = fmaxf(fmaxf(c0, c1), fmaxf(c2, c3));
         const float tie = (MM == 4 ? 3e-5f : 2e-6f) * fmaxf(fmaxf(fabsf(c0), fabsf(c1)), fmaxf(fabsf(c2), fabsf(c3))) + tie_floor;
         const float mx = m - tie;
@@ -1304,7 +1311,6 @@
         if (c2 >= mx) arg = 2;
         if (c1 >= mx) arg = 1;
         if (c0 >= mx) arg = 0;
-        const size_t oo = (((size_t)n * a.K + k) * Pp + pp) * Qp + qq;
         a.pool_y[oo] = m;
         a.code[oo] = (unsigned char)(arg | (m > 0.f ? 4 : 0));
       }
@@ -1896,6 +1902,169 @@
     }
   }
   FCD_LAUNCH_CHECK("conv2d_bwd_data_wino_chain");
+  return FCD_OK;
+}
+
+#define FCD_CHAIN_MAXN 16
+static bool wino_chainp_plans(const fcd_conv_desc* d, int n, const int* pool, int mode, WinoPlan* pls) {
+  if (!d || !pool || n < 1 || n > FCD_CHAIN_MAXN) return false;
+  for (int i = 0; i < n; ++i) {
+    if (!wino_plan(&d[i], mode, &pls[i]) || pls[i].m != 4 || !wino_blk_path(pls[i])) return false;
+    if (d[i].N != d[0].N || d[i].P != d[i].H || d[i].Q != d[i].W) return false;
+    if (i == 0) continue;
+    if (d[i].C != d[i - 1].K) return false;
+    if (pool[i - 1]) {
+      if (2 * d[i].H != d[i - 1].H || 2 * d[i].W != d[i - 1].W) return false;
+      if (mode == 0 ? !wino_oi_pool_ok(d[i].C, d[i - 1].H, d[i - 1].W) : !fcd_sw(FCD_SW_WINO_CHAIN_POOL)) return false;
+    } else {
+      if (d[i].H != d[i - 1].H || d[i].W != d[i - 1].W || !wino_oi_ok(d[i].C, d[i].H, d[i].W)) return false;
+    }
+  }
+  return true;
+}
+extern "C" int fcd_conv_wino_chain_pool_ok(const fcd_conv_desc* d, int n, const int* pool, int mode) {
+  WinoPlan pls[FCD_CHAIN_MAXN];
+  return (mode == 0 || mode == 1) && wino_chainp_plans(d, n, pool, mode, pls) ? 1 : 0;
+}
+static size_t wino_chainp_tmp_bytes(const fcd_conv_desc* d, int n, const int* pool, int mode) {
+  size_t t = 0;
+  if (mode == 1)
+    for (int i = 0; i + 1 < n; ++i)
+      if (pool[i] && !wino_oi_unpool_ok(d[i].K, d[i].H, d[i].W))
+        t = std::max(t, (size_t)d[i].N * d[i].K * d[i + 1].H * d[i + 1].W * sizeof(float));
+  return (t + 255) & ~(size_t)255;
+}
+extern "C" size_t fcd_conv_wino_chain_pool_ws_bytes(const fcd_conv_desc* d, int n, const int* pool, int mode) {
+  WinoPlan pls[FCD_CHAIN_MAXN];
+  if (!(mode == 0 || mode == 1) || !wino_chainp_plans(d, n, pool, mode, pls)) return 0;
+  size_t v = 0, m = 0;
+  for (int i = 0; i < n; ++i) { v = std::max(v, pls[i].v_bytes); m = std::max(m, pls[i].m_bytes); }
+  return ((v + 255) & ~(size_t)255) + ((m + 255) & ~(size_t)255) + wino_chainp_tmp_bytes(d, n, pool, mode) + 256;
+}
+extern "C" int fcd_conv_wino_chain_pool_bwd_fused(const fcd_conv_desc* d, int n, const int* pool, int i) {
+  WinoPlan pls[FCD_CHAIN_MAXN];
+  if (i < 0 || i + 1 >= n || !wino_chainp_plans(d, n, pool, 1, pls) || !pool[i]) return 0;
+  return wino_oi_unpool_ok(d[i].K, d[i].H, d[i].W);
+}
+
+static void wino_stage_oi_pool(const WinoPlan& prod, const WinoGemmArgs& ga, const float* Mb, const WinoPlan& cons, int N, int H, int W,
+                               const float* bias, unsigned char* code, int unpool, float* V, hipStream_t st) {
+  WinoOiArgs oa;
+  memset(&oa, 0, sizeof(oa));
+  oa.Mb = Mb; oa.xs_blk = ga.c_batch; oa.tblk = ga.c_tblk;
+  oa.bias = bias; oa.relu = unpool ? 0 : 1; oa.code = code; oa.V = V;
+  oa.N = N; oa.K = prod.rows; oa.H = H; oa.W = W; oa.TH = cons.TH; oa.TW = cons.TW; oa.Q = cons.Q; oa.T = cons.T;
+  oa.pTH = prod.TH; oa.pTW = prod.TW;
+  FcdProfScope p(FCD_K_WINO_XFORM, st, 0.0, (double)prod.m_bytes + (double)cons.v_bytes + (double)prod.rows * N * H * W / (unpool ? 4 : 1),
+                 fcd_prof_tagf("oi %s K=%d img=%dx%dx%d", unpool ? "unpool" : "pool", prod.rows, N, H, W));
+  if (unpool) wino_oi_unpool_launch(oa, st); else wino_oi_pool_launch(oa, st);
+}
+
+extern "C" int fcd_conv2d_fwd_wino_chain_pool(const fcd_conv_desc* d, int n, const int* pool, const float* x, const float* const* U,
+                                              const float* const* bias, float* y, float* pool_y, unsigned char* const* codes,
+                                              unsigned short* const* relu_bits, void* ws, size_t ws_bytes, void* stream) {
+  WinoPlan pls[FCD_CHAIN_MAXN];
+  FCD_CHECK_ARG(d && pool && x && U && bias && codes, "fcd_conv2d_fwd_wino_chain_pool: null pointer");
+  FCD_CHECK_ARG(wino_chainp_plans(d, n, pool, 0, pls), "fcd_conv2d_fwd_wino_chain_pool: fcd_conv_wino_chain_pool_ok(d, n, pool, 0) == 0 for this run");
+  FCD_CHECK_ARG(pool[n - 1] ? (pool_y && codes[n - 1]) : (y != nullptr), "fcd_conv2d_fwd_wino_chain_pool: null output");
+  const size_t need = fcd_conv_wino_chain_pool_ws_bytes(d, n, pool, 0);
+  if (!ws || ws_bytes < need) {
+    fcd_set_error("fcd_conv2d_fwd_wino_chain_pool: workspace %zu < %zu bytes", ws_bytes, need);
+    return FCD_ERR_WORKSPACE;
+  }
+  size_t vmax = 0;
+  for (int i = 0; i < n; ++i) {
+    vmax = std::max(vmax, pls[i].v_bytes);
+    FCD_CHECK_ARG(U[i] && (i == n - 1 || !pool[i] || codes[i]), "fcd_conv2d_fwd_wino_chain_pool: null filter pack / code buffer");
+  }
+  float* V = (float*)ws;
+  float* Mb = (float*)((char*)ws + ((vmax + 255) & ~(size_t)255));
+  hipStream_t st = (hipStream_t)stream;
+  const int N = d[0].N;
+  WinoGemmArgs ga;
+  for (int i = 0; i < n; ++i) {
+    const WinoPlan& pl = pls[i];
+    const int H = d[i].H, W = d[i].W;
+    const bool last_pool = i == n - 1 && pool[i];
+    const double v = (double)pl.v_bytes, m = (double)pl.m_bytes;
+    const double in_b = i == 0 ? 4.0 * N * d[0].C * H * W + v : (double)pls[i - 1].m_bytes + v;
+    const double out_b = i == n - 1 ? m + m / pl.A2 * 16.0 * (last_pool ? 0.3125 : 1.0) : 0.0;
+    FcdProfScope prof(FCD_K_WINO_FWD, st, conv_flops(&d[i]), in_b + v + m + out_b + 4.0 * pl.A2 * pl.rows * pl.Kc,
+                      fcd_prof_tag_desc("wino_fwd_chain", &d[i]));
+    if (i == 0) {
+      const WinoInSrc in = {x, nullptr, nullptr, nullptr, 0, 0, nullptr};
+      wino_stage_input(pl, N, d[0].C, H, W, in, V, st);
+    } else if (pool[i - 1]) {
+      wino_stage_oi_pool(pls[i - 1], ga, Mb, pl, N, H, W, bias[i - 1], codes[i - 1], 0, V, st);
+    } else {
+      wino_stage_oi(pls[i - 1], ga, Mb, pl, N, H, W, bias[i - 1], 1, relu_bits ? relu_bits[i - 1] : nullptr, nullptr, V, st);
+    }
+    ga = wino_stage_gemm(pl, U[i], V, Mb, N, H, W, st);
+    if (i == n - 1) {
+      const WinoOutDst out = {bias[i], 1, last_pool ? nullptr : y, last_pool ? pool_y : nullptr, last_pool ? codes[i] : nullptr, nullptr,
+                              (!last_pool && relu_bits) ? relu_bits[i] : nullptr, nullptr, nullptr, 0};
+      wino_stage_output(pl, ga, Mb, N, H, W, out, st);
+    }
+  }
+  FCD_LAUNCH_CHECK("conv2d_fwd_wino_chain_pool");
+  return FCD_OK;
+}
+
+extern "C" int fcd_conv2d_bwd_data_wino_chain_pool(const fcd_conv_desc* d, int n, const int* pool, const float* dy,
+                                                   const unsigned char* const* codes, const unsigned short* const* relu_bits,
+                                                   const unsigned short* gate_in, const float* const* U1, float* dx, void* ws,
+                                                   size_t ws_bytes, void* stream) {
+  WinoPlan pls[FCD_CHAIN_MAXN];
+  FCD_CHECK_ARG(d && pool && dy && U1 && dx && codes && relu_bits, "fcd_conv2d_bwd_data_wino_chain_pool: null pointer");
+  FCD_CHECK_ARG(wino_chainp_plans(d, n, pool, 1, pls), "fcd_conv2d_bwd_data_wino_chain_pool: fcd_conv_wino_chain_pool_ok(d, n, pool, 1) == 0 for this run");
+  const size_t need = fcd_conv_wino_chain_pool_ws_bytes(d, n, pool, 1);
+  if (!ws || ws_bytes < need) {
+    fcd_set_error("fcd_conv2d_bwd_data_wino_chain_pool: workspace %zu < %zu bytes", ws_bytes, need);
+    return FCD_ERR_WORKSPACE;
+  }
+  size_t vmax = 0, mmax = 0;
+  for (int i = 0; i < n; ++i) {
+    vmax = std::max(vmax, pls[i].v_bytes);
+    mmax = std::max(mmax, pls[i].m_bytes);
+    FCD_CHECK_ARG(U1[i] && (pool[i] ? codes[i] != nullptr : (i == n - 1 || relu_bits[i] != nullptr)),
+                  "fcd_conv2d_bwd_data_wino_chain_pool: null filter pack / sign bits / code");
+  }
+  float* V = (float*)ws;
+  float* Mb = (float*)((char*)ws + ((vmax + 255) & ~(size_t)255));
+  float* tmp = (float*)((char*)Mb + ((mmax + 255) & ~(size_t)255));
+  hipStream_t st = (hipStream_t)stream;
+  const int N = d[0].N;
+  WinoGemmArgs ga;
+  for (int i = n - 1; i >= 0; --i) {
+    const WinoPlan& pl = pls[i];
+    const int H = d[i].H, W = d[i].W;
+    const double v = (double)pl.v_bytes, m = (double)pl.m_bytes;
+    const double in_b = i == n - 1 ? 4.0 * N * d[i].K * H * W * (pool[i] ? 0.3125 : 1.03125) + v : (double)pls[i + 1].m_bytes + v;
+    const double out_b = i == 0 ? m + m / pl.A2 * 16.0 : 0.0;
+    FcdProfScope prof(FCD_K_WINO_DGRAD, st, conv_flops(&d[i]), in_b + v + m + out_b + 4.0 * pl.A2 * pl.rows * pl.Kc,
+                      fcd_prof_tag_desc("wino_dgrad_chain", &d[i]));
+    if (i == n - 1) {
+      const WinoInSrc in = {dy, nullptr, pool[i] ? nullptr : relu_bits[i], pool[i] ? codes[i] : nullptr, H / 2, W / 2, nullptr};
+      wino_stage_input(pl, N, d[i].K, H, W, in, V, st);
+    } else if (pool[i]) {
+      if (wino_oi_unpool_ok(d[i].K, H, W)) {
+        wino_stage_oi_pool(pls[i + 1], ga, Mb, pl, N, H, W, nullptr, const_cast<unsigned char*>(codes[i]), 1, V, st);
+      } else {
+        const WinoOutDst out = {nullptr, 0, tmp, nullptr, nullptr, nullptr, nullptr, nullptr, nullptr, 0};
+        wino_stage_output(pls[i + 1], ga, Mb, N, d[i + 1].H, d[i + 1].W, out, st);
+        const WinoInSrc in = {tmp, nullptr, nullptr, codes[i], H / 2, W / 2, nullptr};
+        wino_stage_input(pl, N, d[i].K, H, W, in, V, st);
+      }
+    } else {
+      wino_stage_oi(pls[i + 1], ga, Mb, pl, N, H, W, nullptr, 0, nullptr, relu_bits[i], V, st);
+    }
+    ga = wino_stage_gemm(pl, U1[i], V, Mb, N, H, W, st);
+    if (i == 0) {
+      const WinoOutDst out = {nullptr, 0, dx, nullptr, nullptr, nullptr, nullptr, gate_in, nullptr, 0};
+      wino_stage_output(pl, ga, Mb, N, H, W, out, st);
+    }
+  }
+  FCD_LAUNCH_CHECK("conv2d_bwd_data_wino_chain_pool");
   return FCD_OK;
 }
 
diff --git a/fcd_gan_pytorch_amd/csrc/conv_wino_chain.hip b/fcd_gan_pytorch_amd/csrc/conv_wino_chain.hip
--- a/fcd_gan_pytorch_amd/csrc/conv_wino_chain.hip
+++ b/fcd_gan_pytorch_amd/csrc/conv_wino_chain.hip
@@ -135,6 +135,244 @@
   }
 }
 
+template <int PTW, int PTR, int NCH, int NT, int MINB>
+__global__ __launch_bounds__(NT, MINB) void wino_oi_pool_kernel(WinoOiArgs a) {
+  constexpr int A = 6, CHB = 32, VW = 2, GP = 2, QD = CHB / 4;
+  constexpr int BW = PTW / 2;
+  constexpr int RR = 2 * PTR + 5;
+  constexpr int CW = 4 * BW + 2;
+  constexpr int PL = (RR * CW) | 1;
+  static_assert(PTR == 1 || PTR == 2 || PTR == 4, "ring rows are worked out for these");
+  constexpr int PCW = PTW / NCH;
+  static_assert(NCH == 1 || PTR == 1, "column chunks: one tile row per NCH steps");
+  static_assert(PTR * PCW * QD * GP == NT, "output phase: one item per thread");
+  __shared__ float ring[CHB * PL];
+  const int tid = threadIdx.x;
+  const int kb = blockIdx.y * CHB;
+  const int n = blockIdx.z;
+  const int Hp = a.H, Wp = a.W;
+
+  for (int i = tid; i < CHB * RR; i += NT) {
+    const int c = i / RR, r = i % RR;
+    ring[c * PL + r * CW] = 0.f;
+    ring[c * PL + r * CW + CW - 1] = 0.f;
+  }
+  for (int i = tid; i < CHB * CW; i += NT) ring[(i / CW) * PL + i % CW] = 0.f;
+
+  const int og = tid % GP, ojl = (tid / GP) % PCW, orest = tid / (GP * PCW);
+  const int otr = orest % PTR, ocq = orest / PTR;
+  const int k0 = kb + 4 * ocq + VW * og;
+  const int cl0 = 4 * ocq + VW * og;
+  f32x2 m4[A * A];
+  auto issue = [&](int s) {
+    const int ty = (s / NCH) * PTR + otr, oj = (s % NCH) * PCW + ojl;
+    if (ty >= a.pTH) return;
+    const long long t = ((long long)n * a.pTH + ty) * a.pTW + oj;
+    const float* mp = a.Mb + ((size_t)(k0 >> 5) * a.tblk + (size_t)(t >> 5)) * 1024 +
+                      ((((k0 >> 2) & 1) * 4 + ((k0 >> 3) & 3)) * 32 + (int)(t & 31)) * 4 + (k0 & 3);
+#pragma unroll
+    for (int q = 0; q < A * A; ++q) m4[q] = __builtin_nontemporal_load((const f32x2*)(mp + (size_t)q * a.xs_blk));
+  };
+  auto out_phase = [&](int s) {
+    const int ty = (s / NCH) * PTR + otr, oj = (s % NCH) * PCW + ojl;
+    if (ty == a.pTH) {
+#pragma unroll
+      for (int e = 0; e < VW; ++e)
+#pragma unroll
+        for (int ch = 0; ch < NCH; ++ch) {
+          float* rp = ring + (cl0 + e) * PL + ((Hp + 1) % RR) * CW + 1 + 2 * (ch * PCW + ojl);
+          rp[0] = 0.f;
+          rp[1] = 0.f;
+        }
+    }
+    if (ty >= a.pTH) return;
+#pragma unroll
+    for (int e = 0; e < VW; ++e) {
+      float mv[A][A];
+      float mabs = 0.f;
+#pragma unroll
+      for (int q = 0; q < A * A; ++q) {
+        mv[q / A][q % A] = m4[q][e];
+        mabs = fmaxf(mabs, fabsf(m4[q][e]));
+      }
+      const float tie_floor = 4e-6f * mabs;
+      float o[4][4];
+      wino_out_tile<4>(mv, a.bias ? a.bias[k0 + e] : 0.f, 1, o);
+      float* rp = ring + (cl0 + e) * PL + 1 + 2 * oj;
+      unsigned char* cp = a.code + (((size_t)n * a.K + k0 + e) * Hp + 2 * ty) * Wp + 2 * oj;
+#pragma unroll
+      for (int wi = 0; wi < 2; ++wi) {
+        unsigned c0, c1;
+        const float p0 = wino_pool_window4(o[2 * wi][0], o[2 * wi][1], o[2 * wi + 1][0], o[2 * wi + 1][1], tie_floor, c0);
+        const float p1 = wino_pool_window4(o[2 * wi][2], o[2 * wi][3], o[2 * wi + 1][2], o[2 * wi + 1][3], tie_floor, c1);
+        const int ro = ((2 * ty + wi + 1) % RR) * CW;
+        rp[ro] = p0;
+        rp[ro + 1] = p1;
+        *(unsigned short*)(cp + (size_t)wi * Wp) = (unsigned short)(c0 | (c1 << 8));
+      }
+    }
+  };
+  auto done = [&](int s) {
+    if (s < 0) return 0;
+    if (s >= (a.pTH / PTR) * NCH) return a.TH;
+    const int v = 2 * PTR * ((s + 1) / NCH) - 5;
+    return v < 0 ? 0 : min(a.TH, v / 4 + 1);
+  };
+
+  const size_t xi_stride = (size_t)a.Q * a.T * 32;
+  const int steps = (a.pTH / PTR) * NCH + 1;
+  issue(0);
+#pragma unroll 1
+  for (int s = 0; s < steps; ++s) {
+    out_phase(s);
+    if (s + 1 < steps) issue(s + 1);
+    __syncthreads();
+    const int r0 = done(s - 1), r1 = done(s);
+#pragma unroll 1
+    for (int it = tid; it < (r1 - r0) * BW * CHB; it += NT) {
+      const int c = it % CHB, tl = it / CHB;
+      const int tc = tl % BW, r = r0 + tl / BW;
+      const float* rc = ring + c * PL + 4 * tc;
+      float d[A][A];
+#pragma unroll
+      for (int i = 0; i < A; ++i) {
+        const int ro = ((4 * r + i) % RR) * CW;
+#pragma unroll
+        for (int j = 0; j < A; ++j) d[i][j] = rc[ro + j];
+      }
+      float t1[A][A];
+      wino_in_rows<4>(d, t1);
+      const size_t t = ((size_t)n * a.TH + r) * a.TW + tc;
+      const int kg = kb + c;
+      float* vout = a.V + ((size_t)(kg >> 5) * a.T + t) * 32 + (kg & 31);
+#pragma unroll
+      for (int i = 0; i < A; ++i)
+#pragma unroll
+        for (int j = 0; j < A; ++j) vout[(size_t)(i * A + j) * xi_stride] = wino_in_col<4>(t1, i, j);
+    }
+    __syncthreads();
+  }
+}
+
+template <int PTW, int NT, int MINB>
+__global__ __launch_bounds__(NT, MINB) void wino_oi_unpool_kernel(WinoOiArgs a) {
+  constexpr int A = 6, CHB = 32, VW = 2, GP = 2, QD = CHB / 4;
+  constexpr int BW = 2 * PTW;
+  constexpr int RR = 9;
+  constexpr int CW = 4 * BW + 2;
+  constexpr int PL = (RR * CW) | 1;
+  static_assert(PTW * QD * GP <= NT, "output phase: one item per thread");
+  __shared__ float ring[CHB * PL];
+  const int tid = threadIdx.x;
+  const int kb = blockIdx.y * CHB;
+  const int n = blockIdx.z;
+  const int Hp = a.H >> 1, Wp = a.W >> 1;
+
+  for (int i = tid; i < CHB * RR; i += NT) {
+    const int c = i / RR, r = i % RR;
+    ring[c * PL + r * CW] = 0.f;
+    ring[c * PL + r * CW + CW - 1] = 0.f;
+  }
+  for (int i = tid; i < CHB * CW; i += NT) ring[(i / CW) * PL + i % CW] = 0.f;
+
+  const int og = tid % GP, oj = (tid / GP) % PTW, ocq = tid / (GP * PTW);
+  const bool o_on = ocq < QD;
+  const int k0 = kb + 4 * ocq + VW * og;
+  const int cl0 = 4 * ocq + VW * og;
+  f32x2 m4[A * A];
+  unsigned cwn[VW][4];
+  auto issue = [&](int ty) {
+    if (!o_on || ty >= a.pTH) return;
+    const long long t = ((long long)n * a.pTH + ty) * a.pTW + oj;
+    const float* mp = a.Mb + ((size_t)(k0 >> 5) * a.tblk + (size_t)(t >> 5)) * 1024 +
+                      ((((k0 >> 2) & 1) * 4 + ((k0 >> 3) & 3)) * 32 + (int)(t & 31)) * 4 + (k0 & 3);
+#pragma unroll
+    for (int q = 0; q < A * A; ++q) m4[q] = __builtin_nontemporal_load((const f32x2*)(mp + (size_t)q * a.xs_blk));
+#pragma unroll
+    for (int e = 0; e < VW; ++e)
+#pragma unroll
+      for (int i = 0; i < 4; ++i)
+        cwn[e][i] = *(const unsigned*)(a.code + (((size_t)n * a.K + k0 + e) * Hp + 4 * ty + i) * Wp + 4 * oj);
+  };
+  auto put = [&](int e, const float (&g0)[4], const float (&g1)[4], unsigned c0, unsigned c1, int y0) {
+    float* rp = ring + (cl0 + e) * PL + 1 + 8 * oj;
+#pragma unroll
+    for (int i = 0; i < 2; ++i)
+#pragma unroll
+      for (int ai = 0; ai < 2; ++ai) {
+        const int ro = ((y0 + 2 * i + ai + 1) % RR) * CW;
+#pragma unroll
+        for (int j = 0; j < 4; ++j) {
+          const unsigned cd = ((i ? c1 : c0) >> (8 * j)) & 0xffu;
+          const float g = i ? g1[j] : g0[j];
+#pragma unroll
+          for (int bi = 0; bi < 2; ++bi) rp[ro + 2 * j + bi] = cd == (unsigned)((ai << 1) | bi | 4) ? g : 0.f;
+        }
+      }
+  };
+  const size_t xi_stride = (size_t)a.Q * a.T * 32;
+  auto in_phase = [&](int r) {
+    __syncthreads();
+#pragma unroll 1
+    for (int it = tid; it < (r >= 0 ? BW * CHB : 0); it += NT) {
+      const int c = it % CHB, tc = it / CHB;
+      const float* rc = ring + c * PL + 4 * tc;
+      float d[A][A];
+#pragma unroll
+      for (int i = 0; i < A; ++i) {
+        const int ro = ((4 * r + i) % RR) * CW;
+#pragma unroll
+        for (int j = 0; j < A; ++j) d[i][j] = rc[ro + j];
+      }
+      float t1[A][A];
+      wino_in_rows<4>(d, t1);
+      const size_t t = ((size_t)n * a.TH + r) * a.TW + tc;
+      const int kg = kb + c;
+      float* vout = a.V + ((size_t)(kg >> 5) * a.T + t) * 32 + (kg & 31);
+#pragma unroll
+      for (int i = 0; i < A; ++i)
+#pragma unroll
+        for (int j = 0; j < A; ++j) vout[(size_t)(i * A + j) * xi_stride] = wino_in_col<4>(t1, i, j);
+    }
+    __syncthreads();
+  };
+
+  issue(0);
+#pragma unroll 1
+  for (int ty = 0; ty < a.pTH; ++ty) {
+    float o[VW][4][4];
+    unsigned cw[VW][4];
+    if (o_on) {
+#pragma unroll
+      for (int e = 0; e < VW; ++e) {
+        float mv[A][A];
+#pragma unroll
+        for (int q = 0; q < A * A; ++q) mv[q / A][q % A] = m4[q][e];
+        wino_out_tile<4>(mv, 0.f, 0, o[e]);
+#pragma unroll
+        for (int i = 0; i < 4; ++i) cw[e][i] = cwn[e][i];
+        put(e, o[e][0], o[e][1], cw[e][0], cw[e][1], 8 * ty);
+      }
+      issue(ty + 1);
+    }
+    in_phase(2 * ty - 1);
+    if (o_on) {
+#pragma unroll
+      for (int e = 0; e < VW; ++e) put(e, o[e][2], o[e][3], cw[e][2], cw[e][3], 8 * ty + 4);
+    }
+    in_phase(2 * ty);
+  }
+  if (o_on) {
+#pragma unroll
+    for (int e = 0; e < VW; ++e) {
+      float* rp = ring + (cl0 + e) * PL + ((a.H + 1) % RR) * CW + 1 + 8 * oj;
+#pragma unroll
+      for (int j = 0; j < 8; ++j) rp[j] = 0.f;
+    }
+  }
+  in_phase(a.TH - 1);
+}
+
 int wino_oi_ok(int K, int H, int W) {
   if (!fcd_sw(FCD_SW_WINO_CHAIN) || (K & 31) || (H & 3) || (W & 3)) return 0;
   const int TW = W / 4, TH = H / 4;
@@ -144,6 +382,32 @@
   return 0;
 }
 
+int wino_oi_pool_ok(int K, int H, int W) {
+  if (!fcd_sw(FCD_SW_WINO_CHAIN) || !fcd_sw(FCD_SW_WINO_CHAIN_POOL) || (K & 31) || (H & 7) || (W & 7)) return 0;
+  const int TW = W / 4;
+  return TW == 8 || TW == 16 || TW == 32 || TW == 64;
+}
+int wino_oi_unpool_ok(int K, int H, int W) {
+  if (!fcd_sw(FCD_SW_WINO_CHAIN) || !fcd_sw(FCD_SW_WINO_CHAIN_POOL) || (K & 31) || (H & 7) || (W & 7)) return 0;
+  const int TW = W / 4;
+  return TW == 8 || TW == 16 || TW == 32;
+}
+
+void wino_oi_pool_launch(const WinoOiArgs& a, hipStream_t st) {
+  const dim3 grid(1, (unsigned)(a.K / 32), (unsigned)a.N);
+  if (a.pTW == 64) hipLaunchKernelGGL((wino_oi_pool_kernel<64, 1, 2, 512, 1>), grid, dim3(512), 0, st, a);
+  else if (a.pTW == 32) hipLaunchKernelGGL((wino_oi_pool_kernel<32, 1, 2, 256, 2>), grid, dim3(256), 0, st, a);
+  else if (a.pTW == 16) hipLaunchKernelGGL((wino_oi_pool_kernel<16, 1, 1, 256, 2>), grid, dim3(256), 0, st, a);
+  else hipLaunchKernelGGL((wino_oi_pool_kernel<8, 2, 1, 256, 2>), grid, dim3(256), 0, st, a);
+}
+
+void wino_oi_unpool_launch(const WinoOiArgs& a, hipStream_t st) {
+  const dim3 grid(1, (unsigned)(a.K / 32), (unsigned)a.N);
+  if (a.pTW == 16) hipLaunchKernelGGL((wino_oi_unpool_kernel<16, 512, 1>), grid, dim3(512), 0, st, a);
+  else if (a.pTW == 8) hipLaunchKernelGGL((wino_oi_unpool_kernel<8, 256, 2>), grid, dim3(256), 0, st, a);
+  else hipLaunchKernelGGL((wino_oi_unpool_kernel<4, 256, 2>), grid, dim3(256), 0, st, a);
+}
+
 void wino_oi_launch(const WinoOiArgs& a, hipStream_t st) {
   const dim3 grid((unsigned)cdiv(a.TW, a.TW >= 16 ? 16 : a.TW), (unsigned)(a.K / 32), (unsigned)a.N);
   if (a.TW == 32) hipLaunchKernelGGL((wino_oi_kernel<32, 1, 2, 512, 1>), dim3(1, (unsigned)(a.K / 32), (unsigned)a.N), dim3(512), 0, st, a);
diff --git a/fcd_gan_pytorch_amd/csrc/switches.h b/fcd_gan_pytorch_amd/csrc/switches.h
--- a/fcd_gan_pytorch_amd/csrc/switches.h
+++ b/fcd_gan_pytorch_amd/csrc/switches.h
@@ -27,6 +27,7 @@
   X(WINO_BNSTATS, 1, "BatchNorm statistics out of the F(4x4) output transform")                                                     \
   X(WINO_KEEPV, 1, "weight gradient reuses the forward pass's transformed input (0: re-transforms x)")                              \
   X(WINO_CHAIN, 1, "frozen VGG runs through the fused output->input transform (0: layer by layer)")                                 \
+  X(WINO_CHAIN_POOL, 1, "frozen VGG runs continue across an untapped max-pool: pooling / un-pooling inside the fused transform (0: one run per block)") \
   X(WINO_RELU_BITS, 1, "frozen F(4x4) layers keep 16 sign bits per tile as the ReLU mask (0: fp32 y on the tape)")                  \
   X(BN_FUSE, 1, "train-mode BatchNorm + ReLU inside the next convolution's loader / the density head (0: kernels of their own)")    \
   X(PAIR_CAT, 1, "first decoder convolution reads skip pair + upsampled tensor in place (0: materialise the concatenation)")        \
diff --git a/include/fcdgan_hip.h b/include/fcdgan_hip.h
--- a/include/fcdgan_hip.h
+++ b/include/fcdgan_hip.h
@@ -120,6 +120,16 @@
 int fcd_conv2d_bwd_data_wino_chain(const fcd_conv_desc* d, int n, const float* dy, const unsigned char* pool_code,
                                    const unsigned short* const* relu_bits, const unsigned short* gate_in,
                                    const float* const* U1, float* dx, void* ws, size_t ws_bytes, void* stream);
+int fcd_conv_wino_chain_pool_ok(const fcd_conv_desc* d, int n, const int* pool, int mode);
+size_t fcd_conv_wino_chain_pool_ws_bytes(const fcd_conv_desc* d, int n, const int* pool, int mode);
+int fcd_conv_wino_chain_pool_bwd_fused(const fcd_conv_desc* d, int n, const int* pool, int i);
+int fcd_conv2d_fwd_wino_chain_pool(const fcd_conv_desc* d, int n, const int* pool, const float* x, const float* const* U,
+                                   const float* const* bias, float* y, float* pool_y, unsigned char* const* codes,
+                                   unsigned short* const* relu_bits, void* ws, size_t ws_bytes, void* stream);
+int fcd_conv2d_bwd_data_wino_chain_pool(const fcd_conv_desc* d, int n, const int* pool, const float* dy,
+                                        const unsigned char* const* codes, const unsigned short* const* relu_bits,
+                                        const unsigned short* gate_in, const float* const* U1, float* dx, void* ws,
+                                        size_t ws_bytes, void* stream);
 int fcd_conv2d_bwd_data_wino(const fcd_conv_desc* d, const float* dy, const float* relu_out,
                              const unsigned char* pool_code, const float* U, float* dx, void* ws,
                              size_t ws_bytes, void* stream);
```
